# dryman/HashMergeJoin

Measured on AMD Instinct MI355X. Metric: probe-side tuples/s + achieved HBM GB/s, |R|=|S|=2^28 u64 keys, higher is better.
Workload: dtype u64

## Files before the change

### hashmergejoin_amd/_lib.py

```python
import ctypes as C
import os

HMJ_MATERIALIZE = 0x01
HMJ_ORDERED = 0x02
HMJ_FIRST_WINS = 0x04
HMJ_CHECKSUM = 0x08
HMJ_SUM_PROBE = 0x10
HMJ_NULL_EQUAL = 0x20
HMJ_OK, HMJ_E_ARG, HMJ_E_NODEV, HMJ_E_OOM, HMJ_E_HIP, HMJ_E_UNSUPPORTED = 0, -1, -2, -3, -4, -5
HMJ_E_RCCL, HMJ_E_PEER, HMJ_E_TIMEOUT = -6, -7, -8
HMJ_ABI_VERSION = 5
HMJ_PATH_SLAB, HMJ_PATH_EXACT, HMJ_PATH_UNIQ_WRITE, HMJ_PATH_SPLIT, HMJ_PATH_WINDOW = 0x1, 0x2, 0x4, 0x8, 0x10
HMJ_PATH_ORDER_DEFERRED, HMJ_PATH_ORDER_BY_KEY, HMJ_PATH_PREPARED, HMJ_PATH_CHUNKED_BUILD = 0x20, 0x40, 0x80, 0x100
HMJ_PATH_HOT_KEY_HINT = 0x200
HMJ_PATH_SLAB_PROBE = 0x400
HMJ_PATH_SORTED_WRITE = 0x800
HMJ_PATH_SORTED_FK = 0x1000
HMJ_PATH_DENSE_BUILD = 0x2000
HMJ_PATH_GLOBAL_TABLE = 0x100000
HMJ_PATH_ORDER_BY_RANK_SORT = 0x200000
HMJ_PATH_ORDERED_EXPANSION = 0x400000
HMJ_PATH_LDS_TABLE = 0x800000
HMJ_PATH_RANK_RUNS = 0x1000000
HMJ_PATH_RANK_LOOKUP_IN_PASS = 0x2000000
HMJ_PATH_SORT_MSD = 0x4000000
HMJ_PATH_KEY_RANGES = 0x8000000
HMJ_PATH_SLAB_ONE_PASS = 0x80000
HMJ_PATH_HOST_PIPELINE = 0x4000
HMJ_PATH_SORTED_FK_HALF = 0x8000
HMJ_PATH_LOOKBACK_TIMEOUT = 0x10000
HMJ_PATH_SORTED_FK_WIDE = 0x20000
HMJ_PATH_PRESORTED = 0x40000

_HERE = os.path.dirname(os.path.abspath(__file__))
_U64P = C.POINTER(C.c_uint64)


class HmjError(RuntimeError):
    def __init__(self, code, msg):
        super().__init__("hmj error %d: %s" % (code, msg))
        self.code = code


class JoinResult(C.Structure):
    _fields_ = [("n_matches", C.c_uint64), ("sum_r", C.c_uint64), ("sum_s", C.c_uint64),
                ("xor_fold", C.c_uint64), ("mix_sum", C.c_uint64), ("sum_probe_all", C.c_uint64),
                ("key", C.c_void_p), ("rval", C.c_void_p), ("sval", C.c_void_p)]

    def checks(self):
        return {k: int(getattr(self, k)) for k in ("n_matches", "sum_r", "sum_s", "xor_fold", "mix_sum")}


HMJ_JOIN_INNER, HMJ_JOIN_SEMI, HMJ_JOIN_ANTI, HMJ_JOIN_PROBE_OUTER = 0, 1, 2, 3


class JoinOpts(C.Structure):
    _fields_ = [("struct_size", C.c_uint32), ("kind", C.c_uint32), ("outer_fill", C.c_uint64),
                ("n_probe_matched", C.c_uint64), ("n_probe_unmatched", C.c_uint64)]


HMJ_BUILD_SEMI, HMJ_BUILD_ANTI, HMJ_BUILD_OUTER, HMJ_FULL_OUTER = 1, 2, 3, 4


class BuildJoinOpts(C.Structure):
    _fields_ = [("struct_size", C.c_uint32), ("kind", C.c_uint32), ("build_fill", C.c_uint64), ("probe_fill", C.c_uint64),
# ... 223 lines not shown
                ("ms_partition_build", C.c_float), ("ms_partition_probe", C.c_float),
                ("ms_hist", C.c_float), ("ms_scan", C.c_float), ("ms_scatter", C.c_float),
                ("ms_offsets", C.c_float), ("ms_probe_count", C.c_float),
                ("ms_out_scan", C.c_float), ("ms_probe_write", C.c_float), ("ms_order", C.c_float),
                ("radix_bits", C.c_int), ("radix_passes", C.c_int),
                ("n_scatter_launches", C.c_int), ("n_split_retries", C.c_int),
                ("bytes_scatter", C.c_uint64), ("bytes_hist", C.c_uint64),
                ("bytes_probe_count", C.c_uint64), ("bytes_probe_write", C.c_uint64),
                ("path", C.c_uint32), ("key_prefix_bits", C.c_int32), ("key_window_low", C.c_int32),
                ("n_probe_items", C.c_uint32), ("ms_scatter_pass0", C.c_float), ("ms_scatter_pass1", C.c_float)]

    def as_dict(self):
        return {n: getattr(self, n) for n, _ in self._fields_}


class PlanDesc(C.Structure):
    _fields_ = [("struct_size", C.c_uint32), ("path", C.c_uint32), ("radix_bits", C.c_int32), ("radix_passes", C.c_int32),
                ("pass_bits", C.c_int32 * 4), ("key_prefix_bits", C.c_int32), ("key_window_low", C.c_int32),
                ("n_partitions", C.c_uint32), ("probe_items", C.c_uint32), ("attempts", C.c_uint32), ("refused", C.c_uint32),
                ("cooling", C.c_uint32), ("workload", C.c_uint64)]

    def as_dict(self):
        d = {n: getattr(self, n) for n, _ in self._fields_}
        d["pass_bits"] = list(self.pass_bits)
        return d


HMJ_REFUSED_GTABLE_SHAPE, HMJ_REFUSED_GTABLE_COOLING, HMJ_REFUSED_GTABLE_GAVE_UP = 0x1, 0x2, 0x4
HMJ_REFUSED_RANK_SORT_MODEL, HMJ_REFUSED_RANK_SORT_COOLING, HMJ_REFUSED_RANK_SORT_GAVE_UP = 0x8, 0x10, 0x20
HMJ_REFUSED_SLAB_SHAPE, HMJ_REFUSED_SLAB_COOLING, HMJ_REFUSED_SLAB_SORTED_INPUT, HMJ_REFUSED_SLAB_OVERFLOW = 0x40, 0x80, 0x100, 0x200
HMJ_REFUSED_FAST_WRITE_COOLING, HMJ_REFUSED_FAST_WRITE_GAVE_UP = 0x400, 0x800
HMJ_REFUSED_SLAB_PROBE_COOLING, HMJ_REFUSED_SLAB_PROBE_OVERFLOW = 0x1000, 0x2000
HMJ_REFUSED_PREFIX_VIOLATED, HMJ_REFUSED_EXPANSION_GAVE_UP = 0x4000, 0x8000
HMJ_COOL_UNIQ_WRITE, HMJ_COOL_SORTED_WRITE, HMJ_COOL_GTABLE, HMJ_COOL_GTABLE_WRITE = 0x1, 0x2, 0x4, 0x8
HMJ_COOL_RANK_SORT, HMJ_COOL_RANK_SORT_SLAB, HMJ_COOL_EXPANSION, HMJ_COOL_SORT_SLAB = 0x10, 0x20, 0x40, 0x80
HMJ_COOL_SLAB, HMJ_COOL_SLAB_PROBE, HMJ_COOL_ONE_PASS_WRITE, HMJ_COOL_EXACT_PREFIX = 0x100, 0x200, 0x400, 0x800
HMJ_COOL_RANK_RUNS, HMJ_COOL_SORT_MSD = 0x1000, 0x2000


HMJ_PLACE_MAX_CAND = 4


class PlaceInfo(C.Structure):
    _fields_ = [("name", C.c_char * 16), ("bytes", C.c_uint64), ("fill_TBps", C.c_float), ("candidates", C.c_int),
                ("ms_search", C.c_float), ("searched", C.c_int), ("aborted", C.c_int), ("budget_ms", C.c_float),
                ("cand_ms_alloc", C.c_float * HMJ_PLACE_MAX_CAND), ("cand_ms_fill", C.c_float * HMJ_PLACE_MAX_CAND),
                ("cand_TBps", C.c_float * HMJ_PLACE_MAX_CAND)]


def lib_path():
    return os.environ.get("HMJ_LIB") or os.path.join(_HERE, "libhmj_hip.so")


class ExchangeInfo(C.Structure):
    _fields_ = [("n_ranks", C.c_int), ("owner_mode", C.c_int), ("rounds_build", C.c_uint32), ("rounds_probe", C.c_uint32),
                ("recv_build", C.c_uint64), ("recv_probe", C.c_uint64), ("ms_split", C.c_float),
                ("ms_exchange_build", C.c_float), ("ms_exchange_probe", C.c_float), ("ms_local", C.c_float),
                ("ms_total", C.c_float), ("digit_bits", C.c_int32), ("digit_low", C.c_int32), ("n_subjoins", C.c_uint32),
                ("fallback", C.c_uint32), ("sample_max_share", C.c_float), ("ms_kernels", C.c_float),
                ("ms_exposed", C.c_float)]

    def as_dict(self):
        return {n: getattr(self, n) for n, _ in self._fields_}


HMJ_MAX_RANKS, HMJ_MAX_ROUNDS = 16, 16
HMJ_UNIQUE_ID_BYTES = 128
HMJ_OWNER_DIGIT, HMJ_OWNER_SPLIT = 0, 1


# ... 110 lines not shown
```

### hashmergejoin_amd/csrc/api.hip

```cpp
#include <hip/hip_runtime.h>
#include <sys/mman.h>

#include <algorithm>
#include <cstdio>
#include <cstdlib>
#include <chrono>
#include <cmath>
#include <cstring>
#include <mutex>
#include <string>
#include <thread>
#include <vector>

#include "hmj_ctx.h"

using hmj::u32;
using hmj::u64;
using namespace hmj_host;

namespace hmj_host {

constexpr int kMaxEvents = 1024;

int fail(hmj_ctx* c, int code, const char* what, hipError_t e) {
// ... 29 lines not shown
  acc->ms_scatter_pass[0] += t.ms_scatter_pass[0];
  acc->ms_scatter_pass[1] += t.ms_scatter_pass[1];
  if (t.radix_passes) {
    acc->radix_bits = t.radix_bits;
    acc->radix_passes = t.radix_passes;
    acc->key_prefix_bits = t.key_prefix_bits;
    acc->key_window_low = t.key_window_low;
  }
  acc->n_probe_items += t.n_probe_items;
}

static int ilog2_u64(uint64_t v) { return v ? 63 - __builtin_clzll(v) : 0; }
uint64_t workload_signature(uint64_t n_build, uint64_t n_probe, uint32_t flags, int kind) {
  const uint32_t mode = ((flags & HMJ_ORDERED) ? 4u : 0u) | ((flags & (HMJ_MATERIALIZE | HMJ_ORDERED)) ? 2u : 0u) |
                        ((flags & HMJ_FIRST_WINS) ? 1u : 0u);
  return ((uint64_t)(kind & 31) << 20) | ((uint64_t)mode << 16) | ((uint64_t)ilog2_u64(n_build) << 8) | (uint64_t)ilog2_u64(n_probe);
}
WorkloadMemo* memo_for(hmj_ctx* c, uint64_t sig) {
  auto it = c->memos.find(sig);
  if (it == c->memos.end()) {
    if (c->memos.size() >= 1024) c->memos.clear();
    it = c->memos.emplace(sig, c->memo_init).first;
  }
  c->wm = &it->second;
  c->wm_sig = sig;
  return c->wm;
}
uint32_t WorkloadMemo::cooling() const {
  return (uniq_cooldown ? HMJ_COOL_UNIQ_WRITE : 0u) | (sorted_cooldown ? HMJ_COOL_SORTED_WRITE : 0u) | (gtable_cooldown ? HMJ_COOL_GTABLE : 0u) |
         (gtable_write_cooldown ? HMJ_COOL_GTABLE_WRITE : 0u) | (gtable_sort_cooldown ? HMJ_COOL_RANK_SORT : 0u) |
         (gtable_sort_slab_cooldown ? HMJ_COOL_RANK_SORT_SLAB : 0u) | (expand_cooldown ? HMJ_COOL_EXPANSION : 0u) |
         (sort_slab_cooldown ? HMJ_COOL_SORT_SLAB : 0u) | (slab_cooldown ? HMJ_COOL_SLAB : 0u) | (slab_probe_cooldown ? HMJ_COOL_SLAB_PROBE : 0u) |
         (one_pass_write_cooldown ? HMJ_COOL_ONE_PASS_WRITE : 0u) | (exact_prefix_joins ? HMJ_COOL_EXACT_PREFIX : 0u) |
         (rank_runs_cooldown ? HMJ_COOL_RANK_RUNS : 0u) | (sort_msd_cooldown ? HMJ_COOL_SORT_MSD : 0u);
}

int wait_arrival(hmj_ctx* c, hipEvent_t ev) {
  if (c->arrive_wait) return c->arrive_wait(c, ev);
  HIP_TRY(hipStreamWaitEvent(c->stream, ev, 0));
  return HMJ_OK;
}

int ensure_dev(hmj_ctx* c, DevBuf& b, size_t bytes) {
  if (bytes <= b.cap) return HMJ_OK;
  if (c && (&b == &c->rbuf[0] || &b == &c->rbuf[1] || &b == &c->r_off || &b == &c->slab_br || &b == &c->cnt_br))
    c->prep.valid = false;
  if (b.p) {
    hipError_t e = hipFree(b.p);
    b.p = nullptr;
    b.cap = 0;
    if (e != hipSuccess) return fail(c, HMJ_E_HIP, "hipFree", e);
  }
  size_t want = bytes + (bytes >> 4) + 256;
#ifdef HMJ_DEV
  if (const char* e = getenv("HMJ_ALLOC_PAD_KB")) want += (size_t)atoll(e) << 10;
  if (const char* e = getenv("HMJ_ALLOC_ROUND_MB")) {
    const size_t g = (size_t)atoll(e) << 20;
    if (g) want = (want + g - 1) / g * g;
  }
#endif
  const auto t_alloc0 = std::chrono::steady_clock::now();
  hipError_t e = hipMalloc(&b.p, want);
  if (e != hipSuccess) {
    b.p = nullptr;
    (void)hipGetLastError();
    return fail(c, HMJ_E_OOM, "hipMalloc", e);
  }
// ... 424 lines not shown
  a.r_off = (const u32*)c->r_off.p;
  a.S = Sp;
  a.s_off = (const u32*)c->s_off.p;
  a.P = P;
  a.Q = Q;
  a.accum = (u64*)c->accum.p;
  return a;
}
static hmj::ProbeArgs slab_probe_args(hmj_ctx* c, const hmj::SlabGeom* build_slabs, const void* Rp, const DevBuf& s_slab,
                                      const DevBuf& s_cnt, u32 s_cap, u32 P, u32 Q) {
  hmj::ProbeArgs a;
  std::memset(&a, 0, sizeof(a));
  if (build_slabs) {
    a.R = c->slab_br.p;
    a.r_cnt = (const u32*)c->cnt_br.p;
    a.r_cap = build_slabs->CB;
    a.r_cnt_n = c->cnt_br.cap / 4;
    a.r_rows = c->slab_br.cap / 16;
  } else {
    a.R = Rp;
    a.r_off = (const u32*)c->r_off.p;
  }
  a.S = s_slab.p;
  a.s_cnt = (const u32*)s_cnt.p;
  a.s_cap = s_cap;
  a.s_cnt_n = s_cnt.cap / 4;
  a.s_rows = s_slab.cap / 16;
  a.P = P;
  a.Q = Q;
  a.accum = (u64*)c->accum.p;
  return a;
}

static int slab_pass_a(hmj_ctx* c, const void* in, u32 n, int rel, int low, int bits, const hmj::SlabGeom& g, bool arriving) {
  u64* acc = (u64*)c->accum.p;
  const u64 a_rows = c->slab_a.cap / 16, a_cnt = c->cnt_a.cap / 4;
  const int sp = span_begin(c, K_SCATTER, rel, 0);
  if (arriving) {
    u32 w_done = 0;
    for (size_t i = 0; i < c->arrive_ev.size(); i++) {
      RC_TRY(wait_arrival(c, c->arrive_ev[i]));
      const bool last = i + 1 == c->arrive_ev.size();
      const u32 w_end = last ? g.WA : (u32)std::min<u64>(g.WA, c->arrive_rows[i] / g.rpw);
      if (w_end > w_done) {
        HIP_TRY(hmj::launch_slab_a(in, n, low, bits, g, c->slab_a.p, a_rows, (u32*)c->cnt_a.p, a_cnt, acc, c->stream, w_done, w_end));
        w_done = w_end;
      }
    }
  } else {
    HIP_TRY(hmj::launch_slab_a(in, n, low, bits, g, c->slab_a.p, a_rows, (u32*)c->cnt_a.p, a_cnt, acc, c->stream));
  }
  span_end(c, sp);
  c->timing.bytes_scatter += 32ull * n;
  return HMJ_OK;
}
static int slab_passes(hmj_ctx* c, const void* in, u32 n, int rel, int low, int ba, int bb, const hmj::SlabGeom& g, DevBuf& sb,
                       DevBuf& cb, bool arriving) {
  RC_TRY(slab_pass_a(c, in, n, rel, low, ba, g, arriving));
  const int sp = span_begin(c, K_SCATTER, rel, 1);
  HIP_TRY(hmj::launch_slab_b(c->slab_a.p, (const u32*)c->cnt_a.p, ba, low + ba, bb, g, sb.p, sb.cap / 16, (u32*)cb.p, cb.cap / 4,
                             (u64*)c->accum.p, c->stream));
  span_end(c, sp);
  c->timing.bytes_scatter += 32ull * n;
  return HMJ_OK;
}

static int clear_matched(hmj_ctx* c, size_t slots, u32** matched) {
  const size_t bytes = (slots / 32 + 1) * 4;
  RC_TRY(ensure_dev(c, c->matched, bytes));
  *matched = (u32*)c->matched.p;
  HIP_TRY(hipMemsetAsync(c->matched.p, 0, bytes, c->stream));
  return HMJ_OK;
}

int order_rows(hmj_ctx* c, const u32* vstart, const u32* in_base32, const u64* in_base64, u32 P, u32 Q, int low,
               u64 n, bool by_key_only, bool many_per_key, const u64** rk, const u64** rr, const u64** rs, int* retry_code) {
  const size_t bytes = (size_t)n * 8;
  RC_TRY(ensure_dev(c, c->ord_key, bytes));
  RC_TRY(ensure_dev(c, c->ord_rval, bytes));
  RC_TRY(ensure_dev(c, c->ord_sval, bytes));
  const bool can_sort = n <= 0xFFFFFFFFull;
  if (by_key_only && !can_sort) {
    *retry_code = kRetryNoWinOrdered;
    return HMJ_OK;
  }
  int sp = span_begin(c, K_ORDER, -1);
  HIP_TRY(hmj::launch_order((const u64*)c->part_out_off.p, vstart, in_base32, in_base64, P, Q, low,
                            (const u64*)c->out_key.p, (const u64*)c->out_rval.p, (const u64*)c->out_sval.p,
                            (u64*)c->ord_key.p, (u64*)c->ord_rval.p, (u64*)c->ord_sval.p, (u64*)c->accum.p,
                            can_sort ? 65536u : 0u, many_per_key, c->num_cus * 4, c->stream));
  span_end(c, sp);
  u64* h = (u64*)c->h_accum.p;
  HIP_TRY(hipMemcpyAsync(&h[hmj::ACC_ERR], (u64*)c->accum.p + hmj::ACC_ERR, 8, hipMemcpyDeviceToHost, c->stream));
  HIP_TRY(hipStreamSynchronize(c->stream));
  if (h[hmj::ACC_ERR] & hmj::ERR_ORDER_FAIL)
    return fail(c, HMJ_E_UNSUPPORTED, "HMJ_ORDERED: one partition's result exceeds 2^31-1 rows and the whole result 2^32-1 rows");
// ... 520 lines not shown

static int run_slab_join(hmj_ctx* c, const JoinCall& j, const JoinPlan& p) {
  const bool materialize = j.materialize(), first = j.first(), extra = j.extra();
  const u32 nb = j.nb, np = j.np, np_plan = p.np_plan, P = p.P;
  const int* pass_bits = p.pass_bits;
  hmj::SlabGeom gr, gs;
  if (p.allow_slab && c->slab_mode && c->wm->slab_cooldown == 0 && !c->prepare_only && !(c->timing.path & HMJ_PATH_SLAB) &&
      !((!materialize || p.fast_write) && p.Q == 1 && p.probe_fits && p.passes == 2 && pass_bits[0] <= hmj::SLAB_MAX_BITS &&
        pass_bits[1] <= hmj::SLAB_MAX_BITS && p.dense_scale <= 2.5))
    c->plan.refused |= HMJ_REFUSED_SLAB_SHAPE;
  if (!(p.allow_slab && c->slab_mode && c->wm->slab_cooldown == 0 && (!materialize || p.fast_write) && p.Q == 1 &&
        p.probe_fits &&
        p.passes == 2 && pass_bits[0] <= hmj::SLAB_MAX_BITS && pass_bits[1] <= hmj::SLAB_MAX_BITS &&
        slab_sizes_ok(c, nb, np_plan, materialize || np_plan < nb) &&
        p.dense_scale <= 2.5 &&
        hmj::slab_geometry(nb, pass_bits[0], pass_bits[1], &gr, 0, 1.0, p.dense_scale) &&
        hmj::slab_geometry(np_plan, pass_bits[0], pass_bits[1], &gs, 0,
                           (nb && np_plan > nb) ? (double)np_plan / (double)nb : 1.0, p.dense_scale)))
    return kPlanNotTaken;
  const bool reuse = c->prep.valid && c->prep.slab && c->prep.ptr == j.R && c->prep.n == nb &&
                     c->prep.low == p.low && c->prep.B == p.B;
  c->prep.valid = false;
  c->timing.path |= HMJ_PATH_SLAB | (reuse ? HMJ_PATH_PREPARED : 0u);
  c->timing.n_probe_items = P;
  const int ba = pass_bits[0], bb = pass_bits[1];
  const u64 rows_a = gr.rows_a > gs.rows_a ? gr.rows_a : gs.rows_a;
  const u32 wa = gr.WA > gs.WA ? gr.WA : gs.WA;
  RC_TRY(ensure_dev(c, c->slab_a, rows_a * 16));
  RC_TRY(ensure_dev(c, c->cnt_a, ((size_t)wa << ba) * 4));
  RC_TRY(ensure_dev(c, c->slab_br, gr.rows_b * 16));
  RC_TRY(ensure_dev(c, c->slab_bs, gs.rows_b * 16));
  RC_TRY(ensure_dev(c, c->cnt_br, (size_t)P * gr.KB * 4));
  RC_TRY(ensure_dev(c, c->cnt_bs, (size_t)P * gs.KB * 4));
  if (!reuse) RC_TRY(slab_passes(c, j.R, nb, 0, p.low, ba, bb, gr, c->slab_br, c->cnt_br, false));
  if (!c->prepare_only) RC_TRY(slab_passes(c, j.S, np, 1, p.low, ba, bb, gs, c->slab_bs, c->cnt_bs, !c->arrive_ev.empty()));
  u64* hh;
  if (c->prepare_only) {
    RC_TRY(read_accum(c, &hh));
    if (hh[hmj::ACC_ERR] & hmj::ERR_SLAB) {
      c->wm->slab_cooldown = 8;
      return kRetryNoSlab;
    }
    c->prep.valid = true;
    c->prep.slab = true;
    c->prep.ptr = j.R;
    c->prep.n = nb;
    c->prep.low = p.low;
    c->prep.B = p.B;
    return HMJ_OK;
  }
  hmj::ProbeArgs sa = slab_probe_args(c, &gr, nullptr, c->slab_bs, c->cnt_bs, gs.CB, P, 1);
  if (p.fast_write)
    return unique_key_write(c, sa, true, nb, np, p.low, extra, p.verify_pfx ? p.prefix : 0, p.pfx_ref, j.ordered(), j.to_host,
                            p.fk_wide_plan, p.dense_scale, j.out);
#ifdef HMJ_DEV
  sa.debug = c->dev_ablate;
#endif
  int sp = span_begin(c, K_PROBE_COUNT, -1);
  if (first || extra) {
    sa.extra = (extra ? 1u : 0u) | (first ? 2u : 0u);
    HIP_TRY(hmj::launch_probe_count_ext(sa, nullptr, nullptr, true, c->num_cus, c->stream));
  } else {
    HIP_TRY(hmj::launch_probe_count_slab(sa, c->num_cus, c->stream));
  }
  span_end(c, sp);
  c->timing.bytes_probe_count = 16ull * ((u64)nb + np);
  RC_TRY(read_accum(c, &hh));
  if (hh[hmj::ACC_ERR] & hmj::ERR_SLAB) {
    c->wm->slab_cooldown = 8;
    return kRetryNoSlab;
  }
  result_sums(j.out, hh);
  return HMJ_OK;
}

static int partition_build_exact(hmj_ctx* c, const JoinCall& j, const JoinPlan& p, const void** Rp) {
  const bool reuse_exact = c->prep.valid && !c->prep.slab && c->prep.ptr == j.R && c->prep.n == j.nb &&
                           c->prep.low == p.low && c->prep.B == p.B;
  c->prep.valid = false;
  c->timing.path |= HMJ_PATH_EXACT | (reuse_exact ? HMJ_PATH_PREPARED : 0u);
  if (reuse_exact) {
    *Rp = c->prep.Rp;
  } else {
    RC_TRY(partition_relation(c, j.R, j.nb, c->rbuf, p.low, p.passes, p.pass_bits, 0, Rp, p.asc_r));
    const int s = span_begin(c, K_OFFSETS, -1);
    HIP_TRY(hmj::launch_part_offsets(*Rp, j.nb, p.low, p.B, (u32*)c->r_off.p, c->stream));
    span_end(c, s);
  }
  if (c->prepare_only) {
    HIP_TRY(hipStreamSynchronize(c->stream));
    c->prep.valid = true;
    c->prep.slab = false;
    c->prep.ptr = j.R;
    c->prep.Rp = *Rp;
    c->prep.n = j.nb;
    c->prep.low = p.low;
    c->prep.B = p.B;
  }
  return HMJ_OK;
}

static int run_probe_slab_join(hmj_ctx* c, const JoinCall& j, const JoinPlan& p, const void* Rp) {
  const bool materialize = j.materialize(), first = j.first(), extra = j.extra();
// ... 1296 lines not shown
  if (const char* e = getenv("HMJ_SORT_MSD_MIN_LOG2")) {
    const int l = atoi(e);
    if (l >= 16 && l <= 32) c->sort_msd_min = 1ull << l;
  }
  if (const char* e = getenv("HMJ_SORT_SLAB_MIN_LOG2")) {
    const int l = atoi(e);
    if (l >= 12 && l <= 32) c->sort_slab_min = 1ull << l;
  }
  if (const char* e = getenv("HMJ_GTABLE_SORT_SLAB_MIN_LOG2")) {
    const int l = atoi(e);
    if (l >= 12 && l <= 32) c->gtable_sort_slab_min = 1ull << l;
  }
  if (const char* e = getenv("HMJ_GTABLE_SORT_FANOUT")) c->gtable_sort_fanout = atoi(e) > 0 ? (u32)atoi(e) : 1u;
  if (const char* e = getenv("HMJ_PLACE")) {
    c->place_tune = atoi(e) != 0;
    if (atoi(e) > 0) {
      c->place_tries = atoi(e);
      c->place_search_always = true;
    }
  }
  if (const char* e = getenv("HMJ_PLACE_BUDGET_MS")) {
    if (atof(e) >= 0.0) c->place_budget_ms = (float)atof(e);
  }
  if (const char* e = getenv("HMJ_PLACE_MIN_MB")) {
    const long long mb = atoll(e);
    if (mb >= 1) c->place_min_bytes = (size_t)mb << 20;
  }
  if (const char* e = getenv("HMJ_UPLOAD")) c->staged_upload = std::strcmp(e, "staged") == 0;
  if (const char* e = getenv("HMJ_HOST_PIPELINE")) c->host_pipeline = atoi(e) != 0;
  if (const char* e = getenv("HMJ_SLAB_MIN_LOG2")) {
    const int l = atoi(e);
    if (l >= 16 && l <= 31) c->slab_min_rows = 1u << l;
  }
  if (const char* e = getenv("HMJ_SLAB_PROBE_KB")) {
    const int k = atoi(e);
    if (k >= 1 && k <= 512) c->slab_probe_kb = (u32)k;
  }
  if (const char* e = getenv("HMJ_TRACE")) c->trace = atoi(e) != 0;
#ifdef HMJ_DEV
  if (const char* e = getenv("HMJ_LTABLE")) c->ltable_mode = atoi(e) != 0;
  if (const char* e = getenv("HMJ_GTABLE_MAX_LOG2")) {
    const int l = atoi(e);
    if (l >= 0 && l <= 28) c->gtable_max_rows = 1ull << l;
  }
  if (const char* e = getenv("HMJ_GTABLE_FANOUT")) c->gtable_min_fanout = atoi(e) > 0 ? (u32)atoi(e) : 0u;
  if (const char* e = getenv("HMJ_GTABLE_WG")) c->gtable_wg_per_cu = atoi(e) > 0 ? atoi(e) : 8;
  if (const char* e = getenv("HMJ_BUILD_SORT_MSD")) c->build_sort_msd = atoi(e) != 0;
  if (const char* e = getenv("HMJ_GTABLE_SORT_SLAB")) c->gtable_sort_slab = atoi(e) != 0;
  if (const char* e = getenv("HMJ_FK_PAYLOAD_BUCKETS")) c->fk_payload_buckets = atoi(e) > 0 ? (u32)atoi(e) : 0u;
  if (const char* e = getenv("HMJ_ORDERED_EXPANSION")) c->expand_mode = atoi(e) != 0;
  if (const char* e = getenv("HMJ_SORT_SLAB")) c->sort_slab = atoi(e) != 0;
  if (const char* e = getenv("HMJ_GTABLE_SLOTS")) c->gtable_slots_per_row = atoi(e) >= 2 ? (u32)atoi(e) : 2u;
  if (const char* e = getenv("HMJ_GTABLE_MAX_LOG_CAP")) {
    const int l = atoi(e);
    if (l >= 10 && l <= 30) c->gtable_max_log_cap = l;
  }
  if (const char* e = getenv("HMJ_DENSE_PLAN")) c->dense_plan = atoi(e) != 0;
  if (const char* e = getenv("HMJ_SORTED_WRITE")) {
    c->sorted_mode = atoi(e) != 0;
    c->memo_init.sorted_chained = atoi(e) == 2;
    c->sorted_chained_forced = atoi(e) == 2 || atoi(e) == 3;
  }
  if (const char* e = getenv("HMJ_SORTED_HALF")) c->sorted_half = atoi(e) != 0;
  if (const char* e = getenv("HMJ_FK_PLAN"))
    c->fk_plan = std::strcmp(e, "wide") == 0 ? 1 : std::strcmp(e, "half") == 0 ? 2 : std::strcmp(e, "narrow") == 0 ? 3 : 0;
  if (const char* e = getenv("HMJ_SORTED_WIDE")) c->memo_init.sorted_wide = atoi(e) != 0;
// ... 776 lines not shown
```

### hashmergejoin_amd/csrc/hmj_ctx.h

```cpp
#pragma once
#include <hip/hip_runtime.h>

#include <string>
#include <unordered_map>
#include <vector>

#include "../../include/hmj.h"
#include "hmj_args.h"
#include "hmj_dev.h"
#include "hmj_launch.h"
#include "hmj_smallplan.h"

struct hmj_comm;
struct hmj_ctx;

namespace hmj_host {

struct DevBuf {
  void* p = nullptr;
  size_t cap = 0;
};
struct HostBuf {
  void* p = nullptr;
  size_t cap = 0;
  bool pinned = true;
};
template <int N>
struct PhaseEvents {
  hipEvent_t ev[N] = {};
  int record(hmj_ctx* c, int k);
  float ms(int a, int b) {
    float t = 0.f;
    if (ev[a] && ev[b] && hipEventElapsedTime(&t, ev[a], ev[b]) != hipSuccess) {
      (void)hipGetLastError();
      t = 0.f;
    }
    return t;
  }
  void destroy() {
    for (hipEvent_t& e : ev) {
      if (e) (void)hipEventDestroy(e);
      e = nullptr;
    }
// ... 108 lines not shown
  void each_buf(F f) {
    for (DevBuf* b : {&acc, &below, &tied, &blk, &blk_off, &tie[0], &tie[1], &words, &map}) f(*b);
  }
};

enum Kind {
  K_TOTAL = 0, K_H2D, K_D2H, K_HIST, K_SCAN, K_SCATTER, K_OFFSETS, K_PROBE_COUNT, K_OUT_SCAN,
  K_PROBE_WRITE, K_ORDER, K_NKINDS
};
struct Span {
  int kind, rel, e0, e1;
  int pass;
};

struct WorkloadMemo {
  int uniq_cooldown = 0;
  int sorted_cooldown = 0;
  bool sorted_chained = false;
  bool sorted_wide = true;
  bool sorted_fk = false;
  int sorted_fk_age = 0;
  int gtable_cooldown = 0;
  int gtable_write_cooldown = 0;
  int gtable_sort_cooldown = 0;
  int gtable_sort_slab_cooldown = 0;
  int rank_runs_cooldown = 0;
  int rank_lookup_cooldown = 0;
  int expand_cooldown = 0;
  int sort_slab_cooldown = 0;
  int sort_msd_cooldown = 0;
  int slab_cooldown = 0;
  int slab_probe_cooldown = 0;
  int one_pass_write_cooldown = 0;
  int exact_prefix_joins = 0;
  uint32_t cooling() const;
};

}

struct hmj_ctx {
  using DevBuf = hmj_host::DevBuf;
  using HostBuf = hmj_host::HostBuf;
  using Span = hmj_host::Span;
  using WorkloadMemo = hmj_host::WorkloadMemo;
  using u32 = hmj::u32;
  using u64 = hmj::u64;
  int device = 0, num_cus = 256;
  hipStream_t own_stream = nullptr, stream = nullptr;
  DevBuf rbuf[2], sbuf[2], in_r, in_s, hist, totals, r_off, s_off, part_count, part_out_off, accum,
      out_key, out_rval, out_sval, ord_key, ord_rval, ord_sval, offs64, irregular, matched, vparts,
      slab_a, slab_br, slab_bs, cnt_a, cnt_br, cnt_bs, lookback, gtab, piece_off,
      split_r, split_s, split_off, cat_key, cat_rval, cat_sval,
      msd_off,
      bmatched, bsweep;
  hmj_host::KeyJoinWs str_ws, col_ws, mix_ws;
  hmj_host::GroupWs grp_ws;
  hmj_host::OrderWs ord_ws;
  hmj_host::TakeWs take_ws;
  hmj_host::TakeStrWs takestr_ws;
  hmj_host::AggWs agg_ws;
  hmj_host::FilterWs filter_ws;
  hmj_host::WindowWs window_ws;
  hmj_host::TopkWs topk_ws;
  int memo_kind = 0;
  HostBuf h_accum, h_key, h_rval, h_sval;
  int host_threads = 0;
// ... 42 lines not shown
  uint64_t gtable_max_rows = 1ull << 17;
  u32 gtable_min_fanout = 0;
  uint64_t gtable_min_probe = 1;
  int gtable_wg_per_cu = 8;
  u32 gtable_slots_per_row = 16;
  int gtable_max_log_cap = 18;
  bool ltable_mode = true;
  bool gtable_sort_mode = true;
  u32 gtable_sort_fanout = 128;
  bool rank_runs_mode = true;
  int rank_runs_max_cut = 10;
  int rank_runs_max_group = 3;
  int rank_runs_max_level = 2;
  uint64_t big_join_rows = 1ull << 29;
  bool promote_to_ordered = true;
  bool key_ranges = true;
  int key_ranges_force = 0;
  bool rank_runs_wave = true;
  bool build_sort_msd = true;
  bool gtable_sort_slab = true;
  u64 gtable_sort_slab_min = 1ull << 25;
  bool expand_mode = true;
  u32 fk_payload_buckets = 24;
  u32 expand_fk_fanout = 0;
  bool expand_allow_rebits = true;
  int expand_rebits = 0;
  bool sort_msd = true;
  double sort_msd_mean = 1200.0;
  int sort_msd_max_bits = 18;
  u64 sort_msd_min = 1ull << 22;
  bool sort_slab = true;
  u64 sort_slab_min = 1ull << 25;
  int slab_mode = 1;
  bool staged_upload = false;
  bool host_pipeline = true;
  hipStream_t copy_stream = nullptr;
  std::vector<hipEvent_t> copy_ev;
  bool split_mode = true;
  bool window_mode = true;
  u32 slab_min_rows = 1u << 21;
  u32 slab_probe_kb = 0;
  bool one_pass_slab = true;
  int scatter_variant = 1;
  bool profiling = false;
  bool trace = false;
#ifdef HMJ_DEV
  u32 dev_ablate = 0;
#endif
  std::vector<hipEvent_t> events;
  std::vector<Span> spans;
  int ev_used = 0;
  hmj_timing timing;
  std::string last_error;
  hmj_comm* comm = nullptr;
  std::vector<u64> arrive_rows;
  std::vector<hipEvent_t> arrive_ev;
  bool sample_build_only = false;
  int (*arrive_wait)(hmj_ctx*, hipEvent_t) = nullptr;
};


namespace hmj_host {
int fail(hmj_ctx* c, int code, const char* what, hipError_t e = hipSuccess);
#define HIP_TRY(expr)                                                        \
  do {                                                                       \
    hipError_t _e = (expr);                                                  \
// ... 38 lines not shown
```

### hashmergejoin_amd/csrc/hmj_dev.h

```cpp
#pragma once
#include <hip/hip_runtime.h>
#include <stdint.h>

namespace hmj {

typedef unsigned long long u64;
typedef unsigned int u32;
typedef unsigned short u16;

struct __attribute__((aligned(16))) Tup {
  u64 key;
  u64 val;
};

constexpr int kWave = 64;
#ifndef HMJ_SCAN_DPP
#define HMJ_SCAN_DPP 1
#endif

#ifndef HMJ_STREAM_POLICY
#define HMJ_STREAM_POLICY 2
#endif
typedef u64 u64x2_t __attribute__((ext_vector_type(2)));
__device__ __forceinline__ void store_stream(Tup* p, const Tup& v) {
// ... 51 lines not shown
          slot[r] = (slot[r] + 1) & mask;
          any_live = true;
        }
      }
    }
  }
}

constexpr int RP_THREADS = 512;
constexpr int RP_WAVES = RP_THREADS / kWave;
constexpr int RP_ITEMS = 8;
constexpr int RP_TILE = RP_THREADS * RP_ITEMS;
constexpr int RP_MAX_BITS = 9;
constexpr int RP_MAXD = 1 << RP_MAX_BITS;
constexpr int RP_MAX_BLOCKS = 2048;

constexpr int PB_THREADS = 1024;
constexpr int PB_CAP = 5120;
constexpr int PB_LOG_NB = 12;
constexpr int PB_TARGET_AVG = 4096;
constexpr int PB_PLAN_SLACK = 256;

constexpr int SLAB_KB = 4;
constexpr int SLAB_MAX_BITS = 9;

enum { ACC_N = 0, ACC_SUM_R, ACC_SUM_S, ACC_XOR, ACC_MIX, ACC_SUM_P, ACC_ERR, ACC_PAD };
constexpr u64 ERR_SLAB = 2;
constexpr u64 ERR_ORDER_DEFER = 16;
constexpr u64 ERR_ORDER_FAIL = 32;
constexpr u64 ERR_SORTED = 64;
constexpr u64 ERR_FASTPATH = 8;
constexpr u64 ERR_GTABLE = 128;
constexpr u64 ERR_PREFIX = 4;

__device__ __forceinline__ u64 mix64(u64 x) {
  x ^= x >> 30;
  x *= 0xBF58476D1CE4E5B9ull;
  x ^= x >> 27;
  x *= 0x94D049BB133111EBull;
  x ^= x >> 31;
  return x;
}

__device__ __forceinline__ u64 tmix(u64 key, u64 rval, u64 sval) {
  u64 t = mix64(key);
  t = mix64(t ^ rval);
  t = mix64(t + sval);
  return t;
}

__device__ __forceinline__ int lane_id() {
  return __builtin_amdgcn_mbcnt_hi(~0u, __builtin_amdgcn_mbcnt_lo(~0u, 0u));
}

__device__ __forceinline__ u32 popc_below(u64 m) {
  return __builtin_amdgcn_mbcnt_hi((u32)(m >> 32), __builtin_amdgcn_mbcnt_lo((u32)m, 0u));
}

__device__ __forceinline__ u32 wave_incl_scan_u32(u32 v, int ) {
#if HMJ_SCAN_DPP
  v += (u32)__builtin_amdgcn_update_dpp(0, (int)v, 0x111, 0xF, 0xF, false);
  v += (u32)__builtin_amdgcn_update_dpp(0, (int)v, 0x112, 0xF, 0xF, false);
  v += (u32)__builtin_amdgcn_update_dpp(0, (int)v, 0x114, 0xF, 0xF, false);
  v += (u32)__builtin_amdgcn_update_dpp(0, (int)v, 0x118, 0xF, 0xF, false);
  v += (u32)__builtin_amdgcn_update_dpp(0, (int)v, 0x142, 0xA, 0xF, false);
  v += (u32)__builtin_amdgcn_update_dpp(0, (int)v, 0x143, 0xC, 0xF, false);
// ... 83 lines not shown
```

### hashmergejoin_amd/csrc/hmj_launch.h

```cpp
#pragma once
#include <hip/hip_runtime.h>
#include <stddef.h>
#include <stdint.h>

#include <atomic>

namespace hmj {
typedef unsigned long long u64;
typedef unsigned int u32;

struct SmemAttrOnce {
  std::atomic<unsigned long long> devices{0};
};
inline hipError_t ensure_max_smem(SmemAttrOnce& once, const void* kernel, size_t bytes) {
  int dev = 0;
  hipError_t e = hipGetDevice(&dev);
  if (e != hipSuccess) return e;
  const unsigned long long bit = 1ull << (dev & 63);
  if (dev < 64 && (once.devices.load(std::memory_order_acquire) & bit)) return hipSuccess;
  e = hipFuncSetAttribute(kernel, hipFuncAttributeMaxDynamicSharedMemorySize, (int)bytes);
  if (e != hipSuccess) return e;
  if (dev < 64) once.devices.fetch_or(bit, std::memory_order_release);
  return hipSuccess;
}

constexpr int kMaxRanks = 16;
struct OwnerFn {
  u32 mode;
  u32 G;
  u64 spl[kMaxRanks - 1];
};
int radix_tile_rows(int bits, int variant);
void radix_pass_geometry(u32 n, int tile, u32* nblk, u32* rows_per_block);
size_t radix_scatter_smem_bytes();
hipError_t launch_radix_hist(const void* in, u32 n, int tile, int shift, int bits, u32* hist,
                             u32 nblk, u32 rows_per_block, hipStream_t st, const OwnerFn* own = nullptr);
hipError_t launch_owner_scatter(const void* in, void* out, u32 n, int bits, const OwnerFn& own,
                                const u32* hist_scanned, const u32* totals, u32 nblk, u32 rows_per_block,
                                u64* offsets_out, hipStream_t st);
hipError_t launch_radix_rowscan(u32* hist, u32 nblk, int bits, u32* totals, hipStream_t st);
hipError_t launch_radix_scatter(const void* in, void* out, u32 n, int variant, int shift, int bits,
                                const u32* hist_scanned, const u32* totals, u32 nblk,
                                u32 rows_per_block, u64* offsets_out, hipStream_t st);
struct SlabGeom {
  u32 WA, rpw, CA, CB, KB;
  u64 rows_a, rows_b;
};
bool slab_geometry(u32 n, int bits_a, int bits_b, SlabGeom* g, u32 kb = 0, double fan = 1.0, double density = 1.0);
bool slab_geometry_one_pass(u32 n, int bits, double keys_per_digit, u32 max_workers, SlabGeom* g, double density = 1.0);
u32 slab_capacity(double mean, double fan);
hipError_t launch_slab_a(const void* in, u32 n, int shift, int bits, const SlabGeom& g, void* slab_a, u64 slab_a_rows,
                         u32* cnt_a, u64 cnt_a_n, u64* accum, hipStream_t st, u32 w_begin = 0, u32 w_end = 0xFFFFFFFFu);
hipError_t launch_slab_b(const void* slab_a, const u32* cnt_a, int bits_a, int shift, int bits,
                         const SlabGeom& g, void* slab_b, u64 slab_b_rows, u32* cnt_b, u64 cnt_b_n, u64* accum, hipStream_t st);
hipError_t launch_key_sample(const void* R, u32 nb, const void* S, u32 np, u64* out, hipStream_t st);
hipError_t launch_key_exact(const void* R, u32 nb, const void* S, u32 np, u64 ref, u64* out, int num_cus, hipStream_t st,
                            bool ref_is_first_key = false);
hipError_t launch_check_partitioned(const void* a, u32 n, int low, int bits, u32* flag, int num_cus, hipStream_t st);
hipError_t launch_part_offsets(const void* a, u32 n, int low, int bits, u32* off, hipStream_t st);

struct ProbeArgs {
  const void* R;
  const u32* r_off;
  const void* S;
  const u32* s_off;
  u32 P;
  u32 Q;
  u64* part_count;
  const u64* part_out_off;
  u64* out_key;
  u64* out_rval;
  u64* out_sval;
  u64 out_cap;
  u64* accum;
  const u32* item_list;
  const u32* n_item_list;
  const u32* r_cnt;
  const u32* s_cnt;
  u32 r_cap, s_cap;
  u32 s_wa, s_ppi;
  u64 r_cnt_n, s_cnt_n;
  u64 r_rows, s_rows;
  const u64* item_base;
  const u32* r_end;
  const u32* s_end;
  u32 extra;
  u32 pfx_shift;
  u64 pfx_val;
  u32* matched;
  u32 debug;
};
hipError_t launch_probe(const ProbeArgs& a, int mode, bool first_wins, bool extra, int grid,
                        hipStream_t st);
int probe_default_grid(int num_cus);
hipError_t launch_probe_kind(const ProbeArgs& a, int mode, int kind, bool first_wins, u64 fill, int grid, hipStream_t st);
hipError_t launch_probe_build_kind(const ProbeArgs& a, int mode, int kind, u64 fill, u32* bmark, int grid, hipStream_t st);
hipError_t launch_build_sweep(const ProbeArgs& a, const u32* r_off, u32 P, const u32* vstart, u64* sweep_n, int mode,
                              bool set, u64 fill, int num_cus, hipStream_t st);
hipError_t launch_probe_count_ext(const ProbeArgs& a, u32* irregular, u32* n_irregular, bool slab,
                                  int num_cus, hipStream_t st);
hipError_t launch_probe_count_slab(const ProbeArgs& a, int num_cus, hipStream_t st);
hipError_t launch_probe_write_sorted(const ProbeArgs& a, bool slab, bool fk, int shape, u64* lookback, bool chained, int key_low,
                                     int num_cus, hipStream_t st);
hipError_t launch_probe_write_uniq(const ProbeArgs& a, bool slab, int num_cus, hipStream_t st);
hipError_t launch_slab_np(const u32* cnt, u32 P, u64* out, hipStream_t st);
hipError_t launch_probe_count_fast(const ProbeArgs& a, u32* irregular, u32* n_irregular, bool big,
                                   bool per_partition_counts, int num_cus, hipStream_t st);
hipError_t launch_scan_u64(const u64* in, u64* out_excl, u32 n, hipStream_t st);
hipError_t launch_probe_expand_ordered(const ProbeArgs& a, int key_low, int num_cus, hipStream_t st);
hipError_t launch_order(const u64* part_out_off, const u32* vstart, const u32* in_base32, const u64* in_base64, u32 P, u32 Q,
                        int low, const u64* akey, const u64* arval, const u64* asval, u64* bkey, u64* brval,
                        u64* bsval, u64* accum, u32 defer_rows, bool many_per_key, int grid, hipStream_t st);
hipError_t launch_compact(const u64* part_out_off, const u32* in_base32, const u64* in_base64, u32 P, const u64* akey,
                          const u64* arval, const u64* asval, u64* bkey, u64* brval, u64* bsval, int grid, hipStream_t st);
hipError_t launch_rekey(void* pairs, u64 n, const u64* col, hipStream_t st);

hipError_t launch_gtable_build(const void* R, u32 nb, void* tab, int log_cap, u64* accum, bool first, int num_cus,
                               hipStream_t st);
hipError_t launch_gtable_probe(const void* S, u32 np, const void* tab, int log_cap, const void* R, u64* accum, bool first,
                               bool extra, int num_cus, int wg_per_cu, hipStream_t st);
hipError_t launch_gtable_write(const void* S, u32 np, const void* tab, int log_cap, const void* R, u64* accum, u64* out_key,
                               u64* out_rval, u64* out_sval, bool first, bool extra, int num_cus, int wg_per_cu, hipStream_t st);

hipError_t launch_ltable_probe(const void* R, u32 nb, const void* S, u32 np, u64* accum, bool first, bool extra, int num_cus, hipStream_t st);
int ltable_max_rows();
hipError_t launch_sval_range(const void* S, u32 np, u64* out2 , int num_cus, hipStream_t st,
                             u32 every = 1 );
// ... 43 lines not shown
```

### hashmergejoin_amd/csrc/probe.hip

```cpp
#include "hmj_dev.h"
#include "hmj_launch.h"
#include <type_traits>

namespace hmj {

constexpr u32 PB_NB = 1u << PB_LOG_NB;
constexpr u32 NIL = 0xFFFFu;
static_assert(PB_CAP < 0xFFFF, "chain links are 16-bit");

struct ProbeSmem {
  u64 key[PB_CAP];
  u64 val[PB_CAP];
  u32 head[PB_NB];
  u32 aux[PB_CAP];
  u16 next[PB_CAP];
  u32 scratch[PB_THREADS / kWave + 1];
  u64 pcount;
  u64 red[8];
  u64 obase;
  u32 wtot[PB_THREADS / kWave];
  u32 nslot;
};
constexpr u32 PB_BATCH = 2 * PB_THREADS;
static_assert(PB_BATCH <= PB_CAP, "a batch must fit an empty table");

__device__ __forceinline__ u32 key_bucket(u64 key, int sh, u32 mask) {
  return (sh >= 0 ? (u32)(key >> sh) : (u32)(key << (-sh))) & mask;
}

__device__ __forceinline__ u32 tab_hash(u64 k) {
  u32 x = (u32)k ^ ((u32)(k >> 32) * 0x85EBCA6Bu);
  x *= 0x9E3779B1u;
  return x >> (32 - PB_LOG_NB);
}
// ... 850 lines not shown
};

template <int LOG_NB>
__device__ __forceinline__ u32 fast_hash(u64 k) {
  u32 x = (u32)k ^ ((u32)(k >> 32) * 0x85EBCA6Bu);
  x *= 0x9E3779B1u;
  return x >> (32 - LOG_NB);
}

template <int THREADS, int ROWS = FP_ROWS>
__device__ __forceinline__ void fp_load(Tup (&t)[ROWS], const Tup* __restrict__ base, u32 n,
                                        int tid) {
#pragma unroll
  for (int k = 0; k < ROWS; k++) {
    u32 i = k * THREADS + tid;
    t[k] = base[i < n ? i : n - 1];
  }
}

static_assert(SLAB_KB == 4, "fp_load_slab / fp_load_pieces / slab_np_kernel unroll exactly four pieces per partition");
template <int THREADS, int ROWS = FP_ROWS>
__device__ __forceinline__ void fp_load_slab(Tup (&t)[ROWS], const Tup* __restrict__ base, u32 cap,
                                             u32 p1, u32 p2, u32 p3, u32 n, int tid) {
#pragma unroll
  for (int k = 0; k < ROWS; k++) {
    u32 i = k * THREADS + tid;
    i = i < n ? i : n - 1;
    const u32 j = (i >= p1) + (i >= p2) + (i >= p3);
    const u32 pre = j == 0 ? 0u : (j == 1 ? p1 : (j == 2 ? p2 : p3));
    t[k] = base[(u64)j * cap + (i - pre)];
  }
}

template <int THREADS>
__device__ __forceinline__ void fp_load_pieces(Tup (&t)[FP_ROWS], const Tup* __restrict__ base, u32 cap, u32 cnt_mine, int tid) {
  constexpr int QT = THREADS / 4;
  const u32 g = (u32)tid / QT, l = (u32)tid % QT;
  const Tup* __restrict__ piece = base + (u64)g * cap;
  const u32 last = cnt_mine ? cnt_mine - 1 : 0;
#pragma unroll
  for (int k = 0; k < FP_ROWS; k++) {
    const u32 r = l + (u32)k * QT;
    t[k] = piece[r < last ? r : last];
  }
}

template <int THREADS, int LOG_NB, bool PCOUNT, bool SLAB, int OUT>
__global__ __launch_bounds__(THREADS, 4) void probe_count_fast_kernel(
    ProbeArgs a, u32* __restrict__ irregular, u32* __restrict__ n_irregular) {
  typedef FastSmem<THREADS, LOG_NB> Smem;
  constexpr u32 CAP = Smem::CAP, NB = 1u << LOG_NB;
  constexpr bool PIECES = SLAB && OUT == 0 && !PCOUNT && HMJ_PROBE_PIECES;
  constexpr u32 QT = THREADS / 4, PIECE_CAP = FP_ROWS * QT;
  extern __shared__ __attribute__((aligned(16))) unsigned char smem_raw[];
  Smem& sm = *reinterpret_cast<Smem*>(smem_raw);
  const Tup* __restrict__ R = static_cast<const Tup*>(a.R);
  const Tup* __restrict__ S = static_cast<const Tup*>(a.S);
  const u32* __restrict__ r_off = a.r_off;
  const u32* __restrict__ s_off = a.s_off;
  const u32* __restrict__ r_end = (SLAB || a.r_end == nullptr) ? a.r_off + 1 : a.r_end;
  const u32* __restrict__ s_end = (SLAB || a.s_end == nullptr) ? a.s_off + 1 : a.s_end;
  const u32 P = a.P;
  const int tid = threadIdx.x;
  u64 acc_n = 0, acc_r = 0, acc_s = 0, acc_x = 0, acc_m = 0, acc_p = 0;
  bool pfx_bad = false, giveup = false;
  for (u32 i = tid; i < NB; i += THREADS) sm.head[i] = 0;
  if (tid < 2) sm.itemcnt[tid] = 0;
  u32 epoch = 0;
  u32 prev_p = 0xFFFFFFFFu, parity = 0;

  u32 p = blockIdx.x;
  u32 rb = 0, nb = 0, sb = 0, np = 0;
  bool regular = false;
  Tup br[FP_ROWS], pr[FP_ROWS], pq[FP_ROWS];
  u32 r1 = 0, r2 = 0, r3 = 0, s1 = 0, s2 = 0, s3 = 0, r1n = 0, r2n = 0, r3n = 0, s1n = 0, s2n = 0, s3n = 0;
  u32 rm = 0, sm_ = 0, rmn = 0, smn = 0;
  const u32 my_piece = (u32)tid / QT;
  bool slab_bad = false;
  if (p < P) {
    if (SLAB) {
      const u32* rc = a.r_cnt + (u64)p * SLAB_KB;
      const u32* sc = a.s_cnt + (u64)p * SLAB_KB;
      r1 = rc[0]; r2 = r1 + rc[1]; r3 = r2 + rc[2]; nb = r3 + rc[3];
      s1 = sc[0]; s2 = s1 + sc[1]; s3 = s2 + sc[2]; np = s3 + sc[3];
      if (nb > CAP || np > CAP) slab_bad = true;
      if (PIECES) {
        rm = my_piece == 0 ? rc[0] : my_piece == 1 ? rc[1] : my_piece == 2 ? rc[2] : rc[3];
        sm_ = my_piece == 0 ? sc[0] : my_piece == 1 ? sc[1] : my_piece == 2 ? sc[2] : sc[3];
        if (rc[0] > PIECE_CAP || rc[1] > PIECE_CAP || rc[2] > PIECE_CAP || rc[3] > PIECE_CAP || sc[0] > PIECE_CAP ||
            sc[1] > PIECE_CAP || sc[2] > PIECE_CAP || sc[3] > PIECE_CAP) {
          slab_bad = true;
          nb = CAP + 1;
        }
      }
    } else {
      rb = r_off[p]; nb = r_end[p] - rb;
      sb = s_off[p]; np = s_end[p] - sb;
    }
    regular = nb && np && nb <= CAP && np <= CAP;
    if (regular) {
      if (PIECES) {
        fp_load_pieces<THREADS>(br, R + (u64)p * SLAB_KB * a.r_cap, a.r_cap, rm, tid);
        fp_load_pieces<THREADS>(pr, S + (u64)p * SLAB_KB * a.s_cap, a.s_cap, sm_, tid);
      } else if (SLAB) {
        fp_load_slab<THREADS>(br, R + (u64)p * SLAB_KB * a.r_cap, a.r_cap, r1, r2, r3, nb, tid);
        if (OUT == 0) fp_load_slab<THREADS>(pr, S + (u64)p * SLAB_KB * a.s_cap, a.s_cap, s1, s2, s3, np, tid);
      } else {
        fp_load<THREADS>(br, R + rb, nb, tid);
        if (OUT == 0) fp_load<THREADS>(pr, S + sb, np, tid);
      }
    }
  }
  const Tup* __restrict__ dummy = reinterpret_cast<const Tup*>(a.accum);
  auto load_build = [&](Tup (&t)[FP_ROWS], bool ok, u32 pp, u32 rb_, u32 nb_, u32 q1, u32 q2, u32 q3, u32 mine) {
    if (PIECES)
      fp_load_pieces<THREADS>(t, ok ? R + (u64)pp * SLAB_KB * a.r_cap : dummy, ok ? a.r_cap : 0u, ok ? mine : 1u, tid);
    else if (SLAB)
      fp_load_slab<THREADS>(t, ok ? R + (u64)pp * SLAB_KB * a.r_cap : dummy, ok ? a.r_cap : 0u, ok ? q1 : 1u, ok ? q2 : 1u,
                            ok ? q3 : 1u, ok ? nb_ : 1u, tid);
    else
      fp_load<THREADS>(t, ok ? R + rb_ : dummy, ok ? nb_ : 1u, tid);
  };
  auto load_probe = [&](Tup (&t)[FP_ROWS], bool ok, u32 pp, u32 sb_, u32 np_, u32 q1, u32 q2, u32 q3, u32 mine) {
    if (PIECES)
      fp_load_pieces<THREADS>(t, ok ? S + (u64)pp * SLAB_KB * a.s_cap : dummy, ok ? a.s_cap : 0u, ok ? mine : 1u, tid);
    else if (SLAB)
      fp_load_slab<THREADS>(t, ok ? S + (u64)pp * SLAB_KB * a.s_cap : dummy, ok ? a.s_cap : 0u, ok ? q1 : 1u, ok ? q2 : 1u,
                            ok ? q3 : 1u, ok ? np_ : 1u, tid);
    else
      fp_load<THREADS>(t, ok ? S + sb_ : dummy, ok ? np_ : 1u, tid);
  };
  const int tid_outer = tid;
  while (p < P) {
    int tid = tid_outer;
    if constexpr (OUT != 0) asm volatile("" : "+v"(tid));
    u64 out_base = (u64)sb;
    if constexpr (OUT == 1 && SLAB) {
      const u64* ibp = a.item_base + p;
      asm volatile("s_load_dwordx2 %0, %1, 0x0\n\ts_waitcnt lgkmcnt(0)" : "=s"(out_base) : "s"(ibp) : "memory");
    }
    const u32 pn = __builtin_amdgcn_readfirstlane(p + gridDim.x);
    u32 rb2 = 0, nb2 = 0, sb2 = 0, np2 = 0;
    bool regular2 = false;
    if (pn < P) {
      if (SLAB) {
        const u32* rc = a.r_cnt + (u64)pn * SLAB_KB;
        const u32* sc = a.s_cnt + (u64)pn * SLAB_KB;
        r1n = rc[0]; r2n = r1n + rc[1]; r3n = r2n + rc[2]; nb2 = r3n + rc[3];
        s1n = sc[0]; s2n = s1n + sc[1]; s3n = s2n + sc[2]; np2 = s3n + sc[3];
        if (nb2 > CAP || np2 > CAP) slab_bad = true;
        if (PIECES) {
          rmn = my_piece == 0 ? rc[0] : my_piece == 1 ? rc[1] : my_piece == 2 ? rc[2] : rc[3];
          smn = my_piece == 0 ? sc[0] : my_piece == 1 ? sc[1] : my_piece == 2 ? sc[2] : sc[3];
          if (rc[0] > PIECE_CAP || rc[1] > PIECE_CAP || rc[2] > PIECE_CAP || rc[3] > PIECE_CAP || sc[0] > PIECE_CAP ||
              sc[1] > PIECE_CAP || sc[2] > PIECE_CAP || sc[3] > PIECE_CAP) {
            slab_bad = true;
            nb2 = CAP + 1;
          }
        }
      } else {
        rb2 = r_off[pn]; nb2 = r_end[pn] - rb2;
        sb2 = s_off[pn]; np2 = s_end[pn] - sb2;
      }
      regular2 = nb2 && np2 && nb2 <= CAP && np2 <= CAP;
    }
    if (OUT == 0) {
      load_probe(pq, regular2, pn, sb2, np2, s1n, s2n, s3n, smn);
    } else if (regular) {
      if (SLAB)
        fp_load_slab<THREADS>(pr, S + (u64)p * SLAB_KB * a.s_cap, a.s_cap, s1, s2, s3, np, tid);
      else
        fp_load<THREADS>(pr, S + sb, np, tid);
    }
    if (regular) {
      lds_barrier();
      if (PCOUNT && prev_p != 0xFFFFFFFFu && tid == 0) {
        a.part_count[prev_p] = sm.itemcnt[parity ^ 1];
        sm.itemcnt[parity ^ 1] = 0;
      }
      if (PCOUNT) prev_p = 0xFFFFFFFFu;
      epoch++;
      if (epoch == 0x10000u) {
        for (u32 i = tid; i < NB; i += THREADS) sm.head[i] = 0;
        epoch = 1;
        lds_barrier();
      }
      const u32 tag = epoch << 16;
      if (!HMJ_ABLATE(1u)) {
        u32 old[FP_ROWS];
#pragma unroll
        for (int k = 0; k < FP_ROWS; k++) {
          const u32 i = k * THREADS + tid;
          old[k] = tag | NIL;
          if (PIECES ? ((u32)tid % QT + (u32)k * QT < rm) : (i < nb)) {
            if (a.pfx_shift && (br[k].key >> a.pfx_shift) != a.pfx_val) pfx_bad = true;
            sm.key[i] = br[k].key;
            sm.val[i] = br[k].val;
            old[k] = atomicExch(&sm.head[fast_hash<LOG_NB>(br[k].key)], tag | i);
          }
        }
#pragma unroll
        for (int k = 0; k < FP_ROWS; k++) {
          const u32 i = k * THREADS + tid;
          if (PIECES ? ((u32)tid % QT + (u32)k * QT < rm) : (i < nb)) sm.next[i] = ((old[k] >> 16) == epoch) ? (u16)old[k] : (u16)NIL;
        }
      } else {
#pragma unroll
        for (int k = 0; k < FP_ROWS; k++) acc_r += br[k].key;
      }
      load_build(br, regular2, pn, rb2, nb2, r1n, r2n, r3n, rmn);
      lds_barrier();
      const u64 n_before = acc_n;
      if (!HMJ_ABLATE(1u)) {
        u32 cur[FP_ROWS];
        u32 cnt[FP_ROWS], first[FP_ROWS];
#pragma unroll
        for (int k = 0; k < FP_ROWS; k++) {
          const u32 j = k * THREADS + tid;
          cur[k] = NIL;
          cnt[k] = 0;
          first[k] = OUT == 2 ? NIL : 0;
          if (PIECES ? ((u32)tid % QT + (u32)k * QT < sm_) : (j < np)) {
            if (a.pfx_shift && (pr[k].key >> a.pfx_shift) != a.pfx_val) pfx_bad = true;
            if (OUT >= 1 && (a.extra & 1u)) acc_p += pr[k].val;
            const u32 hv = sm.head[fast_hash<LOG_NB>(pr[k].key)];
            cur[k] = ((hv >> 16) == epoch) ? (hv & 0xFFFFu) : NIL;
          }
        }
        for (; !HMJ_ABLATE(2u);) {
          bool any = false;
#pragma unroll
          for (int k = 0; k < FP_ROWS; k++) any |= (cur[k] != NIL);
          if (!__any(any)) break;
#pragma unroll
          for (int k = 0; k < FP_ROWS; k++) {
            if (cur[k] != NIL) {
              const u32 i = cur[k];
              const u64 kk = sm.key[i], vv = sm.val[i];
              cur[k] = sm.next[i];
              if (kk == pr[k].key) {
                if (OUT == 2 && (a.extra & 2u)) {
                  first[k] = i < first[k] ? i : first[k];
                } else {
                  acc_n++;
                  acc_r += vv;
                  acc_s += pr[k].val;
                  if (OUT == 1) {
                    if (cnt[k] == 0) first[k] = i;
                    cnt[k]++;
                  }
                  if (OUT >= 1 && (a.extra & 1u)) {
                    const u64 m = tmix(kk, vv, pr[k].val);
                    acc_x ^= m;
                    acc_m += m;
                  }
                }
              }
            }
          }
        }
        if (OUT == 2 && (a.extra & 2u)) {
#pragma unroll
          for (int k = 0; k < FP_ROWS; k++) {
            if (first[k] != NIL) {
              const u64 vv = sm.val[first[k]];
              acc_n++;
              acc_r += vv;
              acc_s += pr[k].val;
              if (a.extra & 1u) {
                const u64 m = tmix(pr[k].key, vv, pr[k].val);
                acc_x ^= m;
                acc_m += m;
              }
            }
          }
        }
        if (OUT == 1) {
          u64 packed = 0;
          bool cx = false;
#pragma unroll
          for (int k = 0; k < FP_ROWS; k++) {
            cx |= cnt[k] > 1;
            packed |= (u64)(cnt[k] ? 1u : 0u) << (12 * k);
          }
          const int lane = tid & 63, wv = tid >> 6;
          const bool wave_dup = __any(cx);
          u64 incl = packed;
#pragma unroll
          for (int o = 1; o < kWave; o <<= 1) {
            u64 t = __shfl_up(incl, o, kWave);
            if (lane >= o) incl += t;
          }
          if (lane == 63) {
            sm.wscan[wv] = incl;
            sm.wdup[wv] = wave_dup ? 1u : 0u;
          }
          lds_barrier();
          u64 pre = 0, tot = 0;
          u32 dup = 0;
#pragma unroll
          for (int q = 0; q < THREADS / kWave; q++) {
            const u64 ws = sm.wscan[q];
            dup |= sm.wdup[q];
            if (q < wv) pre += ws;
            tot += ws;
          }
          const u64 ex = pre + incl - packed;
          if (dup) {
            giveup = true;
          } else {
            u64 o = out_base;
            u32 total = 0;
#pragma unroll
            for (int k = 0; k < FP_ROWS; k++) {
              if (cnt[k]) {
                const u64 d = o + ((ex >> (12 * k)) & 0xFFFu);
                a.out_key[d] = pr[k].key;
                a.out_rval[d] = sm.val[first[k]];
                a.out_sval[d] = pr[k].val;
              }
              const u32 tk = (u32)((tot >> (12 * k)) & 0xFFFu);
              o += tk;
              total += tk;
            }
            if (tid == 0) a.part_count[p] = total;
          }
        }
      } else {
#pragma unroll
        for (int k = 0; k < FP_ROWS; k++) acc_r += pr[k].key;
      }
      if (PCOUNT) {
        const u32 mine = (u32)(acc_n - n_before);
        const u32 ws = (u32)wave_sum_u64(mine);
        if ((tid & 63) == 0 && ws) atomicAdd(&sm.itemcnt[parity], ws);
        prev_p = p;
        parity ^= 1;
      }
    } else {
      if ((PCOUNT || OUT == 1) && tid == 0 && !(nb && np)) a.part_count[p] = 0;
      if (OUT == 1 && nb && np) giveup = true;
      if (OUT >= 1 && (a.extra & 1u) && !nb) {
        if (SLAB) {
          const Tup* base = S + (u64)p * SLAB_KB * a.s_cap;
          for (u32 j = tid; j < np; j += THREADS) {
            const u32 pc = (j >= s1) + (j >= s2) + (j >= s3);
            const u32 pre = pc == 0 ? 0 : pc == 1 ? s1 : pc == 2 ? s2 : s3;
            acc_p += base[(u64)pc * a.s_cap + (j - pre)].val;
          }
        } else {
          for (u32 j = tid; j < np; j += THREADS) acc_p += S[sb + j].val;
        }
      }
      if (OUT != 1 && !SLAB && tid == 0 && nb && np) irregular[atomicAdd(n_irregular, 1u)] = p;
      load_build(br, regular2, pn, rb2, nb2, r1n, r2n, r3n, rmn);
    }
    if (OUT == 0) {
#pragma unroll
      for (int k = 0; k < FP_ROWS; k++) pr[k] = pq[k];
    }
    p = pn; rb = rb2; nb = nb2; sb = sb2; np = np2; regular = regular2;
    r1 = r1n; r2 = r2n; r3 = r3n; s1 = s1n; s2 = s2n; s3 = s3n;
    rm = rmn; sm_ = smn;
  }
  if (SLAB && slab_bad && tid == 0) atomicOr(&a.accum[ACC_ERR], ERR_SLAB);
  if (OUT == 1 && __any(giveup) && (tid & 63) == 0) atomicOr(&a.accum[ACC_ERR], ERR_FASTPATH);
  if (__any(pfx_bad) && (tid & 63) == 0) atomicOr(&a.accum[ACC_ERR], ERR_PREFIX);
  lds_barrier();
  if (PCOUNT && prev_p != 0xFFFFFFFFu && tid == 0) a.part_count[prev_p] = sm.itemcnt[parity ^ 1];
  if (tid < 8) sm.red[tid] = 0;
  lds_barrier();
  const u64 v[6] = {acc_n, acc_r, acc_s, acc_x, acc_m, acc_p};
  block_accumulate(sm.red, a.accum, v, 1u << ACC_XOR);
}

constexpr int SW_LOGB = 12, SW_NB = 1 << SW_LOGB, SW_MAXBUCKET = 32;
constexpr u64 LB_AGG = 1ull << 62, LB_PFX = 2ull << 62, LB_MASK = (1ull << 62) - 1;
constexpr u32 LB_SPIN_LIMIT = 1u << 22;

template <int THREADS>
struct SortedSmem {
  static constexpr int CAP = THREADS * FP_ROWS, CAPB = CAP, LOGB = SW_LOGB;
  u64 key[CAP];
  u64 val[CAP];
  u64 sval[CAP];
  u32 cnt[SW_NB];
  u16 bstart[SW_NB + 2];
  u16 perm[CAP];
  u32 mbits[2][CAP / 32];
  u32 scratch[THREADS / kWave + 1];
  u32 tick[2];
  u32 flag;
  u64 obase;
  u64 red[8];
};

constexpr int SWF_LOGB = 11, SWF_CAPB = 4608, SWF_MAXDUP = 1024;
constexpr int SWF_HALF_THREADS = 512, SWF_HALF_ROWS = 6, SWF_HALF_CAPB = 2048, SWF_HALF_LOGB = 10;
constexpr int SWF_WIDE_ROWS = 6, SWF_WIDE_CAPB = 2560;
// ... 1095 lines not shown
      vr_beg[v] = rb + b;
      vr_end[v] = rb + e;
    }
    if (ns == 1) {
      vs_beg[v] = sb;
      vs_end[v] = sb + np;
    } else {
      const u32 step = (np + ns - 1) / ns;
      const u32 b = qs * step, e = (b + step < np) ? b + step : np;
      vs_beg[v] = sb + (b < np ? b : np);
      vs_end[v] = sb + e;
    }
  }
}
hipError_t launch_split_parts(const u32* r_off, const u32* s_off, u32 P, u32 thr_rows, u32 slice_rows, u32 build_thr,
                              u32 build_slice, u32 cap_v, u32* vstart, u32* vr_beg, u32* vr_end, u32* vs_beg,
                              u32* vs_end, u32* nv_out, hipStream_t st) {
  hipLaunchKernelGGL(split_count_kernel, dim3(1), dim3(1024), 0, st, r_off, s_off, P, thr_rows, slice_rows, build_thr,
                     build_slice, cap_v, vstart, nv_out);
  hipLaunchKernelGGL(split_fill_kernel, dim3((cap_v + 255) / 256), dim3(256), 0, st, r_off, s_off, P, thr_rows,
                     slice_rows, build_thr, build_slice, cap_v, vstart, vr_beg, vr_end, vs_beg, vs_end);
  return hipGetLastError();
}

template <int MODE, bool FIRST, bool EXTRA>
static hipError_t launch_probe_t(const ProbeArgs& a, int grid, hipStream_t st) {
  static SmemAttrOnce attr_once;
  if (hipError_t e = ensure_max_smem(attr_once, reinterpret_cast<const void*>(probe_kernel<MODE, FIRST, EXTRA>), (size_t)sizeof(ProbeSmem)); e != hipSuccess) return e;
  hipLaunchKernelGGL((probe_kernel<MODE, FIRST, EXTRA>), dim3(grid), dim3(PB_THREADS),
                     sizeof(ProbeSmem), st, a);
  return hipGetLastError();
}

template <int THREADS, int LOG_NB, bool PCOUNT, bool SLAB = false, int OUT = 0>
static hipError_t launch_fast_t(const ProbeArgs& a, u32* irregular, u32* n_irregular, int grid,
                                hipStream_t st) {
  typedef FastSmem<THREADS, LOG_NB> Smem;
  static SmemAttrOnce attr_once;
  if (hipError_t e = ensure_max_smem(attr_once, reinterpret_cast<const void*>(probe_count_fast_kernel<THREADS, LOG_NB, PCOUNT, SLAB, OUT>), (size_t)sizeof(Smem)); e != hipSuccess) return e;
  if ((u32)grid > a.P) grid = (int)a.P;
  if (grid < 1) grid = 1;
  hipLaunchKernelGGL((probe_count_fast_kernel<THREADS, LOG_NB, PCOUNT, SLAB, OUT>), dim3(grid), dim3(THREADS),
                     sizeof(Smem), st, a, irregular, n_irregular);
  return hipGetLastError();
}

hipError_t launch_probe_count_fast(const ProbeArgs& a, u32* irregular, u32* n_irregular, bool big,
                                   bool per_partition_counts, int num_cus, hipStream_t st) {
  if (per_partition_counts) {
    if (big) return launch_fast_t<1024, BIG_LOG_NB, true>(a, irregular, n_irregular, num_cus * 4, st);
    return launch_fast_t<512, 11, true>(a, irregular, n_irregular, num_cus * 3 * 4, st);
  }
  if (big) return launch_fast_t<1024, BIG_LOG_NB, false>(a, irregular, n_irregular, num_cus * 4, st);
  return launch_fast_t<512, 11, false>(a, irregular, n_irregular, num_cus * 3 * 4, st);
}

static bool slab_operands_ok(const ProbeArgs& a) {
  const u64 pieces = (u64)a.P * SLAB_KB;
  return a.r_cnt && a.s_cnt && a.r_cnt_n >= pieces && a.s_cnt_n >= pieces && a.r_rows >= pieces * a.r_cap &&
         a.s_rows >= pieces * a.s_cap;
}

hipError_t launch_probe_write_uniq(const ProbeArgs& a, bool slab, int num_cus, hipStream_t st) {
  if (slab && !slab_operands_ok(a)) return hipErrorInvalidValue;
  if (slab) return launch_fast_t<1024, BIG_LOG_NB, false, true, 1>(a, nullptr, nullptr, num_cus * 4, st);
  return launch_fast_t<1024, BIG_LOG_NB, false, false, 1>(a, nullptr, nullptr, num_cus * 4, st);
}

template <bool SLAB, bool FK, bool EXTRA, bool PB = false>
static hipError_t launch_sorted_t(const ProbeArgs& a, u64* lookback, bool chained, int key_low, int grid, hipStream_t st) {
  typedef typename std::conditional<FK, SortedFkSmem<1024>, SortedSmem<1024>>::type Smem;
  static_assert(sizeof(Smem) <= 160 * 1024, "one workgroup's LDS");
  if constexpr (FK && !PB) {
    if (a.extra & 4u) return launch_sorted_t<SLAB, FK, EXTRA, true>(a, lookback, chained, key_low, grid, st);
  }
// ... 38 lines not shown
  if (grid < 1) grid = 1;
  if (fk && shape == 1)
    return launch_sorted_shape<SWF_HALF_THREADS, SWF_HALF_ROWS, SWF_HALF_CAPB, SWF_HALF_LOGB>(a, slab, lookback, chained, key_low, grid, st);
  if (fk && shape == 2)
    return launch_sorted_shape<1024, SWF_WIDE_ROWS, SWF_WIDE_CAPB, SWF_LOGB>(a, slab, lookback, chained, key_low, grid, st);
  if (slab) return fk ? launch_sorted_x<true, true>(a, lookback, chained, key_low, grid, st)
                      : launch_sorted_x<true, false>(a, lookback, chained, key_low, grid, st);
  return fk ? launch_sorted_x<false, true>(a, lookback, chained, key_low, grid, st)
            : launch_sorted_x<false, false>(a, lookback, chained, key_low, grid, st);
}

__global__ void slab_np_kernel(const u32* __restrict__ cnt, u32 P, u64* __restrict__ out) {
  u32 p = blockIdx.x * blockDim.x + threadIdx.x;
  if (p < P) {
    const u32* q = cnt + (u64)p * SLAB_KB;
    out[p] = (u64)q[0] + q[1] + q[2] + q[3];
  }
}
hipError_t launch_slab_np(const u32* cnt, u32 P, u64* out, hipStream_t st) {
  hipLaunchKernelGGL(slab_np_kernel, dim3((P + 255) / 256), dim3(256), 0, st, cnt, P, out);
  return hipGetLastError();
}

hipError_t launch_probe_count_ext(const ProbeArgs& a, u32* irregular, u32* n_irregular, bool slab,
                                  int num_cus, hipStream_t st) {
  if (slab && !slab_operands_ok(a)) return hipErrorInvalidValue;
  if (slab) return launch_fast_t<1024, BIG_LOG_NB, false, true, 2>(a, nullptr, nullptr, num_cus * 4, st);
  return launch_fast_t<1024, BIG_LOG_NB, false, false, 2>(a, irregular, n_irregular, num_cus * 4, st);
}

hipError_t launch_probe_count_slab(const ProbeArgs& a, int num_cus, hipStream_t st) {
  if (!slab_operands_ok(a)) return hipErrorInvalidValue;
  return launch_fast_t<1024, BIG_LOG_NB, false, true>(a, nullptr, nullptr, num_cus * 4, st);
}

hipError_t launch_probe(const ProbeArgs& a, int mode, bool first_wins, bool extra, int grid,
                        hipStream_t st) {
  if (!a.item_list && (u64)grid > (u64)a.P * a.Q) grid = (int)((u64)a.P * a.Q);
  if (grid < 1) grid = 1;
  if (a.s_ppi) {
    if (!a.s_cnt || (mode != 0 && mode != 3) || (mode == 3 && (!a.out_key || !a.out_rval || !a.out_sval || a.out_cap == 0)) || (first_wins && !a.matched) || a.s_wa == 0 || (u64)a.P * a.s_wa * a.s_cap > 0xFFFFFFFFull || (u64)a.Q * a.s_ppi < a.s_wa || (u64)(a.Q - 1) * a.s_ppi >= a.s_wa ||
        a.s_cnt_n < (u64)a.P * a.s_wa || a.s_rows < (u64)a.P * a.s_wa * a.s_cap)
      return hipErrorInvalidValue;
  } else if (a.s_cnt && (a.s_cnt_n < (u64)a.P * a.Q || a.s_rows < (u64)a.P * a.Q * a.s_cap || (u64)a.P * a.Q * a.s_cap > 0xFFFFFFFFull))
    return hipErrorInvalidValue;
#define HMJ_DISPATCH(M)                                                          \
  if (first_wins)                                                                \
    return extra ? launch_probe_t<M, true, true>(a, grid, st)                    \
                 : launch_probe_t<M, true, false>(a, grid, st);                  \
  else                                                                           \
    return extra ? launch_probe_t<M, false, true>(a, grid, st)                   \
                 : launch_probe_t<M, false, false>(a, grid, st);
  if (mode == 3 && !a.s_ppi) return hipErrorInvalidValue;
  if (mode == 0) {
    HMJ_DISPATCH(0)
  } else if (mode == 3) {
    HMJ_DISPATCH(3)
  } else if (mode == 1) {
    HMJ_DISPATCH(1)
  } else {
    if (first_wins) return launch_probe_t<2, true, false>(a, grid, st);
    return launch_probe_t<2, false, false>(a, grid, st);
  }
#undef HMJ_DISPATCH
}

// ... 426 lines not shown
```

### hashmergejoin_amd/csrc/radix.hip

```cpp
#include <cstdlib>
#include <cstring>

#include <type_traits>

#include "hmj_dev.h"
#include "hmj_launch.h"

namespace hmj {

template <int OWN>
__device__ __forceinline__ u32 owner_digit(u64 key, int shift, u32 mask, const OwnerFn& f) {
  if (OWN == 1) return (u32)__umul64hi(mix64(key), (u64)f.G);
  if (OWN == 2) {
    u32 d = 0;
#pragma unroll
    for (int i = 0; i < kMaxRanks - 1; i++) d += ((u32)i + 1 < f.G && key >= f.spl[i]) ? 1u : 0u;
    return d;
  }
  return (u32)(key >> shift) & mask;
}

template <int OWN>
__global__ __launch_bounds__(RP_THREADS) void radix_hist_kernel(const Tup* __restrict__ in, u32 n,
                                                                int shift, u32 mask,
// ... 177 lines not shown
    for (int h = 0; h < 2; h++) {
      Tup v[RP_ITEMS / 2];
#pragma unroll
      for (int r = 0; r < RP_ITEMS / 2; r++) {
        const u32 i = (h * (RP_ITEMS / 2) + r) * RP_THREADS + tid;
        if (FULL || i < tile_n) v[r] = sm.stage[i];
      }
      if (h == 0) {
#pragma unroll
        for (int r = 0; r < RP_ITEMS / 2; r++) {
          Tup z;
          z.key = 0;
          z.val = 0;
          sm.stage[r * RP_THREADS + tid] = z;
        }
      }
#pragma unroll
      for (int r = 0; r < RP_ITEMS / 2; r++) {
        const u32 i = (h * (RP_ITEMS / 2) + r) * RP_THREADS + tid;
        if (FULL || i < tile_n) {
          const u32 d = OWN ? owner_digit<OWN>(v[r].key, shift, mask, own) : digit_of<HI>(v[r].key, shift, mask);
          store_stream(&out[sm.delta[d] + i], v[r]);
        }
      }
    }
    for (int i = tid; i < RP_WAVES * RP_MAXD / 2; i += RP_THREADS)
      reinterpret_cast<u32*>(&sm.wcnt[0][0])[i] = 0;
    lds_barrier();
  }
}

constexpr int WC_ITEMS = 4;
constexpr int WC_LINE = 8;

#ifndef HMJ_WC_PLAN1
#define HMJ_WC_PLAN1 0
#endif
#ifndef HMJ_WC_FULLTILE
#define HMJ_WC_FULLTILE 1
#endif
#ifndef HMJ_WC_NOBAR5
#define HMJ_WC_NOBAR5 1
#endif
#ifdef HMJ_STAMPS
__device__ unsigned long long g_wc_stamps[32];
struct WcStamps {
  u32 acc[14];
  u64 last;
  int base;
  __device__ __forceinline__ void begin() {
    asm volatile("s_waitcnt vmcnt(0)" ::: "memory");
    last = __builtin_amdgcn_s_memtime();
  }
  __device__ __forceinline__ void mark(int i) {
    const u64 now = __builtin_amdgcn_s_memtime();
    acc[i] += (u32)(now - last);
    last = now;
  }
  __device__ __forceinline__ void flush() {
    if ((threadIdx.x & 63) == 0)
      for (int i = 0; i < 14; i++) atomicAdd(&g_wc_stamps[base + i], (unsigned long long)acc[i]);
  }
};
#define WC_STAMP_ARG , WcStamps& stamps
#define WC_STAMP_PASS , stamps
#define WC_MARK(i) stamps.mark(i)
#define WC_VMWAIT() asm volatile("s_waitcnt vmcnt(0)" ::: "memory")
#else
#define WC_STAMP_ARG
#define WC_STAMP_PASS
#define WC_MARK(i)
#define WC_VMWAIT()
#endif

template <int THREADS, int MAXD>
struct WcSmem {
  static constexpr int TILE = THREADS * WC_ITEMS;
  static constexpr int WAVES = THREADS / kWave;
  static constexpr int ZROWS = WAVES * MAXD * 8 / 16;
  static constexpr int MAXLINES = TILE / WC_LINE + 2 * MAXD;
  static_assert(ZROWS <= TILE && ZROWS % THREADS == 0, "lane masks must alias whole row slabs");
  static_assert(MAXD <= THREADS && MAXD * WC_LINE == TILE, "one digit per thread; carry == tile slots");
  union {
    Tup stage[TILE];
    u64 lanemask[WAVES][MAXD];
  };
  Tup carry[MAXD][WC_LINE];
  u16 wcnt[WAVES][MAXD];
  u32 tile_off[MAXD];
  u32 cflush[MAXD];
  static constexpr bool HAS_CF_TILE = MAXD <= 256;
  u32 cf_tile[HAS_CF_TILE ? MAXD : 1];
  u32 plan[MAXD];
  u32 pend[MAXD];
  u32 line_off[MAXD];
  u16 line_tab[MAXLINES];
  u32 total_lines;
  u32 scratch[WAVES + 1];
};

struct NoLimit {
  __device__ __forceinline__ u32 operator()(u32) const { return 0xFFFFFFFFu; }
};
template <int THREADS, int MAXD, bool HI, bool ALLVALID, bool LIMIT, typename Prefetch, typename Limit>
__device__ __forceinline__ void wc_tile(WcSmem<THREADS, MAXD>& sm, Tup (&t)[WC_ITEMS], u32 tile_n,
                                        Tup* __restrict__ out, int shift, u32 mask, u32 D,
                                        Prefetch&& prefetch, const Limit& limit, bool* ovf WC_STAMP_ARG) {
  typedef WcSmem<THREADS, MAXD> Smem;
  constexpr int WAVES = Smem::WAVES;
  const int tid = threadIdx.x, lane = tid & 63, w = tid >> 6;
  u16* wc = &sm.wcnt[w][0];
  u64* lm = &sm.lanemask[w][0];
  const u64 lanebit = 1ull << lane;
  const u32 wbase = (u32)w * (WC_ITEMS * 64) + lane;

  u32 dr[WC_ITEMS];
#ifdef HMJ_STAMPS
  stamps.last = __builtin_amdgcn_s_memtime();
  WC_VMWAIT();
  WC_MARK(0);
  stamps.acc[11]++;
#endif
#pragma unroll
  for (int r = 0; r < WC_ITEMS; r++) {
    u32 d = 0, rank = 0;
    if (ALLVALID || wbase + r * 64 < tile_n) {
      d = digit_of<HI>(t[r].key, shift, mask);
      __hip_atomic_fetch_or(&lm[d], lanebit, __ATOMIC_RELAXED, __HIP_MEMORY_SCOPE_WORKGROUP);
      const u64 m = __hip_atomic_load(&lm[d], __ATOMIC_RELAXED, __HIP_MEMORY_SCOPE_WORKGROUP);
      const u32 old = __hip_atomic_load(&wc[d], __ATOMIC_RELAXED, __HIP_MEMORY_SCOPE_WORKGROUP);
      const u32 below = popc_below(m);
      if (below == 0) {
        __hip_atomic_store(&lm[d], 0ull, __ATOMIC_RELAXED, __HIP_MEMORY_SCOPE_WORKGROUP);
        __hip_atomic_store(&wc[d], (u16)(old + (u32)__popcll(m)), __ATOMIC_RELAXED,
                           __HIP_MEMORY_SCOPE_WORKGROUP);
      }
      rank = old + below;
    }
    dr[r] = (d << 16) | rank;
  }
  WC_MARK(1);
  lds_barrier();
  WC_MARK(2);

#if HMJ_WC_PLAN1
  if (w == 0) {
    constexpr int DPL = MAXD / kWave;
    u32 cnt[DPL], nl[DPL], pd[DPL], cf[DPL], fl[DPL];
#pragma unroll
    for (int j = 0; j < DPL; j++) {
      const u32 d = (u32)j * kWave + lane;
      cnt[j] = nl[j] = pd[j] = cf[j] = fl[j] = 0;
      if (d < D) {
        u32 c[WAVES];
#pragma unroll
        for (int k = 0; k < WAVES; k++) c[k] = sm.wcnt[k][d];
        u32 run = 0;
#pragma unroll
        for (int k = 0; k < WAVES; k++) {
          sm.wcnt[k][d] = (u16)run;
          run += c[k];
        }
        cnt[j] = run;
        pd[j] = sm.pend[d];
        cf[j] = sm.cflush[d];
        u32 avail = pd[j] + run;
        if (LIMIT && cf[j] + avail > limit(d)) {
          *ovf = true;
          avail = 0;
          pd[j] = 0;
        }
        const u32 tail = (cf[j] + avail) & (WC_LINE - 1);
        fl[j] = (tail >= avail) ? 0u : avail - tail;
        nl[j] = fl[j] ? (((cf[j] & (WC_LINE - 1)) + fl[j] + WC_LINE - 1) >> 3) : 0u;
        sm.pend[d] = avail - fl[j];
        sm.cflush[d] = cf[j] + fl[j];
      }
    }
    u32 running = 0;
#pragma unroll
    for (int j = 0; j < DPL; j++) {
      const u32 d = (u32)j * kWave + lane;
      const u32 v = (nl[j] << 16) | cnt[j];
      const u32 incl = wave_incl_scan_u32(v, lane);
      const u32 sc = running + incl - v;
      running += (u32)__builtin_amdgcn_readlane((int)incl, 63);
      if (d < D) {
        const u32 loff = sc >> 16;
        sm.tile_off[d] = sc & 0xFFFFu;
        if constexpr (Smem::HAS_CF_TILE) sm.cf_tile[d] = cf[j];
        sm.plan[d] = (fl[j] << 8) | pd[j];
        sm.line_off[d] = loff;
        for (u32 l = 0; l < nl[j]; l++) sm.line_tab[loff + l] = (u16)d;
      }
    }
    if (lane == 0) sm.total_lines = running >> 16;
  }
#else
  {
    u32 cnt = 0, nl = 0, pd = 0, cf = 0, fl = 0;
    if ((u32)tid < D) {
#pragma unroll
      for (int k = 0; k < WAVES; k++) {
        u32 c = sm.wcnt[k][tid];
        sm.wcnt[k][tid] = (u16)cnt;
        cnt += c;
      }
      pd = sm.pend[tid];
      cf = sm.cflush[tid];
      u32 avail = pd + cnt;
      if (LIMIT && cf + avail > limit((u32)tid)) {
        *ovf = true;
        avail = 0;
        pd = 0;
      }
      const u32 tail = (cf + avail) & (WC_LINE - 1);
      fl = (tail >= avail) ? 0u : avail - tail;
      nl = fl ? (((cf & (WC_LINE - 1)) + fl + WC_LINE - 1) >> 3) : 0u;
      sm.pend[tid] = avail - fl;
      sm.cflush[tid] = cf + fl;
    }
    u32 tot;
    const u32 sc = block_excl_scan_u32<THREADS, false>((nl << 16) | cnt, sm.scratch, &tot);
    if ((u32)tid < D) {
      const u32 loff = sc >> 16;
      sm.tile_off[tid] = sc & 0xFFFFu;
      if constexpr (Smem::HAS_CF_TILE) sm.cf_tile[tid] = cf;
      sm.plan[tid] = (fl << 8) | pd;
      sm.line_off[tid] = loff;
      for (u32 l = 0; l < nl; l++) sm.line_tab[loff + l] = (u16)tid;
    }
    if (tid == 0) sm.total_lines = tot >> 16;
  }
#endif
  WC_MARK(3);
  lds_barrier();
  WC_MARK(4);

#pragma unroll
  for (int r = 0; r < WC_ITEMS; r++) {
    if (ALLVALID || wbase + r * 64 < tile_n) {
      const u32 d = dr[r] >> 16;
      sm.stage[sm.tile_off[d] + sm.wcnt[w][d] + (dr[r] & 0xFFFFu)] = t[r];
    }
  }
  WC_MARK(5);
  prefetch();
  WC_MARK(12);
  lds_barrier();
  WC_MARK(6);

  {
    const u32 TL = sm.total_lines, k = (u32)tid & (WC_LINE - 1);
    for (u32 L = (u32)tid >> 3; L < TL; L += THREADS / WC_LINE) {
      const u32 d = sm.line_tab[L];
      const u32 pl = sm.plan[d], fl = pl >> 8, pd = pl & 0xFFu;
      u32 cfd;
      if constexpr (Smem::HAS_CF_TILE) cfd = sm.cf_tile[d];
      else cfd = sm.cflush[d] - fl;
      const u32 grow = (cfd & ~(u32)(WC_LINE - 1)) + (L - sm.line_off[d]) * WC_LINE + k;
      const u32 j = grow - cfd;
      if (j < fl) store_stream(&out[grow], (j < pd) ? sm.carry[d][j] : sm.stage[sm.tile_off[d] + j - pd]);
    }
  }
  u64 keep_k[WC_ITEMS], keep_v[WC_ITEMS];
  u32 has = 0;
#pragma unroll
  for (int q = 0; q < WC_ITEMS; q++) {
    const u32 s = q * THREADS + tid, d = s >> 3, k = s & (WC_LINE - 1);
    u32 idx = 0;
    if (d < D && k < sm.pend[d]) {
      const u32 pl = sm.plan[d], fl = pl >> 8, pd = pl & 0xFFu;
      if (fl != 0 || k >= pd) {
        idx = sm.tile_off[d] + (fl ? fl - pd + k : k - pd);
        has |= 1u << q;
      }
    }
    const Tup kv = sm.stage[idx];
    keep_k[q] = kv.key;
    keep_v[q] = kv.val;
  }
  WC_MARK(7);
  lds_barrier();
  WC_MARK(8);
#pragma unroll
  for (int q = 0; q < WC_ITEMS; q++) {
    const u32 s = q * THREADS + tid;
    if (has & (1u << q)) {
      Tup kv;
      kv.key = keep_k[q];
      kv.val = keep_v[q];
      sm.carry[s >> 3][s & (WC_LINE - 1)] = kv;
    }
  }
#if HMJ_WC_NOBAR5
  {
    constexpr int ZR = MAXD * 8 / 16;
    Tup z;
    z.key = 0;
    z.val = 0;
#pragma unroll
    for (int r = 0; r < ZR / kWave; r++) sm.stage[w * ZR + r * kWave + lane] = z;
    u32* wz = reinterpret_cast<u32*>(&sm.wcnt[w][0]);
#pragma unroll
    for (int r = 0; r < MAXD / 2 / kWave; r++) wz[r * kWave + lane] = 0;
  }
  WC_MARK(9);
  WC_MARK(10);
#else
#pragma unroll
  for (int r = 0; r < WC_ITEMS; r++) {
    if (r * THREADS < Smem::ZROWS) {
      Tup z;
      z.key = 0;
      z.val = 0;
      sm.stage[r * THREADS + tid] = z;
    }
  }
  for (int i = tid; i < WAVES * MAXD / 2; i += THREADS) reinterpret_cast<u32*>(&sm.wcnt[0][0])[i] = 0;
  WC_MARK(9);
  lds_barrier();
  WC_MARK(10);
#endif
}

template <int THREADS, int MAXD>
__device__ __forceinline__ void wc_flush_carry(WcSmem<THREADS, MAXD>& sm, Tup* __restrict__ out, u32 D) {
  const int tid = threadIdx.x;
  lds_barrier();
#pragma unroll
  for (int q = 0; q < WC_ITEMS; q++) {
    const u32 s = q * THREADS + tid, d = s >> 3, k = s & (WC_LINE - 1);
    if (d < D && k < sm.pend[d]) store_stream(&out[sm.cflush[d] + k], sm.carry[d][k]);
  }
}

template <int THREADS, int MAXD>
__device__ __forceinline__ void wc_clear(WcSmem<THREADS, MAXD>& sm) {
  constexpr int WAVES = WcSmem<THREADS, MAXD>::WAVES;
  const int tid = threadIdx.x;
  for (int i = tid; i < WAVES * MAXD / 2; i += THREADS) reinterpret_cast<u32*>(&sm.wcnt[0][0])[i] = 0;
  for (int i = tid; i < WAVES * MAXD; i += THREADS) (&sm.lanemask[0][0])[i] = 0;
}

template <int THREADS, int MAXD, bool HI, bool FULL>
__global__ __launch_bounds__(THREADS, (THREADS * (MAXD <= 256 ? 2 : 1)) / 256) void radix_scatter_wc_kernel(
    const Tup* __restrict__ in, Tup* __restrict__ out, u32 n, u32 n_full, int shift, int bits,
    u32 rows_per_block, u32 worker_base, const u32* __restrict__ hist_scanned,
    const u32* __restrict__ totals, u32 nblk, u64* __restrict__ offsets_out) {
  typedef WcSmem<THREADS, MAXD> Smem;
  constexpr int TILE = Smem::TILE;
  extern __shared__ __attribute__((aligned(16))) unsigned char smem_raw[];
  Smem& sm = *reinterpret_cast<Smem*>(smem_raw);
  const u32 D = 1u << bits, mask = D - 1;
  const int tid = threadIdx.x, lane = tid & 63, w = tid >> 6;
  const u32 worker = worker_base + blockIdx.x;

  {
    u32 t = ((u32)tid < D) ? totals[tid] : 0, tot;
    u32 base = block_excl_scan_u32<THREADS>(t, sm.scratch, &tot);
    if ((u32)tid < D) {
      sm.cflush[tid] = base + hist_scanned[(u64)tid * nblk + worker];
      sm.pend[tid] = 0;
      if (offsets_out && worker == 0) {
        offsets_out[tid] = base;
        if ((u32)tid == D - 1) offsets_out[D] = n;
      }
    }
    wc_clear(sm);
  }
  __syncthreads();

// ... 10 lines not shown
  const u32 wbase = (u32)w * (WC_ITEMS * 64) + lane;

  Tup t[WC_ITEMS];
#pragma unroll
  for (int r = 0; r < WC_ITEMS; r++)
    if (FULL || begin + wbase + r * 64 < end) t[r] = load_stream(&in[begin + wbase + r * 64]);

  bool ovf = false;
#ifdef HMJ_STAMPS
  WcStamps stamps = {};
#endif
  for (u64 tile = begin; tile < end; tile += TILE) {
    const u32 tile_n = FULL ? (u32)TILE : (u32)(end - tile);
    wc_tile<THREADS, MAXD, HI, FULL, false>(
        sm, t, tile_n, out, shift, mask, D,
        [&]() {
          if (FULL && tile + TILE < end) {
            const Tup* src = in + tile + TILE;
#pragma unroll
            for (int r = 0; r < WC_ITEMS; r++) t[r] = load_stream(&src[wbase + r * 64]);
          }
        },
        NoLimit(), &ovf WC_STAMP_PASS);
  }
  wc_flush_carry(sm, out, D);
#ifdef HMJ_STAMPS
  stamps.flush();
#endif
}

struct NoXform {
  static constexpr bool kStrided = false;
};
template <int THREADS, int MAXD, bool HI, typename Xform>
__device__ __forceinline__ void slab_a_body(const Tup* __restrict__ in, u32 n, int shift, int bits, u32 rows_per_worker,
                                            Tup* __restrict__ slab, u32 CA, u32 WA, u32* __restrict__ cnt_out,
                                            u64* __restrict__ accum, u32 worker_base, Xform& xf) {
  typedef WcSmem<THREADS, MAXD> Smem;
  constexpr int TILE = Smem::TILE;
  extern __shared__ __attribute__((aligned(16))) unsigned char smem_raw[];
  Smem& sm = *reinterpret_cast<Smem*>(smem_raw);
  const u32 D = 1u << bits, mask = D - 1;
  const int tid = threadIdx.x, lane = tid & 63, w = tid >> 6;
  const u32 worker = worker_base + blockIdx.x;
  const auto limit = [=](u32 d) { return (d * WA + worker) * CA + CA; };
  if ((u32)tid < D) {
    sm.cflush[tid] = ((u32)tid * WA + worker) * CA;
    sm.pend[tid] = 0;
  }
  wc_clear(sm);
  __syncthreads();
  const u64 begin = (u64)worker * rows_per_worker;
  u64 end = begin + rows_per_worker;
  if (end > n) end = n;
  const u32 wbase = (u32)w * (WC_ITEMS * 64) + lane;
  bool ovf = false;
#ifdef HMJ_STAMPS
  WcStamps stamps = {};
#endif
  if constexpr (Xform::kStrided) {
    constexpr u32 CH = RANK_PASS_CHUNK_ROWS, IPC = CH / 64, CPT = TILE / CH;
    static_assert(WC_ITEMS % IPC == 0 && IPC >= 1, "a wave's rows of a tile are whole chunks");
    const u64 n_chunks = ((u64)n + CH - 1) / CH, whole_chunks = n / CH;
    const u32 tail = n % CH;
    const u32 slot = (u32)(((u64)worker * xf.slot_mult) % WA);
    const u64 my_whole = whole_chunks > slot ? (whole_chunks - slot + WA - 1) / WA : 0;
    auto chunk_of = [&](u64 k, u32 c) { return (k * CPT + c) * WA + slot; };
    auto rows_of = [&](u64 k) {
      const u64 first = k * CPT;
      const u32 nv = my_whole > first ? (u32)((my_whole - first < CPT) ? my_whole - first : CPT) : 0u;
      return nv * CH + ((nv < CPT && tail && chunk_of(k, nv) == whole_chunks) ? tail : 0u);
// ... 16 lines not shown
        xf(t, tile_n, wbase);
        if (HMJ_WC_FULLTILE && tile_n == (u32)TILE)
          wc_tile<THREADS, MAXD, HI, true, true>(sm, t, tile_n, slab, shift, mask, D, prefetch, limit, &ovf WC_STAMP_PASS);
        else
          wc_tile<THREADS, MAXD, HI, false, true>(sm, t, tile_n, slab, shift, mask, D, prefetch, limit, &ovf WC_STAMP_PASS);
      }
      wc_flush_carry(sm, slab, D);
    }
  } else if (begin < end) {
    Tup t[WC_ITEMS];
    {
      const u32 tn = (u32)((end - begin < TILE) ? end - begin : TILE);
#pragma unroll
      for (int r = 0; r < WC_ITEMS; r++) {
        const u32 q = wbase + r * 64;
        t[r] = load_stream(&in[begin + (q < tn ? q : tn - 1)]);
      }
    }
    for (u64 tile = begin; tile < end; tile += TILE) {
      const u32 tile_n = (u32)((end - tile < TILE) ? end - tile : TILE);
      auto prefetch = [&]() {
        if (tile + TILE < end) {
          const u64 nt = tile + TILE;
          const u32 tn = (u32)((end - nt < TILE) ? end - nt : TILE);
          const Tup* src = in + nt;
#pragma unroll
          for (int r = 0; r < WC_ITEMS; r++) {
            const u32 q = wbase + r * 64;
            t[r] = load_stream(&src[q < tn ? q : tn - 1]);
          }
        }
      };
      if constexpr (!std::is_same<Xform, NoXform>::value) xf(t, tile_n, wbase);
      if (HMJ_WC_FULLTILE && tile_n == (u32)TILE)
        wc_tile<THREADS, MAXD, HI, true, true>(sm, t, tile_n, slab, shift, mask, D, prefetch, limit, &ovf WC_STAMP_PASS);
      else
        wc_tile<THREADS, MAXD, HI, false, true>(sm, t, tile_n, slab, shift, mask, D, prefetch, limit, &ovf WC_STAMP_PASS);
    }
    wc_flush_carry(sm, slab, D);
  }
  if ((u32)tid < D) cnt_out[(u32)tid * WA + worker] = sm.cflush[tid] + sm.pend[tid] - ((u32)tid * WA + worker) * CA;
  if (ovf) atomicOr(&accum[ACC_ERR], ERR_SLAB);
#ifdef HMJ_STAMPS
  stamps.flush();
#endif
}

#ifndef HMJ_B_ADDR
#define HMJ_B_ADDR 2
#endif
#ifndef HMJ_B_NT
#define HMJ_B_NT 0
#endif
#ifdef HMJ_DEV
__device__ u32 g_b_ablate;
static bool g_b_addr_alt = false;
#endif
constexpr int SLAB_MAXSEG = 512;

template <int THREADS, int MAXD, bool HI, int ADDR>
__global__ __launch_bounds__(THREADS, (THREADS * (MAXD <= 256 ? 2 : 1)) / 256) void radix_slab_b_kernel(
    const Tup* __restrict__ slab_a, const u32* __restrict__ cnt_a, u32 CA, u32 WA, int bits_a, int shift,
    int bits, Tup* __restrict__ slab_b, u32 CB, u32* __restrict__ cnt_b, u64* __restrict__ accum, u32 KB) {
  typedef WcSmem<THREADS, MAXD> Smem;
  constexpr int TILE = Smem::TILE;
  static_assert(SLAB_MAXSEG <= THREADS, "one A-slab count per thread in the prologue scan");
  extern __shared__ __attribute__((aligned(16))) unsigned char smem_raw[];
  Smem& sm = *reinterpret_cast<Smem*>(smem_raw);
  u32* pre = reinterpret_cast<u32*>(smem_raw + sizeof(Smem));
  const u32 D = 1u << bits, mask = D - 1;
  const int tid = threadIdx.x, lane = tid & 63, w = tid >> 6;
  const u32 dA = blockIdx.x / KB, k = blockIdx.x % KB;
  const auto limit = [=](u32 d) { return (((d << bits_a) | dA) * KB + k) * CB + CB; };
  const u32 w0 = (u32)((u64)k * WA / KB), w1 = (u32)((u64)(k + 1) * WA / KB), ns = w1 - w0;
  {
    const u32 c = ((u32)tid < ns) ? cnt_a[dA * WA + w0 + tid] : 0;
    u32 tot;
    const u32 ex = block_excl_scan_u32<THREADS>(c, sm.scratch, &tot);
    if ((u32)tid < ns) pre[tid] = ex;
    if (tid == 0) pre[ns] = tot;
    if ((u32)tid < D) {
      sm.cflush[tid] = ((((u32)tid << bits_a) | dA) * KB + k) * CB;
      sm.pend[tid] = 0;
    }
    wc_clear(sm);
  }
  __syncthreads();
  const u32 total = pre[ns];
#ifdef HMJ_DEV
  const u32 abl = g_b_ablate;
#else
  constexpr u32 abl = 0;
#endif
  const u32 wbase = (u32)w * (WC_ITEMS * 64) + lane;
  (void)wbase;
  const Tup* __restrict__ bucket = slab_a + (u64)(dA * WA + w0) * CA;
  bool ovf = false;
#ifdef HMJ_STAMPS
  WcStamps stamps = {};
  stamps.base = 16;
#endif
  if (total) {
    Tup t[WC_ITEMS];
    if constexpr (ADDR != 0) {
    u32 d_s0 = 0, d_b0 = 0, d_b1 = 0, d_b2 = 0, d_b3 = 0;
    const float slabs_per_row = (float)ns / (float)total;
    auto plan1 = [&](u32 tile_begin) {
      u32 q0 = tile_begin + (u32)w * (WC_ITEMS * 64) + (u32)(lane & 3) * 64;
      q0 = q0 < total ? q0 : total - 1;
      u32 g = (u32)((float)q0 * slabs_per_row);
      g = g < ns ? g : ns - 1;
      u32 lo = g >= 3 ? g - 3 : 0;
      u32 pw[8];
#pragma unroll
      for (int i = 0; i < 8; i++) pw[i] = pre[lo + i < ns ? lo + i : ns];
      u32 j = 0;
#pragma unroll
      for (int i = 1; i < 8; i++) j += pw[i] <= q0 ? 1u : 0u;
      const bool bracketed = pw[0] <= q0 && pw[7] > q0;
      lo += j;
      if (__any(!bracketed)) {
        u32 hi = ns;
        lo = 0;
#pragma unroll
        for (int it = 0; it < 9; it++) {
          const u32 mid = (lo + hi) >> 1;
          const bool le = pre[mid] <= q0, act = hi - lo > 1;
          lo = (act && le) ? mid : lo;
          hi = (act && !le) ? mid : hi;
        }
      }
      d_s0 = lo;
      d_b0 = pre[lo];
      d_b1 = pre[lo + 1 < ns ? lo + 1 : ns];
      d_b2 = pre[lo + 2 < ns ? lo + 2 : ns];
      d_b3 = pre[lo + 3 < ns ? lo + 3 : ns];
// ... 53 lines not shown
      u64 m = __ballot(win_v <= q0);
      u32 j = (u32)__popcll(m) - 1;
      if (!(m & 1) || j > 59) {
        u32 g = (u32)__builtin_amdgcn_readfirstlane((int)(u32)((float)q0 * slabs_per_row));
        g = g < ns ? g : ns - 1;
        win_lo = g >= 8 ? g - 8 : 0;
        win_v = pre[win_lo + (u32)lane < ns ? win_lo + (u32)lane : ns];
        m = __ballot(win_v <= q0);
        j = (u32)__popcll(m) - 1;
        if (!(m & 1) || j > 59) {
          u32 lo = 0, hi = ns;
#pragma unroll
          for (int it = 0; it < 9; it++) {
            const u32 mid = (lo + hi) >> 1;
            const bool le = pre[mid] <= q0, act = hi - lo > 1;
            lo = (act && le) ? mid : lo;
            hi = (act && !le) ? mid : hi;
          }
          win_lo = (u32)__builtin_amdgcn_readfirstlane((int)lo);
          win_v = pre[win_lo + (u32)lane < ns ? win_lo + (u32)lane : ns];
          m = __ballot(win_v <= q0);
          j = (u32)__popcll(m) - 1;
          j = j > 59 ? 59 : j;
        }
      }
      u_s0 = win_lo + j;
      u_b0 = (u32)__builtin_amdgcn_readlane((int)win_v, (int)j);
      u_b1 = (u32)__builtin_amdgcn_readlane((int)win_v, (int)j + 1);
      u_b2 = (u32)__builtin_amdgcn_readlane((int)win_v, (int)j + 2);
      u_b3 = (u32)__builtin_amdgcn_readlane((int)win_v, (int)j + 3);
      u_b4 = (u32)__builtin_amdgcn_readlane((int)win_v, (int)j + 4);
    };
    auto issue2 = [&](u32 tile_begin) {
      u64 off[WC_ITEMS];
      const u32 wq0 = tile_begin + wq;
      u32 wlast = wq0 + WC_ITEMS * 64 - 1;
      wlast = wlast < total ? wlast : total - 1;
      if (abl == 4) {
#pragma unroll
        for (int r = 0; r < WC_ITEMS; r++) {
          u32 q = wq0 + lane + r * 64;
          off[r] = q < total ? q : total - 1;
        }
      } else if (u_b1 > wlast) {
        const u64 o0 = (u64)u_s0 * CA;
#pragma unroll
        for (int r = 0; r < WC_ITEMS; r++) {
          u32 q = wq0 + lane + r * 64;
          q = q < total ? q : total - 1;
          off[r] = o0 + (q - u_b0);
        }
      } else if (u_b4 > wlast) {
#pragma unroll
        for (int r = 0; r < WC_ITEMS; r++) {
          u32 q = wq0 + lane + r * 64;
          q = q < total ? q : total - 1;
          const u32 j = (q >= u_b1 ? 1u : 0u) + (q >= u_b2 ? 1u : 0u) + (q >= u_b3 ? 1u : 0u);
          const u32 base = j == 0 ? u_b0 : (j == 1 ? u_b1 : (j == 2 ? u_b2 : u_b3));
          off[r] = (u64)(u_s0 + j) * CA + (q - base);
        }
      } else {
#pragma unroll
        for (int r = 0; r < WC_ITEMS; r++) {
          u32 q = wq0 + lane + r * 64;
          q = q < total ? q : total - 1;
          u32 sx = u_s0;
          while (sx + 1 < ns && pre[sx + 1] <= q) sx++;
          off[r] = (u64)sx * CA + (q - pre[sx]);
        }
      }
#pragma unroll
      for (int r = 0; r < WC_ITEMS; r++) t[r] = HMJ_B_NT ? load_stream(&bucket[off[r]]) : bucket[off[r]];
    };
    auto plan = [&](u32 tb) {
      if constexpr (ADDR == 2) plan2(tb); else plan1(tb);
    };
    auto issue = [&](u32 tb) {
      if constexpr (ADDR == 2) issue2(tb); else issue1(tb);
    };
    if (abl != 4) plan(0);
    issue(0);
    if ((u32)TILE < total && abl != 4) plan(TILE);
    for (u32 tile = 0; tile < total; tile += TILE) {
      const u32 tile_n = (total - tile < (u32)TILE) ? total - tile : (u32)TILE;
      auto prefetch = [&]() {
        if (tile + TILE < total) {
          issue(tile + TILE);
#ifdef HMJ_STAMPS
          stamps.mark(13);
#endif
          if (tile + 2 * TILE < total && abl != 4) plan(tile + 2 * TILE);
        }
      };
#ifdef HMJ_DEV
      if (abl == 1 || abl == 4) {
#pragma unroll
        for (int r = 0; r < WC_ITEMS; r++)
          if (t[r].key == 0) t[r].key = (u64)(tile + (u32)tid + r * THREADS + blockIdx.x * 7919u + 1) * 0x9E3779B97F4A7C15ull;
      }
#endif
      if (HMJ_WC_FULLTILE && tile_n == (u32)TILE)
        wc_tile<THREADS, MAXD, HI, true, true>(sm, t, tile_n, slab_b, shift, mask, D, prefetch, limit, &ovf WC_STAMP_PASS);
      else
        wc_tile<THREADS, MAXD, HI, false, true>(sm, t, tile_n, slab_b, shift, mask, D, prefetch, limit, &ovf WC_STAMP_PASS);
    }
    } else {
    u32 seg = 0;
    auto load = [&](u32 tile_begin) {
      const u32 tn = (total - tile_begin < (u32)TILE) ? total - tile_begin : (u32)TILE;
      while (seg + 1 < ns && pre[seg + 1] <= tile_begin) seg++;
      u32 s = seg;
      u64 off[WC_ITEMS];
#pragma unroll
      for (int r = 0; r < WC_ITEMS; r++) {
        u32 q = wbase + r * 64;
        q = tile_begin + (q < tn ? q : tn - 1);
        while (s + 1 < ns && pre[s + 1] <= q) s++;
        off[r] = (u64)s * CA + (q - pre[s]);
      }
#pragma unroll
      for (int r = 0; r < WC_ITEMS; r++) t[r] = HMJ_B_NT ? load_stream(&bucket[off[r]]) : bucket[off[r]];
    };
    load(0);
    for (u32 tile = 0; tile < total; tile += TILE) {
      const u32 tile_n = (total - tile < (u32)TILE) ? total - tile : (u32)TILE;
      wc_tile<THREADS, MAXD, HI, false, true>(
          sm, t, tile_n, slab_b, shift, mask, D,
          [&]() {
            if (tile + TILE < total) load(tile + TILE);
          },
          limit, &ovf WC_STAMP_PASS);
// ... 98 lines not shown
    atomicMax(&rng[1], (unsigned long long)mx);
  }
  if (eq_r) atomicAdd(&same[0], eq_r);
  if (eq_s) atomicAdd(&same[1], eq_s);
  if (up_r) atomicAdd(&order[0], up_r);
  if (dn_r) atomicAdd(&order[1], dn_r);
  if (up_s) atomicAdd(&order[2], up_s);
  if (dn_s) atomicAdd(&order[3], dn_s);
  __syncthreads();
  {
    const u64 lo = rng[0], span = rng[1] - rng[0];
#pragma unroll
    for (int k = 0; k < 2; k++)
      if (myvalid[k] && span) atomicAdd(&bins[(u32)((mykey[k] - lo) / ((span >> 6) + 1)) & 63u], 1u);
  }
  __syncthreads();
  if (tid == 0) {
    out[0] = acc;
    out[1] = ref;
    out[2] = (u64)same[0] | ((u64)order[0] << 16) | ((u64)order[1] << 32);
    out[3] = (u64)same[1] | ((u64)order[2] << 16) | ((u64)order[3] << 32);
    out[4] = rng[0];
    out[5] = rng[1];
    u32 nonempty = 0, big = 0;
    for (int i = 0; i < 64; i++) {
      nonempty += bins[i] ? 1u : 0u;
      big = bins[i] > big ? bins[i] : big;
    }
    out[6] = nonempty;
    out[7] = big;
  }
}

template <int THREADS, int MAXD, bool HI>
__global__ __launch_bounds__(THREADS, (THREADS * (MAXD <= 256 ? 2 : 1)) / 256) void radix_slab_a_kernel(
    const Tup* __restrict__ in, u32 n, int shift, int bits, u32 rows_per_worker, Tup* __restrict__ slab,
    u32 CA, u32 WA, u32* __restrict__ cnt_out, u64* __restrict__ accum, u32 worker_base) {
  NoXform xf;
  slab_a_body<THREADS, MAXD, HI, NoXform>(in, n, shift, bits, rows_per_worker, slab, CA, WA, cnt_out, accum, worker_base, xf);
}

template <bool CUT>
struct RankXform {
  static constexpr bool kStrided = CUT;
  u32 slot_mult;
  const Tup* __restrict__ tab;
  u32 mask;
  int hshift;
  int tb, pre;
  u64 svmin, svrange, mult;
  u64 acc_s;
  u64 n_rows;
  bool miss;
  __device__ __forceinline__ void operator()(Tup (&t)[WC_ITEMS], u32 tile_n, u32 wbase) {
    u32 slot[WC_ITEMS];
    bool live[WC_ITEMS], want[WC_ITEMS];
    u32 found = 0;
#pragma unroll
    for (int r = 0; r < WC_ITEMS; r++) {
      want[r] = wbase + (u32)r * 64 < tile_n;
      slot[r] = gt_hash(t[r].key, hshift);
      if (want[r]) acc_s += t[r].val;
      if (want[r]) n_rows++;
      live[r] = want[r] && t[r].key != GT_EMPTY;
    }
    u64 rank[WC_ITEMS] = {};
    gt_walk<WC_ITEMS>(tab, mask, slot, live, [&](int r, const Tup& e) {
      const bool eq = e.key == t[r].key;
      if (eq) {
        rank[r] = e.val;
        found |= 1u << r;
      }
// ... 10 lines not shown
        t[r].key = rank[r];
      }
    }
  }
};
template <int THREADS, int MAXD, bool CUT>
__global__ __launch_bounds__(THREADS, (THREADS * (MAXD <= 256 ? 2 : 1)) / 256) void radix_slab_a_rank_kernel(
    const Tup* __restrict__ in, u32 n, int shift, int bits, u32 rows_per_worker, Tup* __restrict__ slab, u32 CA, u32 WA,
    u32* __restrict__ cnt_out, u64* __restrict__ accum, const Tup* __restrict__ tab, int log_cap, bool extra, int tb, u64 svmin, u64 svrange,
    int pre, u64 mult, u32 slot_mult) {
  RankXform<CUT> xf{slot_mult, tab, (1u << log_cap) - 1, 64 - log_cap, tb, pre, svmin, svrange, mult, 0ull, 0ull, false};
  slab_a_body<THREADS, MAXD, false, RankXform<CUT>>(in, n, shift, bits, rows_per_worker, slab, CA, WA, cnt_out, accum, 0u, xf);
  __shared__ u64 wsum[THREADS / kWave], wrows[THREADS / kWave];
  const int lane = threadIdx.x & 63, wv = threadIdx.x >> 6;
  const u64 ws = wave_sum_u64(xf.acc_s), wr = wave_sum_u64(xf.n_rows);
  const bool any_miss = __any(xf.miss);
  if (lane == 0) {
    wsum[wv] = ws;
    wrows[wv] = wr;
  }
  if (any_miss && lane == 0) atomicOr(reinterpret_cast<unsigned long long*>(&accum[ACC_ERR]), (unsigned long long)ERR_FASTPATH);
  __syncthreads();
  if (threadIdx.x == 0) {
    u64 tot = 0, rows = 0;
    for (int w = 0; w < THREADS / kWave; w++) {
      tot += wsum[w];
      rows += wrows[w];
    }
    if (tot) atomicAdd(reinterpret_cast<unsigned long long*>(&accum[ACC_SUM_S]), (unsigned long long)tot);
    if (extra && tot) atomicAdd(reinterpret_cast<unsigned long long*>(&accum[ACC_SUM_P]), (unsigned long long)tot);
    if (rows) atomicAdd(reinterpret_cast<unsigned long long*>(&accum[ACC_N]), (unsigned long long)rows);
  }
}
template <int THREADS, int MAXD, bool HI>
static hipError_t launch_slab_a_t(const void* in, u32 n, int shift, int bits, u32 rpw, void* slab, u32 CA,
                                  u32 WA, u32* cnt, u64* accum, hipStream_t st, u32 w_begin, u32 w_end) {
  typedef WcSmem<THREADS, MAXD> Smem;
  const size_t smem = sizeof(Smem);
  static_assert(sizeof(Smem) <= 160 * 1024, "slab pass A: LDS");
  static SmemAttrOnce attr_once;
  if (hipError_t e = ensure_max_smem(attr_once, reinterpret_cast<const void*>(radix_slab_a_kernel<THREADS, MAXD, HI>), (size_t)smem); e != hipSuccess) return e;
  if (w_end > WA) w_end = WA;
  if (w_begin >= w_end) return hipSuccess;
  hipLaunchKernelGGL((radix_slab_a_kernel<THREADS, MAXD, HI>), dim3(w_end - w_begin), dim3(THREADS), smem, st,
                     static_cast<const Tup*>(in), n, shift, bits, rpw, static_cast<Tup*>(slab), CA, WA, cnt,
                     accum, w_begin);
  return hipGetLastError();
}

template <int THREADS, int MAXD, bool HI>
static hipError_t launch_slab_b_t(const void* slab_a, const u32* cnt_a, u32 CA, u32 WA, int bits_a, int shift,
                                  int bits, void* slab_b, u32 CB, u32* cnt_b, u64* accum, hipStream_t st, u32 KB) {
  typedef WcSmem<THREADS, MAXD> Smem;
  const size_t smem = sizeof(Smem) + (SLAB_MAXSEG + 1) * sizeof(u32);
  static_assert(sizeof(Smem) + (SLAB_MAXSEG + 1) * sizeof(u32) <= 160 * 1024, "slab pass B: LDS");
#ifdef HMJ_DEV
  if (g_b_addr_alt) {
    constexpr int ALT = HMJ_B_ADDR == 2 ? 1 : 2;
    static SmemAttrOnce attr_alt;
    if (hipError_t e = ensure_max_smem(attr_alt, reinterpret_cast<const void*>(radix_slab_b_kernel<THREADS, MAXD, HI, ALT>), (size_t)smem); e != hipSuccess) return e;
    hipLaunchKernelGGL((radix_slab_b_kernel<THREADS, MAXD, HI, ALT>), dim3((1u << bits_a) * KB), dim3(THREADS), smem, st,
                       static_cast<const Tup*>(slab_a), cnt_a, CA, WA, bits_a, shift, bits,
                       static_cast<Tup*>(slab_b), CB, cnt_b, accum, KB);
    return hipGetLastError();
  }
#endif
  static SmemAttrOnce attr_once;
  if (hipError_t e = ensure_max_smem(attr_once, reinterpret_cast<const void*>(radix_slab_b_kernel<THREADS, MAXD, HI, HMJ_B_ADDR>), (size_t)smem); e != hipSuccess) return e;
  hipLaunchKernelGGL((radix_slab_b_kernel<THREADS, MAXD, HI, HMJ_B_ADDR>), dim3((1u << bits_a) * KB), dim3(THREADS), smem, st,
                     static_cast<const Tup*>(slab_a), cnt_a, CA, WA, bits_a, shift, bits,
                     static_cast<Tup*>(slab_b), CB, cnt_b, accum, KB);
  return hipGetLastError();
}

static u32 slab_cap(double mean, double fan) {
  double c = mean + 8.0 * __builtin_sqrt(fan * mean) + 24.0;
  return ((u32)c + 8) & ~7u;
}
u32 slab_capacity(double mean, double fan) { return slab_cap(mean, fan < 1.0 ? 1.0 : fan); }
bool slab_geometry(u32 n, int bits_a, int bits_b, SlabGeom* g, u32 kb, double fan, double density) {
  if (bits_a < 1 || bits_a > SLAB_MAX_BITS || bits_b < 1 || bits_b > SLAB_MAX_BITS) return false;
  const u32 tile = bits_a > 8 ? 4096 : 2048;
  u64 tiles = ((u64)n + tile - 1) / tile;
  u64 max_workers = 2048;
#ifdef HMJ_DEV
  if (const char* e = getenv("HMJ_SLAB_WORKERS")) max_workers = (u64)atoi(e) > 0 ? (u64)atoi(e) : max_workers;
#endif
  u64 tpw = (tiles + max_workers - 1) / max_workers;
  if (tpw == 0) tpw = 1;
  g->WA = (u32)((tiles + tpw - 1) / tpw);
  g->rpw = (u32)(tpw * tile);
  if (kb == 0) kb = SLAB_KB;
  g->KB = kb;
  if (g->WA < kb || (g->WA + kb - 1) / kb > (u32)SLAB_MAXSEG) return false;
  if (fan < 1.0) fan = 1.0;
  if (density < 1.0) density = 1.0;
  const double fan_a = 1.0 + 4.0 * (double)g->rpw * fan / (double)(n ? n : 1);
  g->CA = slab_cap(density * (double)g->rpw / (double)(1u << bits_a), fan_a < fan ? fan_a : fan);
  g->CB = slab_cap(density * (double)n / (double)(1u << bits_a) / (double)kb / (double)(1u << bits_b), fan);
  const u64 rows_a = (u64)(1u << bits_a) * g->WA * g->CA;
  const u64 rows_b = (u64)(1u << (bits_a + bits_b)) * kb * g->CB;
  g->rows_a = rows_a;
  g->rows_b = rows_b;
  return rows_a < 0xFFFFFFF0ull && rows_b < 0xFFFFFFF0ull;
}

bool slab_geometry_one_pass(u32 n, int bits, double keys_per_digit, u32 max_workers, SlabGeom* g, double density) {
  if (bits < 1 || bits > SLAB_MAX_BITS || max_workers == 0) return false;
  const u32 tile = bits > 8 ? 4096 : 2048;
  const u64 tiles = ((u64)n + tile - 1) / tile;
  u64 tpw = (tiles + max_workers - 1) / max_workers;
  if (tpw == 0) tpw = 1;
  g->WA = (u32)((tiles + tpw - 1) / tpw);
  g->rpw = (u32)(tpw * tile);
  g->KB = 0;
  g->CB = 0;
  g->rows_b = 0;
  if (density < 1.0) density = 1.0;
  const double mean = density * (double)g->rpw / (double)(1u << bits);
  if (keys_per_digit < 1.0) keys_per_digit = 1.0;
  g->CA = slab_cap(mean, 1.0 + mean / keys_per_digit);
  g->rows_a = (u64)(1u << bits) * g->WA * g->CA;
  return g->WA >= 1 && g->rows_a < 0xFFFFFFF0ull;
}

hipError_t launch_slab_a(const void* in, u32 n, int shift, int bits, const SlabGeom& g, void* slab_a, u64 slab_a_rows,
                         u32* cnt_a, u64 cnt_a_n, u64* accum, hipStream_t st, u32 w_begin, u32 w_end) {
  if (bits < 1 || bits > SLAB_MAX_BITS || g.WA == 0 || g.CA == 0 || (u64)g.WA * g.rpw < n) return hipErrorInvalidValue;
  if (slab_a_rows < ((u64)g.WA << bits) * g.CA || cnt_a_n < ((u64)g.WA << bits)) return hipErrorInvalidValue;
  if (((u64)g.WA << bits) * g.CA >= 0xFFFFFFF0ull) return hipErrorInvalidValue;
  const bool hi = shift >= 32;
#define HMJ_SLAB_A(T, M, H) launch_slab_a_t<T, M, H>(in, n, shift, bits, g.rpw, slab_a, g.CA, g.WA, cnt_a, accum, st, w_begin, w_end)
  if (bits > 8) return hi ? HMJ_SLAB_A(1024, 512, true) : HMJ_SLAB_A(1024, 512, false);
  return hi ? HMJ_SLAB_A(512, 256, true) : HMJ_SLAB_A(512, 256, false);
#undef HMJ_SLAB_A
}

hipError_t launch_slab_a_ranks(const void* in, u32 n, int shift, int bits, const SlabGeom& g, void* slab_a, u64 slab_a_rows, u32* cnt_a,
                               u64 cnt_a_n, u64* accum, const void* tab, int log_cap, bool extra, int tb, u64 svmin, u64 svrange, int pre,
                               u64 mult, hipStream_t st) {
  if (bits < 1 || bits > SLAB_MAX_BITS || g.WA == 0 || g.CA == 0 || (u64)g.WA * g.rpw < n || !tab || log_cap < 4 || log_cap > 30 || tb < 0 ||
      tb > 16 || pre < 0 || pre > 32 || shift < 0 || shift > 4 || (shift && tb))
    return hipErrorInvalidValue;
  if (slab_a_rows < ((u64)g.WA << bits) * g.CA || cnt_a_n < ((u64)g.WA << bits)) return hipErrorInvalidValue;
  if (((u64)g.WA << bits) * g.CA >= 0xFFFFFFF0ull) return hipErrorInvalidValue;
  u32 slot_mult = 1;
  if (tb > 0 && g.WA > 2) {
    auto gcd = [](u32 a, u32 b) {
      while (b) {
        const u32 t = a % b;
        a = b;
        b = t;
      }
      return a;
    };
    slot_mult = (u32)((double)g.WA * 0.6180339887498949);
    if (slot_mult < 1) slot_mult = 1;
    while (gcd(slot_mult, g.WA) != 1) slot_mult++;
  }
#define HMJ_SLAB_AR(T, M, C)                                                                                                          \
  {                                                                                                                                   \
    typedef WcSmem<T, M> Smem;                                                                                                        \
    static SmemAttrOnce once;                                                                                                         \
    if (hipError_t e = ensure_max_smem(once, reinterpret_cast<const void*>(radix_slab_a_rank_kernel<T, M, C>), sizeof(Smem)); e != hipSuccess) \
      return e;                                                                                                                       \
    hipLaunchKernelGGL((radix_slab_a_rank_kernel<T, M, C>), dim3(g.WA), dim3(T), sizeof(Smem), st, static_cast<const Tup*>(in), n, shift, bits, g.rpw, \
                       static_cast<Tup*>(slab_a), g.CA, g.WA, cnt_a, accum, static_cast<const Tup*>(tab), log_cap, extra, tb, svmin, svrange, pre, mult, \
                       slot_mult);                                                                                                    \
  }
  if (tb > 0) {
    if (bits > 8) HMJ_SLAB_AR(1024, 512, true) else HMJ_SLAB_AR(512, 256, true)
  } else {
    if (bits > 8) HMJ_SLAB_AR(1024, 512, false) else HMJ_SLAB_AR(512, 256, false)
  }
#undef HMJ_SLAB_AR
  return hipGetLastError();
}

hipError_t launch_slab_b(const void* slab_a, const u32* cnt_a, int bits_a, int shift, int bits,
                         const SlabGeom& g, void* slab_b, u64 slab_b_rows, u32* cnt_b, u64 cnt_b_n, u64* accum, hipStream_t st) {
  if (bits < 1 || bits > SLAB_MAX_BITS || bits_a < 1 || bits_a > SLAB_MAX_BITS || g.KB == 0 || g.WA < g.KB ||
      (g.WA + g.KB - 1) / g.KB > (u32)SLAB_MAXSEG)
    return hipErrorInvalidValue;
  const u64 pieces = ((u64)g.KB << (bits_a + bits));
  if (slab_b_rows < pieces * g.CB || cnt_b_n < pieces || pieces * g.CB >= 0xFFFFFFF0ull) return hipErrorInvalidValue;
  const bool hi = shift >= 32;
#define HMJ_SLAB_B(T, M, H) launch_slab_b_t<T, M, H>(slab_a, cnt_a, g.CA, g.WA, bits_a, shift, bits, slab_b, g.CB, cnt_b, accum, st, g.KB)
  if (bits > 8) return hi ? HMJ_SLAB_B(1024, 512, true) : HMJ_SLAB_B(1024, 512, false);
  return hi ? HMJ_SLAB_B(512, 256, true) : HMJ_SLAB_B(512, 256, false);
#undef HMJ_SLAB_B
}

__global__ __launch_bounds__(256) void key_exact_kernel(const Tup* __restrict__ R, u32 nb, const Tup* __restrict__ S, u32 np,
                                                        u64 ref, bool ref_is_first_key, u64* __restrict__ out) {
  if (ref_is_first_key) ref = nb ? R[0].key : (np ? S[0].key : 0);
  u64 x = 0, mn = ~0ull, mx = 0;
  const u64 stride = (u64)gridDim.x * blockDim.x;
  for (u64 i = (u64)blockIdx.x * blockDim.x + threadIdx.x; i < nb; i += stride) {
    const u64 k = R[i].key;
    x |= k ^ ref;
    mn = k < mn ? k : mn;
    mx = k > mx ? k : mx;
  }
  for (u64 i = (u64)blockIdx.x * blockDim.x + threadIdx.x; i < np; i += stride) x |= S[i].key ^ ref;
#pragma unroll
  for (int o = kWave / 2; o > 0; o >>= 1) {
    x |= __shfl_xor(x, o, kWave);
    const u64 a2 = __shfl_xor(mn, o, kWave), b2 = __shfl_xor(mx, o, kWave);
    mn = a2 < mn ? a2 : mn;
    mx = b2 > mx ? b2 : mx;
  }
  __shared__ u64 wx[4], wmn[4], wmx[4];
  if ((threadIdx.x & 63) == 0) {
    wx[threadIdx.x >> 6] = x;
    wmn[threadIdx.x >> 6] = mn;
    wmx[threadIdx.x >> 6] = mx;
  }
  __syncthreads();
  if (threadIdx.x == 0) {
    for (int w = 1; w < 4; w++) {
// ... 230 lines not shown
```

### include/hmj.h

```cpp
#ifndef HMJ_H
#define HMJ_H

#include <stddef.h>
#include <stdint.h>

#ifdef __cplusplus
extern "C" {
#endif

typedef struct hmj_ctx hmj_ctx;

#define HMJ_OK 0
#define HMJ_E_ARG (-1)
#define HMJ_E_NODEV (-2)
#define HMJ_E_OOM (-3)
#define HMJ_E_HIP (-4)
#define HMJ_E_UNSUPPORTED (-5)

#define HMJ_E_RCCL (-6)
#define HMJ_E_PEER (-7)
#define HMJ_E_TIMEOUT (-8)

#define HMJ_MATERIALIZE 0x01u
#define HMJ_ORDERED 0x02u
// ... 37 lines not shown
  int32_t key_prefix_bits;
  int32_t key_window_low;
  uint32_t n_probe_items;
  float ms_scatter_pass[2];
} hmj_timing;
#define HMJ_PATH_SLAB 0x001u
#define HMJ_PATH_EXACT 0x002u
#define HMJ_PATH_UNIQ_WRITE 0x004u
#define HMJ_PATH_SPLIT 0x008u
#define HMJ_PATH_WINDOW 0x010u
#define HMJ_PATH_ORDER_DEFERRED 0x020u
#define HMJ_PATH_ORDER_BY_KEY 0x040u
#define HMJ_PATH_PREPARED 0x080u
#define HMJ_PATH_CHUNKED_BUILD 0x100u
#define HMJ_PATH_HOT_KEY_HINT 0x200u
#define HMJ_PATH_SLAB_PROBE 0x400u
#define HMJ_PATH_SORTED_WRITE 0x800u
#define HMJ_PATH_SORTED_FK 0x1000u
#define HMJ_PATH_DENSE_BUILD 0x2000u
#define HMJ_PATH_SORTED_FK_HALF 0x8000u
#define HMJ_PATH_SORTED_FK_WIDE 0x20000u
#define HMJ_PATH_LOOKBACK_TIMEOUT 0x10000u
#define HMJ_PATH_PRESORTED 0x40000u
#define HMJ_PATH_SLAB_ONE_PASS 0x80000u
#define HMJ_PATH_ORDER_BY_RANK_SORT 0x200000u
#define HMJ_PATH_RANK_RUNS 0x1000000u
#define HMJ_PATH_RANK_LOOKUP_IN_PASS 0x2000000u
#define HMJ_PATH_SORT_MSD 0x4000000u
#define HMJ_PATH_KEY_RANGES 0x8000000u
#define HMJ_PATH_ORDERED_EXPANSION 0x400000u
#define HMJ_PATH_LDS_TABLE 0x800000u
#define HMJ_PATH_GLOBAL_TABLE 0x100000u
#define HMJ_PATH_HOST_PIPELINE 0x4000u

typedef struct {
  uint32_t struct_size;
  uint32_t path;
  int32_t radix_bits, radix_passes, pass_bits[4];
  int32_t key_prefix_bits, key_window_low;
  uint32_t n_partitions;
  uint32_t probe_items;
  uint32_t attempts;
  uint32_t refused;
  uint32_t cooling;
  uint64_t workload;
} hmj_plan_desc;
#define HMJ_REFUSED_GTABLE_SHAPE 0x0001u
#define HMJ_REFUSED_GTABLE_COOLING 0x0002u
#define HMJ_REFUSED_GTABLE_GAVE_UP 0x0004u
#define HMJ_REFUSED_RANK_SORT_MODEL 0x0008u
#define HMJ_REFUSED_RANK_SORT_COOLING 0x0010u
#define HMJ_REFUSED_RANK_SORT_GAVE_UP 0x0020u
#define HMJ_REFUSED_SLAB_SHAPE 0x0040u
#define HMJ_REFUSED_SLAB_COOLING 0x0080u
#define HMJ_REFUSED_SLAB_SORTED_INPUT 0x0100u
#define HMJ_REFUSED_SLAB_OVERFLOW 0x0200u
#define HMJ_REFUSED_FAST_WRITE_COOLING 0x0400u
#define HMJ_REFUSED_FAST_WRITE_GAVE_UP 0x0800u
#define HMJ_REFUSED_SLAB_PROBE_COOLING 0x1000u
#define HMJ_REFUSED_SLAB_PROBE_OVERFLOW 0x2000u
#define HMJ_REFUSED_PREFIX_VIOLATED 0x4000u
#define HMJ_REFUSED_EXPANSION_GAVE_UP 0x8000u
#define HMJ_COOL_UNIQ_WRITE 0x001u
#define HMJ_COOL_SORTED_WRITE 0x002u
#define HMJ_COOL_GTABLE 0x004u
#define HMJ_COOL_GTABLE_WRITE 0x008u
#define HMJ_COOL_RANK_SORT 0x010u
#define HMJ_COOL_RANK_SORT_SLAB 0x020u
#define HMJ_COOL_EXPANSION 0x040u
#define HMJ_COOL_SORT_SLAB 0x080u
#define HMJ_COOL_SLAB 0x100u
#define HMJ_COOL_SLAB_PROBE 0x200u
#define HMJ_COOL_ONE_PASS_WRITE 0x400u
#define HMJ_COOL_EXACT_PREFIX 0x800u
#define HMJ_COOL_RANK_RUNS 0x1000u
#define HMJ_COOL_SORT_MSD 0x2000u

int hmj_create(hmj_ctx** out, int device_id);
void hmj_destroy(hmj_ctx* ctx);
#define HMJ_STREAM_OWN ((void*)(intptr_t)-1)
int hmj_set_stream(hmj_ctx* ctx, void* hip_stream);
int hmj_reserve(hmj_ctx* ctx, uint64_t n_build, uint64_t n_probe, uint64_t max_matches,
                uint32_t flags);
int hmj_set_radix_bits(hmj_ctx* ctx, int total_bits);
int hmj_autotune_radix_bits(hmj_ctx* ctx, uint64_t n_build, uint64_t n_probe, int apply, int* best_bits,
                            double ms[3]);
int hmj_set_key_prefix_bits(hmj_ctx* ctx, int bits);
int hmj_plan(uint64_t n_build, int* total_bits, int* n_passes, int pass_bits[4]);
#define HMJ_ABI_VERSION 5
int hmj_abi_version(void);
#define HMJ_PLACE_MAX_CAND 4
typedef struct {
  char name[16];
  uint64_t bytes;
  float fill_TBps;
  int candidates;
  float ms_search;
  int searched;
  int aborted;
  float budget_ms;
  float cand_ms_alloc[HMJ_PLACE_MAX_CAND];
  float cand_ms_fill[HMJ_PLACE_MAX_CAND];
  float cand_TBps[HMJ_PLACE_MAX_CAND];
} hmj_place_info;
int hmj_placement_info(hmj_ctx* ctx, hmj_place_info* out, int max_entries);
int hmj_last_plan(hmj_ctx* ctx, hmj_plan_desc* out);
int hmj_forget_workloads(hmj_ctx* ctx);
int hmj_set_profiling(hmj_ctx* ctx, int enabled);
int hmj_last_timing(hmj_ctx* ctx, hmj_timing* out);
// ... 506 lines not shown
```

Before: 34.24 billion.

## Scatter probe side as key-only slabs when every probe row matches exactly one build row

Adds a key-only probe path. When the join has no flags, the probe side is partitioned as 8-byte keys instead of 16-byte tuples through both slab passes, and a count kernel that reads key pairs checks that each probe key has exactly one build match. A sampled pilot kernel decides whether to try it, and per-workload clean/dirty/cooldown state caches that decision. The goal is to roughly halve probe-side scatter and probe traffic. If any probe row fails the one-match check, the whole probe side is redone with full rows, which wastes the key-only work.

Measured after the change: 36.60 billion, median of 6. 1.07x the previous value.

```diff
diff --git a/hashmergejoin_amd/_lib.py b/hashmergejoin_amd/_lib.py
--- a/hashmergejoin_amd/_lib.py
+++ b/hashmergejoin_amd/_lib.py
@@ -31,6 +31,7 @@
 HMJ_PATH_LOOKBACK_TIMEOUT = 0x10000
 HMJ_PATH_SORTED_FK_WIDE = 0x20000
 HMJ_PATH_PRESORTED = 0x40000
+HMJ_PATH_PROBE_KEYS = 0x10000000
 
 _HERE = os.path.dirname(os.path.abspath(__file__))
 _U64P = C.POINTER(C.c_uint64)
@@ -320,10 +321,12 @@
 HMJ_REFUSED_FAST_WRITE_COOLING, HMJ_REFUSED_FAST_WRITE_GAVE_UP = 0x400, 0x800
 HMJ_REFUSED_SLAB_PROBE_COOLING, HMJ_REFUSED_SLAB_PROBE_OVERFLOW = 0x1000, 0x2000
 HMJ_REFUSED_PREFIX_VIOLATED, HMJ_REFUSED_EXPANSION_GAVE_UP = 0x4000, 0x8000
+HMJ_REFUSED_PROBE_KEYS_GAVE_UP, HMJ_REFUSED_PROBE_KEYS_COOLING = 0x10000, 0x20000
 HMJ_COOL_UNIQ_WRITE, HMJ_COOL_SORTED_WRITE, HMJ_COOL_GTABLE, HMJ_COOL_GTABLE_WRITE = 0x1, 0x2, 0x4, 0x8
 HMJ_COOL_RANK_SORT, HMJ_COOL_RANK_SORT_SLAB, HMJ_COOL_EXPANSION, HMJ_COOL_SORT_SLAB = 0x10, 0x20, 0x40, 0x80
 HMJ_COOL_SLAB, HMJ_COOL_SLAB_PROBE, HMJ_COOL_ONE_PASS_WRITE, HMJ_COOL_EXACT_PREFIX = 0x100, 0x200, 0x400, 0x800
 HMJ_COOL_RANK_RUNS, HMJ_COOL_SORT_MSD = 0x1000, 0x2000
+HMJ_COOL_PROBE_KEYS = 0x4000
 
 
 HMJ_PLACE_MAX_CAND = 4
diff --git a/hashmergejoin_amd/csrc/api.hip b/hashmergejoin_amd/csrc/api.hip
--- a/hashmergejoin_amd/csrc/api.hip
+++ b/hashmergejoin_amd/csrc/api.hip
@@ -85,7 +85,8 @@
          (gtable_sort_slab_cooldown ? HMJ_COOL_RANK_SORT_SLAB : 0u) | (expand_cooldown ? HMJ_COOL_EXPANSION : 0u) |
          (sort_slab_cooldown ? HMJ_COOL_SORT_SLAB : 0u) | (slab_cooldown ? HMJ_COOL_SLAB : 0u) | (slab_probe_cooldown ? HMJ_COOL_SLAB_PROBE : 0u) |
          (one_pass_write_cooldown ? HMJ_COOL_ONE_PASS_WRITE : 0u) | (exact_prefix_joins ? HMJ_COOL_EXACT_PREFIX : 0u) |
-         (rank_runs_cooldown ? HMJ_COOL_RANK_RUNS : 0u) | (sort_msd_cooldown ? HMJ_COOL_SORT_MSD : 0u);
+         (rank_runs_cooldown ? HMJ_COOL_RANK_RUNS : 0u) | (sort_msd_cooldown ? HMJ_COOL_SORT_MSD : 0u) |
+         (probe_keys_cooldown ? HMJ_COOL_PROBE_KEYS : 0u);
 }
 
 int wait_arrival(hmj_ctx* c, hipEvent_t ev) {
@@ -576,9 +577,10 @@
   return a;
 }
 
-static int slab_pass_a(hmj_ctx* c, const void* in, u32 n, int rel, int low, int bits, const hmj::SlabGeom& g, bool arriving) {
+static int slab_pass_a(hmj_ctx* c, const void* in, u32 n, int rel, int low, int bits, const hmj::SlabGeom& g, bool arriving,
+                       bool keys = false) {
   u64* acc = (u64*)c->accum.p;
-  const u64 a_rows = c->slab_a.cap / 16, a_cnt = c->cnt_a.cap / 4;
+  const u64 a_rows = c->slab_a.cap / (keys ? 8 : 16), a_cnt = c->cnt_a.cap / 4;
   const int sp = span_begin(c, K_SCATTER, rel, 0);
   if (arriving) {
     u32 w_done = 0;
@@ -592,20 +594,20 @@
       }
     }
   } else {
-    HIP_TRY(hmj::launch_slab_a(in, n, low, bits, g, c->slab_a.p, a_rows, (u32*)c->cnt_a.p, a_cnt, acc, c->stream));
+    HIP_TRY(hmj::launch_slab_a(in, n, low, bits, g, c->slab_a.p, a_rows, (u32*)c->cnt_a.p, a_cnt, acc, c->stream, 0, 0xFFFFFFFFu, keys));
   }
   span_end(c, sp);
-  c->timing.bytes_scatter += 32ull * n;
+  c->timing.bytes_scatter += (keys ? 24ull : 32ull) * n;
   return HMJ_OK;
 }
 static int slab_passes(hmj_ctx* c, const void* in, u32 n, int rel, int low, int ba, int bb, const hmj::SlabGeom& g, DevBuf& sb,
-                       DevBuf& cb, bool arriving) {
-  RC_TRY(slab_pass_a(c, in, n, rel, low, ba, g, arriving));
+                       DevBuf& cb, bool arriving, bool keys = false) {
+  RC_TRY(slab_pass_a(c, in, n, rel, low, ba, g, arriving, keys));
   const int sp = span_begin(c, K_SCATTER, rel, 1);
-  HIP_TRY(hmj::launch_slab_b(c->slab_a.p, (const u32*)c->cnt_a.p, ba, low + ba, bb, g, sb.p, sb.cap / 16, (u32*)cb.p, cb.cap / 4,
-                             (u64*)c->accum.p, c->stream));
+  HIP_TRY(hmj::launch_slab_b(c->slab_a.p, (const u32*)c->cnt_a.p, ba, low + ba, bb, g, sb.p, sb.cap / (keys ? 8 : 16), (u32*)cb.p,
+                             cb.cap / 4, (u64*)c->accum.p, c->stream, keys));
   span_end(c, sp);
-  c->timing.bytes_scatter += 32ull * n;
+  c->timing.bytes_scatter += (keys ? 16ull : 32ull) * n;
   return HMJ_OK;
 }
 
@@ -1192,9 +1194,57 @@
   RC_TRY(ensure_dev(c, c->slab_bs, gs.rows_b * 16));
   RC_TRY(ensure_dev(c, c->cnt_br, (size_t)P * gr.KB * 4));
   RC_TRY(ensure_dev(c, c->cnt_bs, (size_t)P * gs.KB * 4));
+  namespace pk = hmj_host;
+  const pk::ProbeKeysVerdict keys_verdict =
+      pk::probe_keys_decide(pk::ProbeKeysState{c->probe_keys_mode, c->probe_keys_min_log2, c->wm->probe_keys_cooldown,
+                                               c->wm->probe_keys_clean, c->wm->probe_keys_dirty},
+                            pk::ProbeKeysJoin{j.flags, (u64)np, {ba, bb}, c->prepare_only, !c->arrive_ev.empty()});
   if (!reuse) RC_TRY(slab_passes(c, j.R, nb, 0, p.low, ba, bb, gr, c->slab_br, c->cnt_br, false));
+  u64* hh;
+  bool probe_keys = keys_verdict == pk::ProbeKeysVerdict::Attempt;
+  if (keys_verdict == pk::ProbeKeysVerdict::Pilot) {
+    HIP_TRY(hmj::launch_probe_keys_pilot(j.S, np, c->slab_br.p, (const u32*)c->cnt_br.p, gr.CB, p.low, ba + bb, (u64*)c->accum.p,
+                                         c->stream));
+    RC_TRY(read_accum(c, &hh));
+    if (hh[hmj::ACC_ERR] & hmj::ERR_SLAB) {
+      c->wm->slab_cooldown = 8;
+      return kRetryNoSlab;
+    }
+    probe_keys = !(hh[hmj::ACC_ERR] & hmj::ERR_PROBE_PILOT);
+    if (!probe_keys) {
+      c->wm->probe_keys_dirty = true;
+      c->wm->probe_keys_dirty_age = 0;
+    }
+  }
+  if (probe_keys) {
+    hmj::SlabGeom gk = gs;
+    gk.CA = pk::probe_keys_slab_cap(gs.CA);
+    gk.CB = pk::probe_keys_slab_cap(gs.CB);
+    RC_TRY(slab_passes(c, j.S, np, 1, p.low, ba, bb, gk, c->slab_bs, c->cnt_bs, false, true));
+    hmj::ProbeArgs ka = slab_probe_args(c, &gr, nullptr, c->slab_bs, c->cnt_bs, gk.CB, P, 1);
+    ka.s_rows = c->slab_bs.cap / 8;
+    const int sp = span_begin(c, K_PROBE_COUNT, -1);
+    HIP_TRY(hmj::launch_probe_count_slab_keys(ka, c->num_cus, c->stream));
+    span_end(c, sp);
+    c->timing.bytes_probe_count += 16ull * nb + 8ull * np;
+    RC_TRY(read_accum(c, &hh));
+    if (hh[hmj::ACC_ERR] & hmj::ERR_SLAB) {
+      c->wm->slab_cooldown = 8;
+      return kRetryNoSlab;
+    }
+    if (!(hh[hmj::ACC_ERR] & hmj::ERR_PROBE_KEYS)) {
+      c->wm->probe_keys_clean = true;
+      c->timing.path |= HMJ_PATH_PROBE_KEYS;
+      result_sums(j.out, hh);
+      return HMJ_OK;
+    }
+    c->plan.refused |= HMJ_REFUSED_PROBE_KEYS_GAVE_UP;
+    c->wm->probe_keys_clean = false;
+    c->wm->probe_keys_cooldown = pk::kProbeKeysCooldown;
+    if (c->trace) std::fprintf(stderr, "[hmj]   key-only probe side gave up (a probe row without exactly one build row) -> whole rows\n");
+    HIP_TRY(hipMemsetAsync(c->accum.p, 0, 8 * sizeof(u64), c->stream));
+  }
   if (!c->prepare_only) RC_TRY(slab_passes(c, j.S, np, 1, p.low, ba, bb, gs, c->slab_bs, c->cnt_bs, !c->arrive_ev.empty()));
-  u64* hh;
   if (c->prepare_only) {
     RC_TRY(read_accum(c, &hh));
     if (hh[hmj::ACC_ERR] & hmj::ERR_SLAB) {
@@ -1224,11 +1274,17 @@
     HIP_TRY(hmj::launch_probe_count_slab(sa, c->num_cus, c->stream));
   }
   span_end(c, sp);
-  c->timing.bytes_probe_count = 16ull * ((u64)nb + np);
+  c->timing.bytes_probe_count += 16ull * ((u64)nb + np);
   RC_TRY(read_accum(c, &hh));
   if (hh[hmj::ACC_ERR] & hmj::ERR_SLAB) {
     c->wm->slab_cooldown = 8;
     return kRetryNoSlab;
+  }
+  if (keys_verdict == pk::ProbeKeysVerdict::SkipCooling) {
+    c->plan.refused |= HMJ_REFUSED_PROBE_KEYS_COOLING;
+    c->wm->probe_keys_cooldown--;
+  } else if (keys_verdict == pk::ProbeKeysVerdict::SkipDirty && ++c->wm->probe_keys_dirty_age >= pk::kProbeKeysDirtyJoins) {
+    c->wm->probe_keys_dirty = false;
   }
   result_sums(j.out, hh);
   return HMJ_OK;
@@ -2591,6 +2647,11 @@
     const int l = atoi(e);
     if (l >= 16 && l <= 31) c->slab_min_rows = 1u << l;
   }
+  if (const char* e = getenv("HMJ_PROBE_KEYS")) c->probe_keys_mode = atoi(e) == 0 ? 0 : atoi(e) == 1 ? 1 : -1;
+  if (const char* e = getenv("HMJ_PROBE_KEYS_MIN_LOG2")) {
+    const int l = atoi(e);
+    if (l >= hmj_host::kProbeKeysMinLog2Floor && l <= 31) c->probe_keys_min_log2 = l;
+  }
   if (const char* e = getenv("HMJ_SLAB_PROBE_KB")) {
     const int k = atoi(e);
     if (k >= 1 && k <= 512) c->slab_probe_kb = (u32)k;
diff --git a/hashmergejoin_amd/csrc/hmj_ctx.h b/hashmergejoin_amd/csrc/hmj_ctx.h
--- a/hashmergejoin_amd/csrc/hmj_ctx.h
+++ b/hashmergejoin_amd/csrc/hmj_ctx.h
@@ -9,6 +9,7 @@
 #include "hmj_args.h"
 #include "hmj_dev.h"
 #include "hmj_launch.h"
+#include "hmj_probekeys.h"
 #include "hmj_smallplan.h"
 
 struct hmj_comm;
@@ -183,6 +184,10 @@
   int slab_cooldown = 0;
   int slab_probe_cooldown = 0;
   int one_pass_write_cooldown = 0;
+  int probe_keys_cooldown = 0;
+  bool probe_keys_clean = false;
+  bool probe_keys_dirty = false;
+  int probe_keys_dirty_age = 0;
   int exact_prefix_joins = 0;
   uint32_t cooling() const;
 };
@@ -291,6 +296,8 @@
   bool sort_slab = true;
   u64 sort_slab_min = 1ull << 25;
   int slab_mode = 1;
+  int probe_keys_mode = hmj_host::kProbeKeysModeDefault;
+  int probe_keys_min_log2 = hmj_host::kProbeKeysMinLog2Default;
   bool staged_upload = false;
   bool host_pipeline = true;
   hipStream_t copy_stream = nullptr;
diff --git a/hashmergejoin_amd/csrc/hmj_dev.h b/hashmergejoin_amd/csrc/hmj_dev.h
--- a/hashmergejoin_amd/csrc/hmj_dev.h
+++ b/hashmergejoin_amd/csrc/hmj_dev.h
@@ -107,6 +107,8 @@
 constexpr u64 ERR_FASTPATH = 8;
 constexpr u64 ERR_GTABLE = 128;
 constexpr u64 ERR_PREFIX = 4;
+constexpr u64 ERR_PROBE_KEYS = 1ull << 16;
+constexpr u64 ERR_PROBE_PILOT = 1ull << 17;
 
 __device__ __forceinline__ u64 mix64(u64 x) {
   x ^= x >> 30;
diff --git a/hashmergejoin_amd/csrc/hmj_launch.h b/hashmergejoin_amd/csrc/hmj_launch.h
--- a/hashmergejoin_amd/csrc/hmj_launch.h
+++ b/hashmergejoin_amd/csrc/hmj_launch.h
@@ -50,9 +50,11 @@
 bool slab_geometry_one_pass(u32 n, int bits, double keys_per_digit, u32 max_workers, SlabGeom* g, double density = 1.0);
 u32 slab_capacity(double mean, double fan);
 hipError_t launch_slab_a(const void* in, u32 n, int shift, int bits, const SlabGeom& g, void* slab_a, u64 slab_a_rows,
-                         u32* cnt_a, u64 cnt_a_n, u64* accum, hipStream_t st, u32 w_begin = 0, u32 w_end = 0xFFFFFFFFu);
+                         u32* cnt_a, u64 cnt_a_n, u64* accum, hipStream_t st, u32 w_begin = 0, u32 w_end = 0xFFFFFFFFu,
+                         bool keys = false);
 hipError_t launch_slab_b(const void* slab_a, const u32* cnt_a, int bits_a, int shift, int bits,
-                         const SlabGeom& g, void* slab_b, u64 slab_b_rows, u32* cnt_b, u64 cnt_b_n, u64* accum, hipStream_t st);
+                         const SlabGeom& g, void* slab_b, u64 slab_b_rows, u32* cnt_b, u64 cnt_b_n, u64* accum, hipStream_t st,
+                         bool keys = false);
 hipError_t launch_key_sample(const void* R, u32 nb, const void* S, u32 np, u64* out, hipStream_t st);
 hipError_t launch_key_exact(const void* R, u32 nb, const void* S, u32 np, u64 ref, u64* out, int num_cus, hipStream_t st,
                             bool ref_is_first_key = false);
@@ -93,6 +95,9 @@
 hipError_t launch_probe(const ProbeArgs& a, int mode, bool first_wins, bool extra, int grid,
                         hipStream_t st);
 int probe_default_grid(int num_cus);
+hipError_t launch_probe_count_slab_keys(const ProbeArgs& a, int num_cus, hipStream_t st);
+hipError_t launch_probe_keys_pilot(const void* S, u32 np, const void* slab_br, const u32* cnt_br, u32 r_cap, int low, int bits,
+                                   u64* accum, hipStream_t st);
 hipError_t launch_probe_kind(const ProbeArgs& a, int mode, int kind, bool first_wins, u64 fill, int grid, hipStream_t st);
 hipError_t launch_probe_build_kind(const ProbeArgs& a, int mode, int kind, u64 fill, u32* bmark, int grid, hipStream_t st);
 hipError_t launch_build_sweep(const ProbeArgs& a, const u32* r_off, u32 P, const u32* vstart, u64* sweep_n, int mode,
diff --git a/hashmergejoin_amd/csrc/hmj_probekeys.h b/hashmergejoin_amd/csrc/hmj_probekeys.h
--- /dev/null
+++ b/hashmergejoin_amd/csrc/hmj_probekeys.h
@@ -0,0 +1,64 @@
+#pragma once
+#include <cstdint>
+
+#if defined(__HIPCC__) || defined(__CUDACC__)
+#define HMJ_PK_HD __host__ __device__
+#else
+#define HMJ_PK_HD
+#endif
+
+namespace hmj_host {
+
+#ifndef HMJ_PROBE_KEYS_DEFAULT
+#define HMJ_PROBE_KEYS_DEFAULT -1
+#endif
+constexpr int kProbeKeysModeDefault = HMJ_PROBE_KEYS_DEFAULT;
+constexpr uint32_t kProbeKeysPilotRows = 4096;
+constexpr int kProbeKeysMinLog2Default = 25;
+constexpr int kProbeKeysMinLog2Floor = 16;
+constexpr int kProbeKeysCooldown = 8;
+constexpr int kProbeKeysDirtyJoins = 64;
+constexpr int kProbeKeysMaxPassBits = 8;
+
+HMJ_PK_HD inline uint32_t probe_keys_sample_count(uint64_t np) { return np < kProbeKeysPilotRows ? (uint32_t)np : kProbeKeysPilotRows; }
+HMJ_PK_HD inline uint64_t probe_keys_sample_index(uint32_t i, uint64_t np) {
+  return np < kProbeKeysPilotRows ? (uint64_t)i : (uint64_t)i * np / kProbeKeysPilotRows;
+}
+
+struct ProbeKeysState {
+  int mode;
+  int min_log2;
+  int cooldown;
+  bool clean;
+  bool dirty;
+};
+struct ProbeKeysJoin {
+  uint32_t flags;
+  uint64_t np;
+  int pass_bits[2];
+  bool prepare_only;
+  bool arriving;
+};
+enum class ProbeKeysVerdict {
+  SkipShape,
+  SkipOff,
+  SkipCooling,
+  SkipDirty,
+  Pilot,
+  Attempt
+};
+inline ProbeKeysVerdict probe_keys_decide(const ProbeKeysState& s, const ProbeKeysJoin& j) {
+  if (j.flags != 0 || j.prepare_only || j.arriving || j.np == 0) return ProbeKeysVerdict::SkipShape;
+  if (j.pass_bits[0] < 1 || j.pass_bits[0] > kProbeKeysMaxPassBits || j.pass_bits[1] < 1 || j.pass_bits[1] > kProbeKeysMaxPassBits)
+    return ProbeKeysVerdict::SkipShape;
+  if (s.min_log2 < 0 || s.min_log2 > 63 || j.np < (1ull << s.min_log2)) return ProbeKeysVerdict::SkipShape;
+  if (s.mode == 0) return ProbeKeysVerdict::SkipOff;
+  if (s.cooldown > 0) return ProbeKeysVerdict::SkipCooling;
+  if (s.mode == 1 || s.clean) return ProbeKeysVerdict::Attempt;
+  if (s.dirty) return ProbeKeysVerdict::SkipDirty;
+  return ProbeKeysVerdict::Pilot;
+}
+
+HMJ_PK_HD inline uint32_t probe_keys_slab_cap(uint32_t cap) { return (cap + 15u) & ~15u; }
+
+}
diff --git a/hashmergejoin_amd/csrc/probe.hip b/hashmergejoin_amd/csrc/probe.hip
--- a/hashmergejoin_amd/csrc/probe.hip
+++ b/hashmergejoin_amd/csrc/probe.hip
@@ -1,5 +1,6 @@
 #include "hmj_dev.h"
 #include "hmj_launch.h"
+#include "hmj_probekeys.h"
 #include <type_traits>
 
 namespace hmj {
@@ -916,11 +917,15 @@
   }
 }
 
-template <int THREADS>
-__device__ __forceinline__ void fp_load_pieces(Tup (&t)[FP_ROWS], const Tup* __restrict__ base, u32 cap, u32 cnt_mine, int tid) {
+__device__ __forceinline__ u64 prow_key(const Tup& t) { return t.key; }
+__device__ __forceinline__ u64 prow_key(u64 k) { return k; }
+__device__ __forceinline__ u64 prow_val(const Tup& t) { return t.val; }
+__device__ __forceinline__ u64 prow_val(u64) { return 0; }
+template <int THREADS, typename Row>
+__device__ __forceinline__ void fp_load_pieces(Row (&t)[FP_ROWS], const Row* __restrict__ base, u32 cap, u32 cnt_mine, int tid) {
   constexpr int QT = THREADS / 4;
   const u32 g = (u32)tid / QT, l = (u32)tid % QT;
-  const Tup* __restrict__ piece = base + (u64)g * cap;
+  const Row* __restrict__ piece = base + (u64)g * cap;
   const u32 last = cnt_mine ? cnt_mine - 1 : 0;
 #pragma unroll
   for (int k = 0; k < FP_ROWS; k++) {
@@ -929,17 +934,37 @@
   }
 }
 
-template <int THREADS, int LOG_NB, bool PCOUNT, bool SLAB, int OUT>
+constexpr int FP_KEY_ROWS = 6;
+static_assert(FP_KEY_ROWS >= FP_ROWS && FP_KEY_ROWS % 2 == 0, "key pairs must cover a piece of FP_ROWS * T/4 rows");
+template <int THREADS>
+__device__ __forceinline__ void fp_load_key_pieces(u64 (&t)[FP_KEY_ROWS], const u64* __restrict__ base, u32 cap, u32 cnt_mine, int tid) {
+  constexpr int QT = THREADS / 4;
+  const u32 g = (u32)tid / QT, l = (u32)tid % QT;
+  const u64* __restrict__ piece = base + (u64)g * cap;
+  const u32 last = cnt_mine ? (cnt_mine - 1) >> 1 : 0;
+#pragma unroll
+  for (int k = 0; k < FP_KEY_ROWS / 2; k++) {
+    const u32 q = l + (u32)k * QT;
+    const u64x2_t v = *reinterpret_cast<const u64x2_t*>(piece + 2 * (u64)(q < last ? q : last));
+    t[2 * k] = v.x;
+    t[2 * k + 1] = v.y;
+  }
+}
+
+template <int THREADS, int LOG_NB, bool PCOUNT, bool SLAB, int OUT, bool PKEYS = false>
 __global__ __launch_bounds__(THREADS, 4) void probe_count_fast_kernel(
     ProbeArgs a, u32* __restrict__ irregular, u32* __restrict__ n_irregular) {
   typedef FastSmem<THREADS, LOG_NB> Smem;
+  typedef typename std::conditional<PKEYS, u64, Tup>::type PRow;
   constexpr u32 CAP = Smem::CAP, NB = 1u << LOG_NB;
   constexpr bool PIECES = SLAB && OUT == 0 && !PCOUNT && HMJ_PROBE_PIECES;
+  static_assert(!PKEYS || PIECES, "key-only probe rows: slab layout, plain count mode");
+  constexpr int PROWS = PKEYS ? FP_KEY_ROWS : FP_ROWS;
   constexpr u32 QT = THREADS / 4, PIECE_CAP = FP_ROWS * QT;
   extern __shared__ __attribute__((aligned(16))) unsigned char smem_raw[];
   Smem& sm = *reinterpret_cast<Smem*>(smem_raw);
   const Tup* __restrict__ R = static_cast<const Tup*>(a.R);
-  const Tup* __restrict__ S = static_cast<const Tup*>(a.S);
+  const PRow* __restrict__ S = static_cast<const PRow*>(a.S);
   const u32* __restrict__ r_off = a.r_off;
   const u32* __restrict__ s_off = a.s_off;
   const u32* __restrict__ r_end = (SLAB || a.r_end == nullptr) ? a.r_off + 1 : a.r_end;
@@ -947,7 +972,7 @@
   const u32 P = a.P;
   const int tid = threadIdx.x;
   u64 acc_n = 0, acc_r = 0, acc_s = 0, acc_x = 0, acc_m = 0, acc_p = 0;
-  bool pfx_bad = false, giveup = false;
+  bool pfx_bad = false, giveup = false, keys_bad = false;
   for (u32 i = tid; i < NB; i += THREADS) sm.head[i] = 0;
   if (tid < 2) sm.itemcnt[tid] = 0;
   u32 epoch = 0;
@@ -956,10 +981,14 @@
   u32 p = blockIdx.x;
   u32 rb = 0, nb = 0, sb = 0, np = 0;
   bool regular = false;
-  Tup br[FP_ROWS], pr[FP_ROWS], pq[FP_ROWS];
+  Tup br[FP_ROWS];
+  PRow pr[PROWS], pq[PROWS];
   u32 r1 = 0, r2 = 0, r3 = 0, s1 = 0, s2 = 0, s3 = 0, r1n = 0, r2n = 0, r3n = 0, s1n = 0, s2n = 0, s3n = 0;
   u32 rm = 0, sm_ = 0, rmn = 0, smn = 0;
   const u32 my_piece = (u32)tid / QT;
+  auto piece_row = [](int t_, int k) -> u32 {
+    return PKEYS ? 2u * ((u32)t_ % QT + (u32)(k >> 1) * QT) + (u32)(k & 1) : (u32)t_ % QT + (u32)k * QT;
+  };
   bool slab_bad = false;
   if (p < P) {
     if (SLAB) {
@@ -983,10 +1012,11 @@
     }
     regular = nb && np && nb <= CAP && np <= CAP;
     if (regular) {
-      if (PIECES) {
+      if constexpr (PIECES) {
         fp_load_pieces<THREADS>(br, R + (u64)p * SLAB_KB * a.r_cap, a.r_cap, rm, tid);
-        fp_load_pieces<THREADS>(pr, S + (u64)p * SLAB_KB * a.s_cap, a.s_cap, sm_, tid);
-      } else if (SLAB) {
+        if constexpr (PKEYS) fp_load_key_pieces<THREADS>(pr, S + (u64)p * SLAB_KB * a.s_cap, a.s_cap, sm_, tid);
+        else fp_load_pieces<THREADS>(pr, S + (u64)p * SLAB_KB * a.s_cap, a.s_cap, sm_, tid);
+      } else if constexpr (SLAB) {
         fp_load_slab<THREADS>(br, R + (u64)p * SLAB_KB * a.r_cap, a.r_cap, r1, r2, r3, nb, tid);
         if (OUT == 0) fp_load_slab<THREADS>(pr, S + (u64)p * SLAB_KB * a.s_cap, a.s_cap, s1, s2, s3, np, tid);
       } else {
@@ -996,6 +1026,7 @@
     }
   }
   const Tup* __restrict__ dummy = reinterpret_cast<const Tup*>(a.accum);
+  const PRow* __restrict__ dummy_p = reinterpret_cast<const PRow*>(a.accum);
   auto load_build = [&](Tup (&t)[FP_ROWS], bool ok, u32 pp, u32 rb_, u32 nb_, u32 q1, u32 q2, u32 q3, u32 mine) {
     if (PIECES)
       fp_load_pieces<THREADS>(t, ok ? R + (u64)pp * SLAB_KB * a.r_cap : dummy, ok ? a.r_cap : 0u, ok ? mine : 1u, tid);
@@ -1005,10 +1036,12 @@
     else
       fp_load<THREADS>(t, ok ? R + rb_ : dummy, ok ? nb_ : 1u, tid);
   };
-  auto load_probe = [&](Tup (&t)[FP_ROWS], bool ok, u32 pp, u32 sb_, u32 np_, u32 q1, u32 q2, u32 q3, u32 mine) {
-    if (PIECES)
-      fp_load_pieces<THREADS>(t, ok ? S + (u64)pp * SLAB_KB * a.s_cap : dummy, ok ? a.s_cap : 0u, ok ? mine : 1u, tid);
-    else if (SLAB)
+  auto load_probe = [&](PRow (&t)[PROWS], bool ok, u32 pp, u32 sb_, u32 np_, u32 q1, u32 q2, u32 q3, u32 mine) {
+    if constexpr (PKEYS)
+      fp_load_key_pieces<THREADS>(t, ok ? S + (u64)pp * SLAB_KB * a.s_cap : dummy_p, ok ? a.s_cap : 0u, ok ? mine : 1u, tid);
+    else if constexpr (PIECES)
+      fp_load_pieces<THREADS>(t, ok ? S + (u64)pp * SLAB_KB * a.s_cap : dummy_p, ok ? a.s_cap : 0u, ok ? mine : 1u, tid);
+    else if constexpr (SLAB)
       fp_load_slab<THREADS>(t, ok ? S + (u64)pp * SLAB_KB * a.s_cap : dummy, ok ? a.s_cap : 0u, ok ? q1 : 1u, ok ? q2 : 1u,
                             ok ? q3 : 1u, ok ? np_ : 1u, tid);
     else
@@ -1048,7 +1081,7 @@
       }
       regular2 = nb2 && np2 && nb2 <= CAP && np2 <= CAP;
     }
-    if (OUT == 0) {
+    if constexpr (OUT == 0) {
       load_probe(pq, regular2, pn, sb2, np2, s1n, s2n, s3n, smn);
     } else if (regular) {
       if (SLAB)
@@ -1096,45 +1129,46 @@
       lds_barrier();
       const u64 n_before = acc_n;
       if (!HMJ_ABLATE(1u)) {
-        u32 cur[FP_ROWS];
-        u32 cnt[FP_ROWS], first[FP_ROWS];
-#pragma unroll
-        for (int k = 0; k < FP_ROWS; k++) {
+        u32 cur[PROWS];
+        u32 cnt[PROWS], first[PROWS];
+#pragma unroll
+        for (int k = 0; k < PROWS; k++) {
           const u32 j = k * THREADS + tid;
           cur[k] = NIL;
           cnt[k] = 0;
           first[k] = OUT == 2 ? NIL : 0;
-          if (PIECES ? ((u32)tid % QT + (u32)k * QT < sm_) : (j < np)) {
-            if (a.pfx_shift && (pr[k].key >> a.pfx_shift) != a.pfx_val) pfx_bad = true;
-            if (OUT >= 1 && (a.extra & 1u)) acc_p += pr[k].val;
-            const u32 hv = sm.head[fast_hash<LOG_NB>(pr[k].key)];
+          if (PIECES ? (piece_row(tid, k) < sm_) : (j < np)) {
+            if (a.pfx_shift && (prow_key(pr[k]) >> a.pfx_shift) != a.pfx_val) pfx_bad = true;
+            if (OUT >= 1 && (a.extra & 1u)) acc_p += prow_val(pr[k]);
+            const u32 hv = sm.head[fast_hash<LOG_NB>(prow_key(pr[k]))];
             cur[k] = ((hv >> 16) == epoch) ? (hv & 0xFFFFu) : NIL;
           }
         }
         for (; !HMJ_ABLATE(2u);) {
           bool any = false;
 #pragma unroll
-          for (int k = 0; k < FP_ROWS; k++) any |= (cur[k] != NIL);
+          for (int k = 0; k < PROWS; k++) any |= (cur[k] != NIL);
           if (!__any(any)) break;
 #pragma unroll
-          for (int k = 0; k < FP_ROWS; k++) {
+          for (int k = 0; k < PROWS; k++) {
             if (cur[k] != NIL) {
               const u32 i = cur[k];
               const u64 kk = sm.key[i], vv = sm.val[i];
               cur[k] = sm.next[i];
-              if (kk == pr[k].key) {
+              if (kk == prow_key(pr[k])) {
                 if (OUT == 2 && (a.extra & 2u)) {
                   first[k] = i < first[k] ? i : first[k];
                 } else {
                   acc_n++;
                   acc_r += vv;
-                  acc_s += pr[k].val;
+                  acc_s += prow_val(pr[k]);
                   if (OUT == 1) {
                     if (cnt[k] == 0) first[k] = i;
                     cnt[k]++;
                   }
+                  if (PKEYS) cnt[k]++;
                   if (OUT >= 1 && (a.extra & 1u)) {
-                    const u64 m = tmix(kk, vv, pr[k].val);
+                    const u64 m = tmix(kk, vv, prow_val(pr[k]));
                     acc_x ^= m;
                     acc_m += m;
                   }
@@ -1143,6 +1177,10 @@
             }
           }
         }
+        if constexpr (PKEYS) {
+#pragma unroll
+          for (int k = 0; k < PROWS; k++) keys_bad |= piece_row(tid, k) < sm_ && cnt[k] != 1;
+        }
         if (OUT == 2 && (a.extra & 2u)) {
 #pragma unroll
           for (int k = 0; k < FP_ROWS; k++) {
@@ -1150,9 +1188,9 @@
               const u64 vv = sm.val[first[k]];
               acc_n++;
               acc_r += vv;
-              acc_s += pr[k].val;
+              acc_s += prow_val(pr[k]);
               if (a.extra & 1u) {
-                const u64 m = tmix(pr[k].key, vv, pr[k].val);
+                const u64 m = tmix(prow_key(pr[k]), vv, prow_val(pr[k]));
                 acc_x ^= m;
                 acc_m += m;
               }
@@ -1199,9 +1237,9 @@
             for (int k = 0; k < FP_ROWS; k++) {
               if (cnt[k]) {
                 const u64 d = o + ((ex >> (12 * k)) & 0xFFFu);
-                a.out_key[d] = pr[k].key;
+                a.out_key[d] = prow_key(pr[k]);
                 a.out_rval[d] = sm.val[first[k]];
-                a.out_sval[d] = pr[k].val;
+                a.out_sval[d] = prow_val(pr[k]);
               }
               const u32 tk = (u32)((tot >> (12 * k)) & 0xFFFu);
               o += tk;
@@ -1212,7 +1250,7 @@
         }
       } else {
 #pragma unroll
-        for (int k = 0; k < FP_ROWS; k++) acc_r += pr[k].key;
+        for (int k = 0; k < FP_ROWS; k++) acc_r += prow_key(pr[k]);
       }
       if (PCOUNT) {
         const u32 mine = (u32)(acc_n - n_before);
@@ -1224,16 +1262,17 @@
     } else {
       if ((PCOUNT || OUT == 1) && tid == 0 && !(nb && np)) a.part_count[p] = 0;
       if (OUT == 1 && nb && np) giveup = true;
+      if (PKEYS && np && !nb) keys_bad = true;
       if (OUT >= 1 && (a.extra & 1u) && !nb) {
         if (SLAB) {
-          const Tup* base = S + (u64)p * SLAB_KB * a.s_cap;
+          const PRow* base = S + (u64)p * SLAB_KB * a.s_cap;
           for (u32 j = tid; j < np; j += THREADS) {
             const u32 pc = (j >= s1) + (j >= s2) + (j >= s3);
             const u32 pre = pc == 0 ? 0 : pc == 1 ? s1 : pc == 2 ? s2 : s3;
-            acc_p += base[(u64)pc * a.s_cap + (j - pre)].val;
+            acc_p += prow_val(base[(u64)pc * a.s_cap + (j - pre)]);
           }
         } else {
-          for (u32 j = tid; j < np; j += THREADS) acc_p += S[sb + j].val;
+          for (u32 j = tid; j < np; j += THREADS) acc_p += prow_val(S[sb + j]);
         }
       }
       if (OUT != 1 && !SLAB && tid == 0 && nb && np) irregular[atomicAdd(n_irregular, 1u)] = p;
@@ -1241,7 +1280,7 @@
     }
     if (OUT == 0) {
 #pragma unroll
-      for (int k = 0; k < FP_ROWS; k++) pr[k] = pq[k];
+      for (int k = 0; k < PROWS; k++) pr[k] = pq[k];
     }
     p = pn; rb = rb2; nb = nb2; sb = sb2; np = np2; regular = regular2;
     r1 = r1n; r2 = r2n; r3 = r3n; s1 = s1n; s2 = s2n; s3 = s3n;
@@ -1249,6 +1288,7 @@
   }
   if (SLAB && slab_bad && tid == 0) atomicOr(&a.accum[ACC_ERR], ERR_SLAB);
   if (OUT == 1 && __any(giveup) && (tid & 63) == 0) atomicOr(&a.accum[ACC_ERR], ERR_FASTPATH);
+  if (PKEYS && __any(keys_bad) && (tid & 63) == 0) atomicOr(&a.accum[ACC_ERR], ERR_PROBE_KEYS);
   if (__any(pfx_bad) && (tid & 63) == 0) atomicOr(&a.accum[ACC_ERR], ERR_PREFIX);
   lds_barrier();
   if (PCOUNT && prev_p != 0xFFFFFFFFu && tid == 0) a.part_count[prev_p] = sm.itemcnt[parity ^ 1];
@@ -2410,15 +2450,15 @@
   return hipGetLastError();
 }
 
-template <int THREADS, int LOG_NB, bool PCOUNT, bool SLAB = false, int OUT = 0>
+template <int THREADS, int LOG_NB, bool PCOUNT, bool SLAB = false, int OUT = 0, bool PKEYS = false>
 static hipError_t launch_fast_t(const ProbeArgs& a, u32* irregular, u32* n_irregular, int grid,
                                 hipStream_t st) {
   typedef FastSmem<THREADS, LOG_NB> Smem;
   static SmemAttrOnce attr_once;
-  if (hipError_t e = ensure_max_smem(attr_once, reinterpret_cast<const void*>(probe_count_fast_kernel<THREADS, LOG_NB, PCOUNT, SLAB, OUT>), (size_t)sizeof(Smem)); e != hipSuccess) return e;
+  if (hipError_t e = ensure_max_smem(attr_once, reinterpret_cast<const void*>(probe_count_fast_kernel<THREADS, LOG_NB, PCOUNT, SLAB, OUT, PKEYS>), (size_t)sizeof(Smem)); e != hipSuccess) return e;
   if ((u32)grid > a.P) grid = (int)a.P;
   if (grid < 1) grid = 1;
-  hipLaunchKernelGGL((probe_count_fast_kernel<THREADS, LOG_NB, PCOUNT, SLAB, OUT>), dim3(grid), dim3(THREADS),
+  hipLaunchKernelGGL((probe_count_fast_kernel<THREADS, LOG_NB, PCOUNT, SLAB, OUT, PKEYS>), dim3(grid), dim3(THREADS),
                      sizeof(Smem), st, a, irregular, n_irregular);
   return hipGetLastError();
 }
@@ -2523,6 +2563,38 @@
 hipError_t launch_probe_count_slab(const ProbeArgs& a, int num_cus, hipStream_t st) {
   if (!slab_operands_ok(a)) return hipErrorInvalidValue;
   return launch_fast_t<1024, BIG_LOG_NB, false, true>(a, nullptr, nullptr, num_cus * 4, st);
+}
+
+hipError_t launch_probe_count_slab_keys(const ProbeArgs& a, int num_cus, hipStream_t st) {
+  if (!slab_operands_ok(a) || a.pfx_shift) return hipErrorInvalidValue;
+  return launch_fast_t<1024, BIG_LOG_NB, false, true, 0, true>(a, nullptr, nullptr, num_cus * 4, st);
+}
+
+__global__ __launch_bounds__(256) void probe_keys_pilot_kernel(const Tup* __restrict__ S, u32 np, const Tup* __restrict__ R,
+                                                              const u32* __restrict__ r_cnt, u32 r_cap, int low, u32 pmask,
+                                                              u64* __restrict__ accum) {
+  const u32 wave = (blockIdx.x * blockDim.x + threadIdx.x) >> 6, lane = threadIdx.x & 63;
+  if (wave >= hmj_host::probe_keys_sample_count(np)) return;
+  const u64 key = S[hmj_host::probe_keys_sample_index(wave, np)].key;
+  const u32 p = (u32)(key >> low) & pmask;
+  u32 hits = 0;
+#pragma unroll
+  for (int j = 0; j < SLAB_KB; j++) {
+    u32 c = r_cnt[(u64)p * SLAB_KB + j];
+    c = c < r_cap ? c : r_cap;
+    const Tup* __restrict__ piece = R + ((u64)p * SLAB_KB + j) * r_cap;
+    for (u32 i = lane; i < c; i += 64) hits += piece[i].key == key ? 1u : 0u;
+  }
+  const u32 total = (u32)wave_sum_u64((u64)hits);
+  if (lane == 0 && total != 1) atomicOr(reinterpret_cast<unsigned long long*>(&accum[ACC_ERR]), (unsigned long long)ERR_PROBE_PILOT);
+}
+hipError_t launch_probe_keys_pilot(const void* S, u32 np, const void* slab_br, const u32* cnt_br, u32 r_cap, int low, int bits,
+                                   u64* accum, hipStream_t st) {
+  if (!S || !slab_br || !cnt_br || !accum || np == 0 || bits < 1 || bits > 31 || low < 0 || low + bits > 64) return hipErrorInvalidValue;
+  const u32 waves = hmj_host::probe_keys_sample_count(np);
+  hipLaunchKernelGGL(probe_keys_pilot_kernel, dim3((waves + 3) / 4), dim3(256), 0, st, static_cast<const Tup*>(S), np,
+                     static_cast<const Tup*>(slab_br), cnt_br, r_cap, low, (1u << bits) - 1u, accum);
+  return hipGetLastError();
 }
 
 hipError_t launch_probe(const ProbeArgs& a, int mode, bool first_wins, bool extra, int grid,
diff --git a/hashmergejoin_amd/csrc/radix.hip b/hashmergejoin_amd/csrc/radix.hip
--- a/hashmergejoin_amd/csrc/radix.hip
+++ b/hashmergejoin_amd/csrc/radix.hip
@@ -233,6 +233,46 @@
 
 constexpr int WC_ITEMS = 4;
 constexpr int WC_LINE = 8;
+static_assert(WC_LINE * sizeof(Tup) == 128, "one line");
+__device__ __forceinline__ u64 row_key(const Tup& t) { return t.key; }
+__device__ __forceinline__ u64 row_key(u64 k) { return k; }
+__device__ __forceinline__ void row_set_key(Tup& t, u64 k) { t.key = k; }
+__device__ __forceinline__ void row_set_key(u64& t, u64 k) { t = k; }
+__device__ __forceinline__ u64 row_val(const Tup& t) { return t.val; }
+__device__ __forceinline__ u64 row_val(u64) { return 0; }
+template <typename Row>
+__device__ __forceinline__ Row make_row(u64 k, u64 v);
+template <>
+__device__ __forceinline__ Tup make_row<Tup>(u64 k, u64 v) {
+  Tup t;
+  t.key = k;
+  t.val = v;
+  return t;
+}
+template <>
+__device__ __forceinline__ u64 make_row<u64>(u64 k, u64) { return k; }
+__device__ __forceinline__ void store_stream(u64* p, u64 v) {
+#if HMJ_STREAM_POLICY >= 1
+  __builtin_nontemporal_store(v, p);
+#else
+  *p = v;
+#endif
+}
+__device__ __forceinline__ u64 load_stream(const u64* p) {
+#if HMJ_STREAM_POLICY >= 2
+  return __builtin_nontemporal_load(p);
+#else
+  return *p;
+#endif
+}
+__device__ __forceinline__ void store_stream2(u64* p, u64 a, u64 b) {
+#if HMJ_STREAM_POLICY >= 1
+  u64x2_t x = {a, b};
+  __builtin_nontemporal_store(x, reinterpret_cast<u64x2_t*>(p));
+#else
+  *reinterpret_cast<u64x2_t*>(p) = u64x2_t{a, b};
+#endif
+}
 
 #ifndef HMJ_WC_PLAN1
 #define HMJ_WC_PLAN1 0
@@ -274,19 +314,25 @@
 #define WC_VMWAIT()
 #endif
 
-template <int THREADS, int MAXD>
+template <int THREADS, int MAXD, typename Row = Tup, int ITEMS = WC_ITEMS>
 struct WcSmem {
-  static constexpr int TILE = THREADS * WC_ITEMS;
+  typedef Row row_type;
+  static constexpr int TILE = THREADS * ITEMS;
   static constexpr int WAVES = THREADS / kWave;
-  static constexpr int ZROWS = WAVES * MAXD * 8 / 16;
-  static constexpr int MAXLINES = TILE / WC_LINE + 2 * MAXD;
+  static constexpr int LINE = 128 / (int)sizeof(Row);
+  static constexpr int LINE_SHIFT = LINE == 8 ? 3 : 4;
+  static constexpr int CARRY_ITEMS = MAXD * LINE / THREADS;
+  static constexpr int ZROWS = WAVES * MAXD * 8 / (int)sizeof(Row);
+  static constexpr int MAXLINES = TILE / LINE + 2 * MAXD;
+  static_assert(sizeof(Row) == 16 || sizeof(Row) == 8, "rows of 16 bytes (Tup) or 8 (a key)");
   static_assert(ZROWS <= TILE && ZROWS % THREADS == 0, "lane masks must alias whole row slabs");
-  static_assert(MAXD <= THREADS && MAXD * WC_LINE == TILE, "one digit per thread; carry == tile slots");
+  static_assert(MAXD <= THREADS && (MAXD * LINE) % THREADS == 0 && TILE < 65536, "one digit per thread; whole carry rounds");
+  static_assert(sizeof(Row) == 8 || MAXD * LINE == TILE, "Tup rows: carry == tile slots");
   union {
-    Tup stage[TILE];
+    Row stage[TILE];
     u64 lanemask[WAVES][MAXD];
   };
-  Tup carry[MAXD][WC_LINE];
+  Row carry[MAXD][LINE];
   u16 wcnt[WAVES][MAXD];
   u32 tile_off[MAXD];
   u32 cflush[MAXD];
@@ -303,12 +349,15 @@
 struct NoLimit {
   __device__ __forceinline__ u32 operator()(u32) const { return 0xFFFFFFFFu; }
 };
-template <int THREADS, int MAXD, bool HI, bool ALLVALID, bool LIMIT, typename Prefetch, typename Limit>
-__device__ __forceinline__ void wc_tile(WcSmem<THREADS, MAXD>& sm, Tup (&t)[WC_ITEMS], u32 tile_n,
-                                        Tup* __restrict__ out, int shift, u32 mask, u32 D,
+template <int THREADS, int MAXD, bool HI, bool ALLVALID, bool LIMIT, typename Row, int ITEMS, typename Prefetch, typename Limit>
+__device__ __forceinline__ void wc_tile(WcSmem<THREADS, MAXD, Row, ITEMS>& sm, Row (&t)[ITEMS], u32 tile_n,
+                                        Row* __restrict__ out, int shift, u32 mask, u32 D,
                                         Prefetch&& prefetch, const Limit& limit, bool* ovf WC_STAMP_ARG) {
-  typedef WcSmem<THREADS, MAXD> Smem;
+  typedef WcSmem<THREADS, MAXD, Row, ITEMS> Smem;
   constexpr int WAVES = Smem::WAVES;
+  constexpr int WC_ITEMS = ITEMS;
+  constexpr int WC_LINE = Smem::LINE, LSH = Smem::LINE_SHIFT;
+  constexpr int CARRY_ITEMS = Smem::CARRY_ITEMS;
   const int tid = threadIdx.x, lane = tid & 63, w = tid >> 6;
   u16* wc = &sm.wcnt[w][0];
   u64* lm = &sm.lanemask[w][0];
@@ -326,7 +375,7 @@
   for (int r = 0; r < WC_ITEMS; r++) {
     u32 d = 0, rank = 0;
     if (ALLVALID || wbase + r * 64 < tile_n) {
-      d = digit_of<HI>(t[r].key, shift, mask);
+      d = digit_of<HI>(row_key(t[r]), shift, mask);
       __hip_atomic_fetch_or(&lm[d], lanebit, __ATOMIC_RELAXED, __HIP_MEMORY_SCOPE_WORKGROUP);
       const u64 m = __hip_atomic_load(&lm[d], __ATOMIC_RELAXED, __HIP_MEMORY_SCOPE_WORKGROUP);
       const u32 old = __hip_atomic_load(&wc[d], __ATOMIC_RELAXED, __HIP_MEMORY_SCOPE_WORKGROUP);
@@ -373,7 +422,7 @@
         }
         const u32 tail = (cf[j] + avail) & (WC_LINE - 1);
         fl[j] = (tail >= avail) ? 0u : avail - tail;
-        nl[j] = fl[j] ? (((cf[j] & (WC_LINE - 1)) + fl[j] + WC_LINE - 1) >> 3) : 0u;
+        nl[j] = fl[j] ? (((cf[j] & (WC_LINE - 1)) + fl[j] + WC_LINE - 1) >> LSH) : 0u;
         sm.pend[d] = avail - fl[j];
         sm.cflush[d] = cf[j] + fl[j];
       }
@@ -417,7 +466,7 @@
       }
       const u32 tail = (cf + avail) & (WC_LINE - 1);
       fl = (tail >= avail) ? 0u : avail - tail;
-      nl = fl ? (((cf & (WC_LINE - 1)) + fl + WC_LINE - 1) >> 3) : 0u;
+      nl = fl ? (((cf & (WC_LINE - 1)) + fl + WC_LINE - 1) >> LSH) : 0u;
       sm.pend[tid] = avail - fl;
       sm.cflush[tid] = cf + fl;
     }
@@ -451,7 +500,7 @@
   lds_barrier();
   WC_MARK(6);
 
-  {
+  if constexpr (sizeof(Row) == 16) {
     const u32 TL = sm.total_lines, k = (u32)tid & (WC_LINE - 1);
     for (u32 L = (u32)tid >> 3; L < TL; L += THREADS / WC_LINE) {
       const u32 d = sm.line_tab[L];
@@ -463,12 +512,33 @@
       const u32 j = grow - cfd;
       if (j < fl) store_stream(&out[grow], (j < pd) ? sm.carry[d][j] : sm.stage[sm.tile_off[d] + j - pd]);
     }
-  }
-  u64 keep_k[WC_ITEMS], keep_v[WC_ITEMS];
+  } else {
+    const u32 TL = sm.total_lines, k = ((u32)tid & 7u) * 2u;
+    for (u32 L = (u32)tid >> 3; L < TL; L += THREADS / 8) {
+      const u32 d = sm.line_tab[L];
+      const u32 pl = sm.plan[d], fl = pl >> 8, pd = pl & 0xFFu;
+      u32 cfd;
+      if constexpr (Smem::HAS_CF_TILE) cfd = sm.cf_tile[d];
+      else cfd = sm.cflush[d] - fl;
+      const u32 grow = (cfd & ~(u32)(WC_LINE - 1)) + (L - sm.line_off[d]) * WC_LINE + k;
+      const u32 j0 = grow - cfd, j1 = j0 + 1u;
+      const u32 toff = sm.tile_off[d] - pd;
+      const bool v0 = j0 < fl, v1 = j1 < fl;
+      u64 k0 = 0, k1 = 0;
+      if (v0) k0 = (j0 < pd) ? sm.carry[d][j0] : sm.stage[toff + j0];
+      if (v1) k1 = (j1 < pd) ? sm.carry[d][j1] : sm.stage[toff + j1];
+      if (v0 && v1) store_stream2(&out[grow], k0, k1);
+      else if (v0) store_stream(&out[grow], k0);
+      else if (v1) store_stream(&out[grow + 1], k1);
+    }
+  }
+  u64 keep_k[CARRY_ITEMS], keep_v[CARRY_ITEMS];
   u32 has = 0;
-#pragma unroll
-  for (int q = 0; q < WC_ITEMS; q++) {
-    const u32 s = q * THREADS + tid, d = s >> 3, k = s & (WC_LINE - 1);
+  int tid_c = tid;
+  if constexpr (sizeof(Row) == 8) asm volatile("" : "+v"(tid_c));
+#pragma unroll
+  for (int q = 0; q < CARRY_ITEMS; q++) {
+    const u32 s = q * THREADS + tid_c, d = s >> LSH, k = s & (WC_LINE - 1);
     u32 idx = 0;
     if (d < D && k < sm.pend[d]) {
       const u32 pl = sm.plan[d], fl = pl >> 8, pd = pl & 0xFFu;
@@ -477,29 +547,28 @@
         has |= 1u << q;
       }
     }
-    const Tup kv = sm.stage[idx];
-    keep_k[q] = kv.key;
-    keep_v[q] = kv.val;
+    const Row kv = sm.stage[idx];
+    keep_k[q] = row_key(kv);
+    keep_v[q] = row_val(kv);
   }
   WC_MARK(7);
   lds_barrier();
   WC_MARK(8);
 #pragma unroll
-  for (int q = 0; q < WC_ITEMS; q++) {
-    const u32 s = q * THREADS + tid;
-    if (has & (1u << q)) {
-      Tup kv;
-      kv.key = keep_k[q];
-      kv.val = keep_v[q];
-      sm.carry[s >> 3][s & (WC_LINE - 1)] = kv;
-    }
+  for (int q = 0; q < CARRY_ITEMS; q++) {
+    const u32 s = q * THREADS + tid_c;
+    if (has & (1u << q)) sm.carry[s >> LSH][s & (WC_LINE - 1)] = make_row<Row>(keep_k[q], keep_v[q]);
   }
 #if HMJ_WC_NOBAR5
   {
-    constexpr int ZR = MAXD * 8 / 16;
-    Tup z;
-    z.key = 0;
-    z.val = 0;
+    constexpr int ZR = MAXD * 8 / (int)sizeof(Row);
+    Row z;
+    if constexpr (sizeof(Row) == 16) {
+      z.key = 0;
+      z.val = 0;
+    } else {
+      z = 0;
+    }
 #pragma unroll
     for (int r = 0; r < ZR / kWave; r++) sm.stage[w * ZR + r * kWave + lane] = z;
     u32* wz = reinterpret_cast<u32*>(&sm.wcnt[w][0]);
@@ -512,9 +581,13 @@
 #pragma unroll
   for (int r = 0; r < WC_ITEMS; r++) {
     if (r * THREADS < Smem::ZROWS) {
-      Tup z;
-      z.key = 0;
-      z.val = 0;
+      Row z;
+      if constexpr (sizeof(Row) == 16) {
+        z.key = 0;
+        z.val = 0;
+      } else {
+        z = 0;
+      }
       sm.stage[r * THREADS + tid] = z;
     }
   }
@@ -525,20 +598,21 @@
 #endif
 }
 
-template <int THREADS, int MAXD>
-__device__ __forceinline__ void wc_flush_carry(WcSmem<THREADS, MAXD>& sm, Tup* __restrict__ out, u32 D) {
+template <int THREADS, int MAXD, typename Row, int ITEMS>
+__device__ __forceinline__ void wc_flush_carry(WcSmem<THREADS, MAXD, Row, ITEMS>& sm, Row* __restrict__ out, u32 D) {
+  typedef WcSmem<THREADS, MAXD, Row, ITEMS> Smem;
   const int tid = threadIdx.x;
   lds_barrier();
 #pragma unroll
-  for (int q = 0; q < WC_ITEMS; q++) {
-    const u32 s = q * THREADS + tid, d = s >> 3, k = s & (WC_LINE - 1);
+  for (int q = 0; q < Smem::CARRY_ITEMS; q++) {
+    const u32 s = q * THREADS + tid, d = s >> Smem::LINE_SHIFT, k = s & (Smem::LINE - 1);
     if (d < D && k < sm.pend[d]) store_stream(&out[sm.cflush[d] + k], sm.carry[d][k]);
   }
 }
 
-template <int THREADS, int MAXD>
-__device__ __forceinline__ void wc_clear(WcSmem<THREADS, MAXD>& sm) {
-  constexpr int WAVES = WcSmem<THREADS, MAXD>::WAVES;
+template <int THREADS, int MAXD, typename Row, int ITEMS>
+__device__ __forceinline__ void wc_clear(WcSmem<THREADS, MAXD, Row, ITEMS>& sm) {
+  constexpr int WAVES = WcSmem<THREADS, MAXD, Row, ITEMS>::WAVES;
   const int tid = threadIdx.x;
   for (int i = tid; i < WAVES * MAXD / 2; i += THREADS) reinterpret_cast<u32*>(&sm.wcnt[0][0])[i] = 0;
   for (int i = tid; i < WAVES * MAXD; i += THREADS) (&sm.lanemask[0][0])[i] = 0;
@@ -615,11 +689,15 @@
 struct NoXform {
   static constexpr bool kStrided = false;
 };
-template <int THREADS, int MAXD, bool HI, typename Xform>
+template <int THREADS, int MAXD, bool HI, typename Xform, typename Row = Tup>
 __device__ __forceinline__ void slab_a_body(const Tup* __restrict__ in, u32 n, int shift, int bits, u32 rows_per_worker,
-                                            Tup* __restrict__ slab, u32 CA, u32 WA, u32* __restrict__ cnt_out,
+                                            Row* __restrict__ slab, u32 CA, u32 WA, u32* __restrict__ cnt_out,
                                             u64* __restrict__ accum, u32 worker_base, Xform& xf) {
-  typedef WcSmem<THREADS, MAXD> Smem;
+  constexpr bool KEYS = !std::is_same<Row, Tup>::value;
+  constexpr int WC_ITEMS = KEYS ? 2 * hmj::WC_ITEMS : hmj::WC_ITEMS;
+  typedef WcSmem<THREADS, MAXD, Row, WC_ITEMS> Smem;
+  static_assert(!KEYS || std::is_same<Xform, NoXform>::value, "key rows: the join's plain pass A only");
+  u64 val_sum = 0;
   constexpr int TILE = Smem::TILE;
   extern __shared__ __attribute__((aligned(16))) unsigned char smem_raw[];
   Smem& sm = *reinterpret_cast<Smem*>(smem_raw);
@@ -702,15 +780,40 @@
         }
       };
       if constexpr (!std::is_same<Xform, NoXform>::value) xf(t, tile_n, wbase);
-      if (HMJ_WC_FULLTILE && tile_n == (u32)TILE)
-        wc_tile<THREADS, MAXD, HI, true, true>(sm, t, tile_n, slab, shift, mask, D, prefetch, limit, &ovf WC_STAMP_PASS);
-      else
-        wc_tile<THREADS, MAXD, HI, false, true>(sm, t, tile_n, slab, shift, mask, D, prefetch, limit, &ovf WC_STAMP_PASS);
+      if constexpr (KEYS) {
+        u64 tk[WC_ITEMS];
+#pragma unroll
+        for (int r = 0; r < WC_ITEMS; r++) {
+          tk[r] = t[r].key;
+          val_sum += (wbase + (u32)r * 64 < tile_n) ? t[r].val : 0ull;
+        }
+        if (HMJ_WC_FULLTILE && tile_n == (u32)TILE)
+          wc_tile<THREADS, MAXD, HI, true, true>(sm, tk, tile_n, slab, shift, mask, D, prefetch, limit, &ovf WC_STAMP_PASS);
+        else
+          wc_tile<THREADS, MAXD, HI, false, true>(sm, tk, tile_n, slab, shift, mask, D, prefetch, limit, &ovf WC_STAMP_PASS);
+      } else {
+        if (HMJ_WC_FULLTILE && tile_n == (u32)TILE)
+          wc_tile<THREADS, MAXD, HI, true, true>(sm, t, tile_n, slab, shift, mask, D, prefetch, limit, &ovf WC_STAMP_PASS);
+        else
+          wc_tile<THREADS, MAXD, HI, false, true>(sm, t, tile_n, slab, shift, mask, D, prefetch, limit, &ovf WC_STAMP_PASS);
+      }
     }
     wc_flush_carry(sm, slab, D);
   }
   if ((u32)tid < D) cnt_out[(u32)tid * WA + worker] = sm.cflush[tid] + sm.pend[tid] - ((u32)tid * WA + worker) * CA;
   if (ovf) atomicOr(&accum[ACC_ERR], ERR_SLAB);
+  if constexpr (KEYS) {
+    const u64 ws = wave_sum_u64(val_sum);
+    u64* red = reinterpret_cast<u64*>(sm.plan);
+    __syncthreads();
+    if (lane == 0) red[w] = ws;
+    __syncthreads();
+    if (tid == 0) {
+      u64 tot = 0;
+      for (int k = 0; k < THREADS / kWave; k++) tot += red[k];
+      if (tot) atomicAdd(reinterpret_cast<unsigned long long*>(&accum[ACC_SUM_S]), (unsigned long long)tot);
+    }
+  }
 #ifdef HMJ_STAMPS
   stamps.flush();
 #endif
@@ -728,13 +831,15 @@
 #endif
 constexpr int SLAB_MAXSEG = 512;
 
-template <int THREADS, int MAXD, bool HI, int ADDR>
+template <int THREADS, int MAXD, bool HI, int ADDR, typename Row = Tup>
 __global__ __launch_bounds__(THREADS, (THREADS * (MAXD <= 256 ? 2 : 1)) / 256) void radix_slab_b_kernel(
-    const Tup* __restrict__ slab_a, const u32* __restrict__ cnt_a, u32 CA, u32 WA, int bits_a, int shift,
-    int bits, Tup* __restrict__ slab_b, u32 CB, u32* __restrict__ cnt_b, u64* __restrict__ accum, u32 KB) {
-  typedef WcSmem<THREADS, MAXD> Smem;
+    const Row* __restrict__ slab_a, const u32* __restrict__ cnt_a, u32 CA, u32 WA, int bits_a, int shift,
+    int bits, Row* __restrict__ slab_b, u32 CB, u32* __restrict__ cnt_b, u64* __restrict__ accum, u32 KB) {
+  constexpr int WC_ITEMS = 64 / (int)sizeof(Row);
+  typedef WcSmem<THREADS, MAXD, Row, WC_ITEMS> Smem;
   constexpr int TILE = Smem::TILE;
   static_assert(SLAB_MAXSEG <= THREADS, "one A-slab count per thread in the prologue scan");
+  static_assert(ADDR == 2 || sizeof(Row) == 16, "the per-round lookups (ADDR 0 / 1) plan four rounds of Tup rows");
   extern __shared__ __attribute__((aligned(16))) unsigned char smem_raw[];
   Smem& sm = *reinterpret_cast<Smem*>(smem_raw);
   u32* pre = reinterpret_cast<u32*>(smem_raw + sizeof(Smem));
@@ -764,14 +869,14 @@
 #endif
   const u32 wbase = (u32)w * (WC_ITEMS * 64) + lane;
   (void)wbase;
-  const Tup* __restrict__ bucket = slab_a + (u64)(dA * WA + w0) * CA;
+  const Row* __restrict__ bucket = slab_a + (u64)(dA * WA + w0) * CA;
   bool ovf = false;
 #ifdef HMJ_STAMPS
   WcStamps stamps = {};
   stamps.base = 16;
 #endif
   if (total) {
-    Tup t[WC_ITEMS];
+    Row t[WC_ITEMS];
     if constexpr (ADDR != 0) {
     u32 d_s0 = 0, d_b0 = 0, d_b1 = 0, d_b2 = 0, d_b3 = 0;
     const float slabs_per_row = (float)ns / (float)total;
@@ -891,7 +996,7 @@
       u_b4 = (u32)__builtin_amdgcn_readlane((int)win_v, (int)j + 4);
     };
     auto issue2 = [&](u32 tile_begin) {
-      u64 off[WC_ITEMS];
+      typename std::conditional<sizeof(Row) == 8, u32, u64>::type off[WC_ITEMS];
       const u32 wq0 = tile_begin + wq;
       u32 wlast = wq0 + WC_ITEMS * 64 - 1;
       wlast = wlast < total ? wlast : total - 1;
@@ -955,7 +1060,7 @@
       if (abl == 1 || abl == 4) {
 #pragma unroll
         for (int r = 0; r < WC_ITEMS; r++)
-          if (t[r].key == 0) t[r].key = (u64)(tile + (u32)tid + r * THREADS + blockIdx.x * 7919u + 1) * 0x9E3779B97F4A7C15ull;
+          if (row_key(t[r]) == 0) row_set_key(t[r], (u64)(tile + (u32)tid + r * THREADS + blockIdx.x * 7919u + 1) * 0x9E3779B97F4A7C15ull);
       }
 #endif
       if (HMJ_WC_FULLTILE && tile_n == (u32)TILE)
@@ -1120,12 +1225,12 @@
   }
 }
 
-template <int THREADS, int MAXD, bool HI>
+template <int THREADS, int MAXD, bool HI, typename Row = Tup>
 __global__ __launch_bounds__(THREADS, (THREADS * (MAXD <= 256 ? 2 : 1)) / 256) void radix_slab_a_kernel(
-    const Tup* __restrict__ in, u32 n, int shift, int bits, u32 rows_per_worker, Tup* __restrict__ slab,
+    const Tup* __restrict__ in, u32 n, int shift, int bits, u32 rows_per_worker, Row* __restrict__ slab,
     u32 CA, u32 WA, u32* __restrict__ cnt_out, u64* __restrict__ accum, u32 worker_base) {
   NoXform xf;
-  slab_a_body<THREADS, MAXD, HI, NoXform>(in, n, shift, bits, rows_per_worker, slab, CA, WA, cnt_out, accum, worker_base, xf);
+  slab_a_body<THREADS, MAXD, HI, NoXform, Row>(in, n, shift, bits, rows_per_worker, slab, CA, WA, cnt_out, accum, worker_base, xf);
 }
 
 template <bool CUT>
@@ -1202,30 +1307,31 @@
     if (rows) atomicAdd(reinterpret_cast<unsigned long long*>(&accum[ACC_N]), (unsigned long long)rows);
   }
 }
-template <int THREADS, int MAXD, bool HI>
+template <int THREADS, int MAXD, bool HI, typename Row = Tup>
 static hipError_t launch_slab_a_t(const void* in, u32 n, int shift, int bits, u32 rpw, void* slab, u32 CA,
                                   u32 WA, u32* cnt, u64* accum, hipStream_t st, u32 w_begin, u32 w_end) {
-  typedef WcSmem<THREADS, MAXD> Smem;
+  typedef WcSmem<THREADS, MAXD, Row, (sizeof(Row) == 8 ? 2 : 1) * WC_ITEMS> Smem;
   const size_t smem = sizeof(Smem);
   static_assert(sizeof(Smem) <= 160 * 1024, "slab pass A: LDS");
   static SmemAttrOnce attr_once;
-  if (hipError_t e = ensure_max_smem(attr_once, reinterpret_cast<const void*>(radix_slab_a_kernel<THREADS, MAXD, HI>), (size_t)smem); e != hipSuccess) return e;
+  if (hipError_t e = ensure_max_smem(attr_once, reinterpret_cast<const void*>(radix_slab_a_kernel<THREADS, MAXD, HI, Row>), (size_t)smem); e != hipSuccess) return e;
   if (w_end > WA) w_end = WA;
   if (w_begin >= w_end) return hipSuccess;
-  hipLaunchKernelGGL((radix_slab_a_kernel<THREADS, MAXD, HI>), dim3(w_end - w_begin), dim3(THREADS), smem, st,
-                     static_cast<const Tup*>(in), n, shift, bits, rpw, static_cast<Tup*>(slab), CA, WA, cnt,
+  hipLaunchKernelGGL((radix_slab_a_kernel<THREADS, MAXD, HI, Row>), dim3(w_end - w_begin), dim3(THREADS), smem, st,
+                     static_cast<const Tup*>(in), n, shift, bits, rpw, static_cast<Row*>(slab), CA, WA, cnt,
                      accum, w_begin);
   return hipGetLastError();
 }
 
-template <int THREADS, int MAXD, bool HI>
+template <int THREADS, int MAXD, bool HI, typename Row = Tup>
 static hipError_t launch_slab_b_t(const void* slab_a, const u32* cnt_a, u32 CA, u32 WA, int bits_a, int shift,
                                   int bits, void* slab_b, u32 CB, u32* cnt_b, u64* accum, hipStream_t st, u32 KB) {
-  typedef WcSmem<THREADS, MAXD> Smem;
+  typedef WcSmem<THREADS, MAXD, Row, 64 / (int)sizeof(Row)> Smem;
   const size_t smem = sizeof(Smem) + (SLAB_MAXSEG + 1) * sizeof(u32);
   static_assert(sizeof(Smem) + (SLAB_MAXSEG + 1) * sizeof(u32) <= 160 * 1024, "slab pass B: LDS");
+  static_assert(HMJ_B_ADDR == 2 || sizeof(Row) == 16, "key rows: the wave-uniform lookup only");
 #ifdef HMJ_DEV
-  if (g_b_addr_alt) {
+  if (g_b_addr_alt && sizeof(Row) == 16) {
     constexpr int ALT = HMJ_B_ADDR == 2 ? 1 : 2;
     static SmemAttrOnce attr_alt;
     if (hipError_t e = ensure_max_smem(attr_alt, reinterpret_cast<const void*>(radix_slab_b_kernel<THREADS, MAXD, HI, ALT>), (size_t)smem); e != hipSuccess) return e;
@@ -1236,10 +1342,10 @@
   }
 #endif
   static SmemAttrOnce attr_once;
-  if (hipError_t e = ensure_max_smem(attr_once, reinterpret_cast<const void*>(radix_slab_b_kernel<THREADS, MAXD, HI, HMJ_B_ADDR>), (size_t)smem); e != hipSuccess) return e;
-  hipLaunchKernelGGL((radix_slab_b_kernel<THREADS, MAXD, HI, HMJ_B_ADDR>), dim3((1u << bits_a) * KB), dim3(THREADS), smem, st,
-                     static_cast<const Tup*>(slab_a), cnt_a, CA, WA, bits_a, shift, bits,
-                     static_cast<Tup*>(slab_b), CB, cnt_b, accum, KB);
+  if (hipError_t e = ensure_max_smem(attr_once, reinterpret_cast<const void*>(radix_slab_b_kernel<THREADS, MAXD, HI, HMJ_B_ADDR, Row>), (size_t)smem); e != hipSuccess) return e;
+  hipLaunchKernelGGL((radix_slab_b_kernel<THREADS, MAXD, HI, HMJ_B_ADDR, Row>), dim3((1u << bits_a) * KB), dim3(THREADS), smem, st,
+                     static_cast<const Row*>(slab_a), cnt_a, CA, WA, bits_a, shift, bits,
+                     static_cast<Row*>(slab_b), CB, cnt_b, accum, KB);
   return hipGetLastError();
 }
 
@@ -1295,12 +1401,17 @@
 }
 
 hipError_t launch_slab_a(const void* in, u32 n, int shift, int bits, const SlabGeom& g, void* slab_a, u64 slab_a_rows,
-                         u32* cnt_a, u64 cnt_a_n, u64* accum, hipStream_t st, u32 w_begin, u32 w_end) {
+                         u32* cnt_a, u64 cnt_a_n, u64* accum, hipStream_t st, u32 w_begin, u32 w_end, bool keys) {
   if (bits < 1 || bits > SLAB_MAX_BITS || g.WA == 0 || g.CA == 0 || (u64)g.WA * g.rpw < n) return hipErrorInvalidValue;
   if (slab_a_rows < ((u64)g.WA << bits) * g.CA || cnt_a_n < ((u64)g.WA << bits)) return hipErrorInvalidValue;
   if (((u64)g.WA << bits) * g.CA >= 0xFFFFFFF0ull) return hipErrorInvalidValue;
   const bool hi = shift >= 32;
 #define HMJ_SLAB_A(T, M, H) launch_slab_a_t<T, M, H>(in, n, shift, bits, g.rpw, slab_a, g.CA, g.WA, cnt_a, accum, st, w_begin, w_end)
+  if (keys) {
+    if (bits > 8 || (g.CA & 15u)) return hipErrorInvalidValue;
+    return hi ? launch_slab_a_t<512, 256, true, u64>(in, n, shift, bits, g.rpw, slab_a, g.CA, g.WA, cnt_a, accum, st, w_begin, w_end)
+              : launch_slab_a_t<512, 256, false, u64>(in, n, shift, bits, g.rpw, slab_a, g.CA, g.WA, cnt_a, accum, st, w_begin, w_end);
+  }
   if (bits > 8) return hi ? HMJ_SLAB_A(1024, 512, true) : HMJ_SLAB_A(1024, 512, false);
   return hi ? HMJ_SLAB_A(512, 256, true) : HMJ_SLAB_A(512, 256, false);
 #undef HMJ_SLAB_A
@@ -1348,7 +1459,8 @@
 }
 
 hipError_t launch_slab_b(const void* slab_a, const u32* cnt_a, int bits_a, int shift, int bits,
-                         const SlabGeom& g, void* slab_b, u64 slab_b_rows, u32* cnt_b, u64 cnt_b_n, u64* accum, hipStream_t st) {
+                         const SlabGeom& g, void* slab_b, u64 slab_b_rows, u32* cnt_b, u64 cnt_b_n, u64* accum, hipStream_t st,
+                         bool keys) {
   if (bits < 1 || bits > SLAB_MAX_BITS || bits_a < 1 || bits_a > SLAB_MAX_BITS || g.KB == 0 || g.WA < g.KB ||
       (g.WA + g.KB - 1) / g.KB > (u32)SLAB_MAXSEG)
     return hipErrorInvalidValue;
@@ -1356,6 +1468,11 @@
   if (slab_b_rows < pieces * g.CB || cnt_b_n < pieces || pieces * g.CB >= 0xFFFFFFF0ull) return hipErrorInvalidValue;
   const bool hi = shift >= 32;
 #define HMJ_SLAB_B(T, M, H) launch_slab_b_t<T, M, H>(slab_a, cnt_a, g.CA, g.WA, bits_a, shift, bits, slab_b, g.CB, cnt_b, accum, st, g.KB)
+  if (keys) {
+    if (bits > 8 || bits_a > 8 || ((g.CA | g.CB) & 15u)) return hipErrorInvalidValue;
+    return hi ? launch_slab_b_t<512, 256, true, u64>(slab_a, cnt_a, g.CA, g.WA, bits_a, shift, bits, slab_b, g.CB, cnt_b, accum, st, g.KB)
+              : launch_slab_b_t<512, 256, false, u64>(slab_a, cnt_a, g.CA, g.WA, bits_a, shift, bits, slab_b, g.CB, cnt_b, accum, st, g.KB);
+  }
   if (bits > 8) return hi ? HMJ_SLAB_B(1024, 512, true) : HMJ_SLAB_B(1024, 512, false);
   return hi ? HMJ_SLAB_B(512, 256, true) : HMJ_SLAB_B(512, 256, false);
 #undef HMJ_SLAB_B
diff --git a/include/hmj.h b/include/hmj.h
--- a/include/hmj.h
+++ b/include/hmj.h
@@ -93,6 +93,7 @@
 #define HMJ_PATH_LDS_TABLE 0x800000u
 #define HMJ_PATH_GLOBAL_TABLE 0x100000u
 #define HMJ_PATH_HOST_PIPELINE 0x4000u
+#define HMJ_PATH_PROBE_KEYS 0x10000000u
 
 typedef struct {
   uint32_t struct_size;
@@ -122,6 +123,8 @@
 #define HMJ_REFUSED_SLAB_PROBE_OVERFLOW 0x2000u
 #define HMJ_REFUSED_PREFIX_VIOLATED 0x4000u
 #define HMJ_REFUSED_EXPANSION_GAVE_UP 0x8000u
+#define HMJ_REFUSED_PROBE_KEYS_GAVE_UP 0x10000u
+#define HMJ_REFUSED_PROBE_KEYS_COOLING 0x20000u
 #define HMJ_COOL_UNIQ_WRITE 0x001u
 #define HMJ_COOL_SORTED_WRITE 0x002u
 #define HMJ_COOL_GTABLE 0x004u
@@ -136,6 +139,7 @@
 #define HMJ_COOL_EXACT_PREFIX 0x800u
 #define HMJ_COOL_RANK_RUNS 0x1000u
 #define HMJ_COOL_SORT_MSD 0x2000u
+#define HMJ_COOL_PROBE_KEYS 0x4000u
 
 int hmj_create(hmj_ctx** out, int device_id);
 void hmj_destroy(hmj_ctx* ctx);
```
